# saugns/saugns

Hardware: AMD Instinct MI355X
Metric: mono samples/sec/GPU @ N voices (depth-3 FM) (higher is better)
Workload: dtype f32 (f64 table interpolation, u32 phase)

## Files before the change

### __graft_entry__.py

```python
import os
import subprocess
import sys

ROOT = os.path.dirname(os.path.abspath(__file__))
if ROOT not in sys.path:
    sys.path.insert(0, ROOT)


def build():
    import saugns_amd
    saugns_amd.build(force=False)
    subprocess.check_call(["make", "-s", "-C", os.path.join(ROOT, "tests", "seqexec")])
    subprocess.check_call(["make", "-s", "-C", os.path.join(ROOT, "tests", "hooks")])
    subprocess.check_call(["make", "-s", "-C", os.path.join(ROOT, "tests", "hooks_levels")])
    subprocess.check_call(["make", "-s", "-C", os.path.join(ROOT, "tests", "hooks_oversample")])
    subprocess.check_call(["make", "-s", "-C", os.path.join(ROOT, "tests", "hooks_loudness")])
    subprocess.check_call(["make", "-s", "-C", os.path.join(ROOT, "tests", "hooks_limiter")])
    subprocess.check_call(["make", "-s", "-C", os.path.join(ROOT, "tests", "hooks_spectrum")])
    subprocess.check_call(["make", "-s", "-C", os.path.join(ROOT, "tests", "hooks_plan")])
    subprocess.check_call(["make", "-s", "-C", os.path.join(ROOT, "oracle"), "oracle"])
    subprocess.check_call(["make", "-s", "-C", os.path.join(ROOT, "oracle"), "ref"])
    subprocess.check_call(["make", "-s", "-C", os.path.join(ROOT, "oracle"), "hosts"])
    saugns_amd.lib()


def smoke():
    import numpy as np
    import saugns_amd as sa
    from saugns_amd import voicebank
    from oracle import pyoracle as po

    tabs = np.fromfile(os.path.join(ROOT, "tests", "golden", "piluts_ref.f32"),
                       dtype="<f4").reshape(12, 2048)
    sa.set_piluts(tabs)
    po.oracle_use_tables(tabs)
    po.oracle().ora_set_fastmath_forms(1)
    prg = voicebank.config3(n=16, seconds=1)
    want = po.oracle_render(prg.ptr, 44100, False)
    got = sa.Generator(prg, 44100).render(stereo=False)
    assert len(got) == len(want) == 44100, (len(got), len(want))
    diff = int(np.abs(got.astype(np.int32) - want.astype(np.int32)).max())
    assert diff == 0, f"GPU render differs from the oracle by {diff} LSB"
    print("smoke ok: 16 voices x depth-3 PM, 44100 frames, bit-exact vs oracle")
    from saugns_amd.api import POP_FMOD
    fm = [voicebank.Op("sin", freq=voicebank.Line(110.0 + 20 * k, goal=330.0, shape="exp"), time_ms=500,
                       mods={POP_FMOD: [voicebank.Op("sin", freq=5.0 + k, amp=20.0)]}) for k in range(8)]
    for name, p in (("8 FM voices with gliding carriers", voicebank.build_program(fm)),
                    ("16 feedback voices (config 5)", voicebank.config5(n=16, seconds=1))):
        want = po.oracle_render(p.ptr, 44100, False)
        got = sa.Generator(p, 44100).render(stereo=False)
        assert len(got) == len(want) and (got == want).all(), name
        print(f"smoke ok: {name}, {len(got)} frames, bit-exact vs oracle")


if __name__ == "__main__":
    build()
    if "--smoke" in sys.argv:
        smoke()
```

### saugns_amd/build.py

```python
import os
import subprocess
import sys

HERE = os.path.dirname(os.path.abspath(__file__))
CSRC = os.path.join(HERE, "csrc")
LIB = os.path.join(HERE, "libsaugns_amd.so")
SOURCES = ["capi.cpp", "engine.cpp", "plan.cpp", "tables.cpp", "program_io.cpp", "sndout.cpp", "bank_builder.cpp",
           "hip_backend.hip"]
HEADERS = ["engine.h", "hip_backend.h", "capi_internal.h", "sau_dev_math.h", "sau_dev_ops.h", "launch_plan.h",
           "k_common.h", "k_wave_scan.h", "k_block_loop.h", "k_fast_types.h", "k_analyze.h", "k_decode.h", "k_fast_voice.h", "k_fast_group.h", "k_fast_group_lm.h",
           "k_chain.h", "k_finish.h", "k_levels.h", "k_decimate.h", "k_loudness.h", "k_limiter.h", "k_spectrum.h",
           "sau_dev_types.h", "../../include/sau_abi.h", "../../include/saugns_amd.h"]
FLAGS = ["--offload-arch=gfx950", "-O3", "-ffp-contract=off", "-fPIC", "-std=c++17",
         "-Wall", "-fvisibility=hidden", "-fvisibility-inlines-hidden"]


def _stale():
    if not os.path.exists(LIB):
        return True
    t = os.path.getmtime(LIB)
    deps = [os.path.join(CSRC, f) for f in SOURCES + HEADERS] + [__file__]
    return any(os.path.getmtime(d) > t for d in deps)


def build_variant(name, defines):
    build()
    hipcc = os.environ.get("HIPCC", "/opt/rocm/bin/hipcc")
    vdir = os.path.join(HERE, "variants")
    os.makedirs(vdir, exist_ok=True)
    obj = os.path.join(vdir, "hip_backend_%s.o" % name)
    subprocess.check_call([hipcc] + FLAGS + ["-D" + d for d in defines] +
                          ["-c", os.path.join(CSRC, "hip_backend.hip"), "-o", obj])
    objs = [os.path.join(CSRC, s.rsplit(".", 1)[0] + ".o") for s in SOURCES if s != "hip_backend.hip"]
    out = os.path.join(vdir, "lib_%s.so" % name)
    subprocess.check_call([hipcc, "--offload-arch=gfx950", "-shared", "-fPIC", "-o", out] + objs + [obj, "-ldl"])
    return out


def build(force=False, verbose=False):
    if not force and not _stale():
        return LIB
    import fcntl
    with open(os.path.join(HERE, ".build.lock"), "w") as lock:
        fcntl.flock(lock, fcntl.LOCK_EX)
        try:
            if not force and not _stale():
                return LIB
            return _build(verbose, force)
        finally:
            fcntl.flock(lock, fcntl.LOCK_UN)


def _build(verbose, force=False):
    hipcc = os.environ.get("HIPCC", "/opt/rocm/bin/hipcc")
    objs = []
    for src in SOURCES:
        obj = os.path.join(CSRC, src.rsplit(".", 1)[0] + ".o")
        objs.append(obj)
        deps = [src] + [h for h in HEADERS if src.endswith(".hip") or not h.startswith("k_")]
        if not force and os.path.exists(obj) and all(
                os.path.getmtime(os.path.join(CSRC, d)) <= os.path.getmtime(obj) for d in deps) and \
                os.path.getmtime(__file__) <= os.path.getmtime(obj):
            continue
        cmd = [hipcc] + FLAGS + ["-c", os.path.join(CSRC, src), "-o", obj]
        if verbose:
            print(" ".join(cmd), file=sys.stderr)
        subprocess.check_call(cmd)
    cmd = [hipcc, "--offload-arch=gfx950", "-shared", "-fPIC", "-o", LIB] + objs + ["-ldl"]
    subprocess.check_call(cmd)
    return LIB


if __name__ == "__main__":
    if len(sys.argv) > 2 and sys.argv[1] == "--variant":
        print(build_variant(sys.argv[2], sys.argv[3:]))
    else:
        print(build(force="--force" in sys.argv, verbose=True))
```

### saugns_amd/csrc/hip_backend.hip

```cpp
#include <hip/hip_runtime.h>
#include "hip_backend.h"
#include "launch_plan.h"
#include "sau_dev_ops.h"
#include <stdio.h>
#include <stdlib.h>
#include <string.h>
#include <deque>
#include <map>
#include <mutex>
#include <string>
#include <type_traits>
#include <vector>

namespace sauhip {

using namespace saudev;
using sauengine::BackendConfig;
using sauengine::tune_env;
using sauengine::SegmentDesc;
using namespace sauplan;

#include "k_common.h"
#include "k_block_loop.h"
#include "k_fast_types.h"
// ... 129 lines not shown
}
static void pool_free(bool pinned, void *q, size_t bytes) {
	if (!q) return;
	if (!BufPool::get().give(pinned, q, bytes)) { if (pinned) (void)hipHostFree(q); else (void)hipFree(q); }
}

static std::mutex &attr_mutex() { static std::mutex *m = new std::mutex; return *m; }
static bool raise_lds_attr(const void *fn, size_t lds, int dev, std::string &err) {
	static std::map<std::pair<const void *, int>, size_t> *slots = new std::map<std::pair<const void *, int>, size_t>;
	std::lock_guard<std::mutex> lk(attr_mutex());
	size_t &configured = (*slots)[std::make_pair(fn, dev & 15)];
	if (lds > configured) {
		hipError_t e = hipFuncSetAttribute(fn, hipFuncAttributeMaxDynamicSharedMemorySize, (int)lds);
		if (e != hipSuccess) { err = std::string("hipFuncSetAttribute: ") + hipGetErrorString(e); return false; }
		configured = lds;
	}
	return true;
}

enum : unsigned { FK_WIDE = 1, FK_TAIL = 2, FK_CUB = 4, FK_INNER = 8, FK_LANEMAJOR = 16 };
static const void *fast_kernel_fn(int build, uint32_t rows, unsigned form) {
	struct Entry { int build; uint32_t rows; unsigned form; const void *fn; };
#define FK(build, form, ...) {build, FK_ROWS(__VA_ARGS__), form, (const void *)fast_kernel<__VA_ARGS__>}
#define FK_ROWS(rows, ...) rows
	static const Entry table[] = {
		FK(0, 0, 2, 0), FK(0, 0, 4, 0), FK(0, 0, 5, 0), FK(0, 0, 6, 0), FK(0, 0, 8, 0),
		FK(1, 0, 2, 1), FK(1, 0, 4, 1),
		FK(2, 0, 2, 2), FK(2, 0, 4, 2), FK(2, 0, 5, 2), FK(2, 0, 6, 2), FK(2, 0, 8, 2),
		FK(3, 0, 4, 3), FK(3, 0, 5, 3), FK(3, 0, 6, 3),
		FK(0, FK_WIDE, 6, 0, false, true), FK(0, FK_WIDE, 8, 0, false, true), FK(0, FK_WIDE, 10, 0, false, true), FK(0, FK_WIDE, 12, 0, false, true),
		FK(2, FK_WIDE | FK_TAIL, 8, 2, false, true, true), FK(2, FK_WIDE, 8, 2, false, true), FK(2, FK_TAIL, 8, 2, false, false, true),
		FK(2, FK_CUB, (int)FAST_CUB_ROWS, 2, true),
		FK(0, FK_WIDE | FK_INNER | FK_LANEMAJOR, 12, 0, false, true, false, true, true), FK(0, FK_WIDE | FK_INNER, 12, 0, false, true, false, true),
		FK(0, FK_CUB, (int)FAST_CUB_ROWS, 0, true)};
#undef FK
#undef FK_ROWS
	for (const Entry &e : table)
		if (e.build == build && e.rows == rows && e.form == form) return e.fn;
	return nullptr;
}
static const void *repair_kernel_fn(uint32_t rows, bool wide) {
	if (wide)
		return rows == 12 ? (const void *)repair_kernel<12, true> : rows == 10 ? (const void *)repair_kernel<10, true>
		     : rows == 8 ? (const void *)repair_kernel<8, true> : rows == 6 ? (const void *)repair_kernel<6, true> : nullptr;
	return rows == 8 ? (const void *)repair_kernel<8> : rows == 6 ? (const void *)repair_kernel<6> : rows == 5 ? (const void *)repair_kernel<5>
	     : rows == 4 ? (const void *)repair_kernel<4> : rows == 2 ? (const void *)repair_kernel<2> : nullptr;
}
static const void *render_kernel_fn(uint32_t W, uint32_t T, uint32_t V, bool HB) {
	struct Entry { uint32_t W, T, V; bool HB; const void *fn; };
#define RK(W, T, V, HB) {W, T, V, HB, (const void *)render_kernel<W, T, V, HB>}
	static const Entry table[] = {
		RK(1, 4, 8, false), RK(1, 3, 8, false), RK(1, 2, 8, false), RK(1, 1, 8, false),
		RK(1, 4, 16, false), RK(1, 3, 16, false), RK(1, 2, 16, false), RK(1, 1, 16, false),
		RK(1, 1, 1, true), RK(1, 1, 1, false), RK(4, 4, 1, false), RK(8, 2, 1, false)};
#undef RK
	for (const Entry &e : table)
		if (e.W == W && e.T == T && e.V == V && e.HB == HB) return e.fn;
	return nullptr;
}

template <typename T, bool PINNED> struct PoolBuf {
	T *p = nullptr;
	size_t cap = 0, bytes = 0;
	PoolBuf() = default;
	PoolBuf(const PoolBuf &) = delete;
	PoolBuf &operator=(const PoolBuf &) = delete;
	~PoolBuf() { release(); }
	bool ensure(size_t n, std::string &err, bool keep = false) {
		if (n <= cap) return true;
		size_t nbytes = (n + n / 4 + 16) * sizeof(T);
		T *q = (T *)pool_alloc(PINNED, nbytes, err);
		if (!q) return false;
		if (keep && p && cap) {
			hipError_t e = PINNED ? (memcpy(q, p, cap * sizeof(T)), hipSuccess)
			                      : hipMemcpy(q, p, cap * sizeof(T), hipMemcpyDeviceToDevice);
			if (e != hipSuccess) { err = hipGetErrorString(e); return false; }
		}
		if (p) { (void)hipDeviceSynchronize(); pool_free(PINNED, p, bytes); }
		p = q; bytes = nbytes; cap = nbytes / sizeof(T);
		return true;
	}
	void release() { pool_free(PINNED, p, bytes); p = nullptr; cap = 0; bytes = 0; }
};
template <typename T> using DevBuf = PoolBuf<T, false>;
template <typename T> using PinBuf = PoolBuf<T, true>;

struct TableSet {
	int dev;
	std::vector<float> piluts;
	WaveConst wconst[12];
	HerpC23 *c23;
	HerpC01 *c01;
	WaveConst *wc;
};
static const TableSet *shared_tables(const float *piluts, const WaveConst *wconst, std::string &err) {
	static std::mutex mu;
	static std::vector<TableSet *> sets;
	int dev = 0;
	(void)hipGetDevice(&dev);
	std::lock_guard<std::mutex> lk(mu);
	for (const TableSet *t : sets)
		if (t->dev == dev && !memcmp(t->piluts.data(), piluts, (size_t)12 * WAVE_LEN * sizeof(float)) &&
		    !memcmp(t->wconst, wconst, sizeof t->wconst))
			return t;
	std::vector<HerpC23> h23((size_t)12 * WAVE_LEN);
	std::vector<HerpC01> h01((size_t)12 * WAVE_LEN);
	for (uint32_t wv = 0; wv < 12; ++wv)
		for (uint32_t i = 0; i < WAVE_LEN; ++i) {
			if (!herp_c1_scalable(piluts + (size_t)wv * WAVE_LEN, i)) {
				err = "wave table has slopes below 2^-100: unsupported";
				return nullptr;
			}
			herp_coeffs(piluts + (size_t)wv * WAVE_LEN, i,
					h23[(size_t)wv * WAVE_LEN + i], h01[(size_t)wv * WAVE_LEN + i]);
		}
	TableSet *t = new TableSet;
	t->dev = dev;
	t->piluts.assign(piluts, piluts + (size_t)12 * WAVE_LEN);
	memcpy(t->wconst, wconst, sizeof t->wconst);
	t->c23 = nullptr; t->c01 = nullptr; t->wc = nullptr;
	hipError_t e = hipMalloc((void **)&t->c23, h23.size() * sizeof(HerpC23));
	if (e == hipSuccess) e = hipMalloc((void **)&t->c01, h01.size() * sizeof(HerpC01));
	if (e == hipSuccess) e = hipMalloc((void **)&t->wc, 12 * sizeof(WaveConst));
	if (e == hipSuccess) e = hipMemcpy(t->c23, h23.data(), h23.size() * sizeof(HerpC23), hipMemcpyHostToDevice);
	if (e == hipSuccess) e = hipMemcpy(t->c01, h01.data(), h01.size() * sizeof(HerpC01), hipMemcpyHostToDevice);
	if (e == hipSuccess) e = hipMemcpy(t->wc, wconst, 12 * sizeof(WaveConst), hipMemcpyHostToDevice);
	if (e != hipSuccess) {
		err = std::string("wave tables: ") + hipGetErrorString(e);
		(void)hipFree(t->c23); (void)hipFree(t->c01); (void)hipFree(t->wc);
		delete t;
		return nullptr;
	}
	sets.push_back(t);
	return t;
}

int device_count() {
	int n = 0;
	if (hipGetDeviceCount(&n) != hipSuccess) return 0;
	return n;
}

bool device_pci_bus_id(int dev, char *buf, int len) {
	if (!buf || len < 16) return false;
	buf[0] = 0;
	return hipDeviceGetPCIBusId(buf, len, dev) == hipSuccess;
}

class HipBackendImpl : public HipBackend {
public:
	explicit HipBackendImpl(int device = -1) : want_dev_(device) {}
	void use_device() { (void)hipSetDevice(dev_); }

	~HipBackendImpl() override {
		use_device();
		if (stream_) (void)hipStreamSynchronize(stream_);
		if (chain_stream_) { (void)hipStreamSynchronize(chain_stream_); StreamPool::get().give(dev_, chain_stream_, 1); }
		for (hipEvent_t e : chain_ev_) (void)hipEventDestroy(e);
		for (int i = 0; i < 4; ++i) if (fetch_ev_[i]) (void)hipEventDestroy(fetch_ev_[i]);
		if (after_ev_) (void)hipEventDestroy(after_ev_);
		for (auto &e : events_) { (void)hipEventDestroy(e.a); (void)hipEventDestroy(e.b); }
		if (stream_) StreamPool::get().give(dev_, stream_);
	}

	bool init(const BackendConfig &cfg, std::string &err) override {
		cfg_ = cfg;
		int dev = 0;
		const char *env = getenv("SAU_AMD_DEVICE");
		if (want_dev_ >= 0) dev = want_dev_;
		else if (env) dev = atoi(env);
		if (dev < 0 || dev >= device_count()) { err = "no HIP device " + std::to_string(dev) + " (" + std::to_string(device_count()) + " visible)"; return false; }
		HIP_OK(hipSetDevice(dev));
		dev_ = dev;
		stream_ = StreamPool::get().take(dev);
		if (!stream_) HIP_OK(hipStreamCreateWithFlags(&stream_, hipStreamNonBlocking));
		static std::mutex prop_mu;
		static size_t dev_lds[16];
		static uint32_t dev_cus[16];
		static size_t dev_free[16];
		{
			std::lock_guard<std::mutex> lk(prop_mu);
			if (!dev_lds[dev & 15]) {
				hipDeviceProp_t prop;
				HIP_OK(hipGetDeviceProperties(&prop, dev));
				dev_lds[dev & 15] = prop.maxSharedMemoryPerMultiProcessor ? prop.maxSharedMemoryPerMultiProcessor
				                                                          : prop.sharedMemPerBlock;
				dev_cus[dev & 15] = prop.multiProcessorCount > 0 ? (uint32_t)prop.multiProcessorCount : FK_GRID;
				size_t mfree = 0, mtotal = 0;
				if (hipMemGetInfo(&mfree, &mtotal) == hipSuccess) dev_free[dev & 15] = mfree;
			}
			free_hint_ = dev_free[dev & 15];
			tun_ = tuning_from_env(tune_env);
			lim_ = device_limits(dev_lds[dev & 15], dev_cus[dev & 15], tun_);
		}
		debug_ = getenv("SAU_AMD_DEBUG") != nullptr;
		inmix_report_ = tune_env("SAU_AMD_INMIX_REPORT") != nullptr;
		inner_report_ = tune_env("SAU_AMD_INNER_REPORT") != nullptr;
		if (!ops_.ensure(cfg.op_count ? cfg.op_count : 1, err)) return false;
		HIP_OK(hipMemsetAsync(ops_.p, 0, ops_.cap * sizeof(DevOp), stream_));
		tables_ = shared_tables(cfg.piluts, cfg.wconst, err);
		if (!tables_) return false;
		memcpy(wconst_, cfg.wconst, sizeof wconst_);
		return true;
	}

	bool reserve_frames(uint32_t max_frames, bool , std::string &err) override {
		use_device();
		HIP_OK(hipStreamSynchronize(stream_));
		row_stride_ = (max_frames + 63) & ~63u;
		pcm_row_ = (size_t)row_stride_ * 2;
		if (!pcm_.ensure(pcm_row_ * cfg_.n_streams * pcm_units(), err)) return false;
		set_.vout_rows = 0;
		return true;
	}

	size_t pcm_units() const { return pcm_f32_ ? 2 : 1; }
	size_t pcm_pitch() const { return pcm_row_ * pcm_units() * sizeof(int16_t); }
	char *pcm_at(uint32_t stream) const { return (char *)pcm_.p + pcm_pitch() * stream; }
	bool set_format(sauengine::SampleFormat fmt, std::string &err) override {
		use_device();
		const bool f32 = fmt == sauengine::SF_F32;
		if (f32 == pcm_f32_) return true;
		pcm_f32_ = f32;
		if (pcm_row_ && !pcm_.ensure(pcm_row_ * cfg_.n_streams * pcm_units(), err)) { pcm_f32_ = !f32; return false; }
		return true;
	}

	void *stage(const void *src, size_t bytes, std::string &err) {
		const size_t need = (bytes + 63) & ~(size_t)63;
		if (arena_used_ + need > arena_.cap) {
			hipError_t e = hipStreamSynchronize(stream_);
			if (e != hipSuccess) { err = std::string("hipStreamSynchronize: ") + hipGetErrorString(e); return nullptr; }
			arena_used_ = 0;
			const size_t want = need > ((size_t)4 << 20) ? need : ((size_t)4 << 20);
			if (want > arena_.cap && !arena_.ensure(want, err)) return nullptr;
		}
		void *p = arena_.p + arena_used_;
		arena_used_ += need;
		memcpy(p, src, bytes);
		return p;
	}
	bool send(void *dst, const void *src, size_t bytes, std::string &err) {
		if (!bytes) return true;
		void *h = stage(src, bytes, err);
		if (!h) return false;
		HIP_OK(hipMemcpyAsync(dst, h, bytes, hipMemcpyHostToDevice, stream_));
		return true;
	}

	bool upload_plans(const Step *steps, const FastIds *fast_ids, size_t n_steps, const uint32_t *op_ids,
			size_t n_ids, std::string &err) override {
		use_device();
		if (!steps_.ensure(n_steps ? n_steps : 1, err) || !op_ids_.ensure(n_ids ? n_ids : 1, err) ||
		    !fast_ids_.ensure(n_steps ? 2 * n_steps : 1, err))
			return false;
		n_steps_total_ = (uint32_t)n_steps;
		return send(steps_.p, steps, n_steps * sizeof(Step), err) &&
			send(fast_ids_.p, fast_ids, 2 * n_steps * sizeof(FastIds), err) &&
			send(op_ids_.p, op_ids, n_ids * sizeof(uint32_t), err);
	}

	bool apply_updates(const OpUpdate *recs, size_t n, std::string &err) override {
		use_device();
		if (!n) return true;
		if (!recs_.ensure(n, err) || !send(recs_.p, recs, n * sizeof(OpUpdate), err)) return false;
		hipLaunchKernelGGL(event_kernel, dim3((unsigned)((n + 63) / 64)), dim3(64), 0, stream_,
				ops_.p, recs_.p, (uint32_t)n, tables_->wc);
		HIP_OK(hipGetLastError());
		return true;
	}

	bool poison_run(uint32_t frames, bool stereo, std::string &err) override {
		(void)frames; (void)stereo;
		use_device();
		if (pcm_.p) HIP_OK(hipMemsetD16Async((hipDeviceptr_t)pcm_.p, 0x5a5a, pcm_row_ * cfg_.n_streams * pcm_units(), stream_));
		return true;
	}

	bool zero_pcm(uint32_t first_stream, uint32_t n_streams, uint32_t first_frame, uint32_t n_frames, bool stereo,
			std::string &err) override {
		use_device();
		if (!pcm_.p || !n_streams || !n_frames) return true;
		const size_t fb = (stereo ? 2 : 1) * pcm_units() * sizeof(int16_t);
		char *at = pcm_at(first_stream) + (size_t)first_frame * fb;
		if (n_streams == 1) HIP_OK(hipMemsetAsync(at, 0, (size_t)n_frames * fb, stream_));
		else HIP_OK(hipMemset2DAsync(at, pcm_pitch(), 0, (size_t)n_frames * fb, n_streams, stream_));
		return true;
	}

	struct TimedPair { hipEvent_t a, b; int kind; bool used; };

	struct Job {
		const SegmentDesc &seg;
		PlanInputs in;
		BlockLoopPlan bl;
		FastPlan fk;
		RenderParams rp;
		FastParams fp;
		FastParams cfp;
		bool launched = true;
		bool tail_live = false;
		bool inmix_live = false;
		uint32_t early_mixed_blocks = 0;
		uint32_t block_grid = 1;
		TimedPair *tf = nullptr;
		explicit Job(const SegmentDesc &s) : seg(s) { memset(&rp, 0, sizeof rp); memset(&fp, 0, sizeof fp); }
	};

	bool render(const SegmentDesc &seg, std::string &err) override {
		use_device();
		if (!seg.n_voices) return true;
		++acc_launches_;
		Job j(seg);
		j.in.f32 = seg.format == sauengine::SF_F32;
		if (j.in.f32 != pcm_f32_) { err = "a segment of another sample format than the run announced"; return false; }
		if (j.in.f32 && seg.swap_bytes) { err = "float32 samples are not byte-swapped"; return false; }
		j.in.row_stride = row_stride_; j.in.pcm_row = pcm_row_; j.in.chain_budget = chain_rows_budget();
		j.bl = plan_block_loop(seg, tun_, lim_);
		if (!j.bl.ok) { err = "voice too large for one workgroup's LDS (block buffers + operator states)"; return false; }
		if (!ensure_rows(j, err) || !upload_descriptors(j, err)) return false;
		j.fk = plan_fast(seg, tun_, lim_, j.in);
		if (!prepare_fast(j, err) || !prepare_chains(j, err)) return false;
		fill_tables(j);
		if (!launch_analyze(j, err)) return false;
		if (j.fk.use_fast) {
			if (!launch_decode(j, err)) return false;
			if (j.fk.main_build == 2 && !launch_split(j, err)) return false;
			if (j.fp.scan ? !launch_sums_and_chains(j, err) : !launch_closed_form(j, err)) return false;
			if (!launch_cub(j, err)) return false;
			if (!j.launched) return false;
			if (!launch_repair(j, err)) return false;
			if (j.tf) (void)hipEventRecord(j.tf->b, stream_);
		}
		if (!launch_finalize(j, err)) return false;
		if (!launch_block_loop(j, err)) return false;
		return launch_mixer(j, err);
	}

	bool ensure_rows(Job &j, std::string &err) {
		const SegmentDesc &seg = j.seg;
		MixSet &S = set_;
		if (!voices_.ensure(seg.n_voices, err) || !S.vinfo.ensure(seg.n_voices, err)) return false;
		if (seg.n_voices > S.vout_rows || !S.vout.p) {
			HIP_OK(hipStreamSynchronize(stream_));
			if (!S.vout.ensure((size_t)seg.n_voices * row_stride_, err)) return false;
			S.vout_rows = seg.n_voices;
		}
		if (seg.n_pan_rows && !S.pan.ensure((size_t)seg.n_pan_rows * row_stride_, err)) return false;
		if (tun_.poison) {
			HIP_OK(hipMemsetD32Async((hipDeviceptr_t)S.vout.p, 0x3ea5a5a5, (size_t)seg.n_voices * row_stride_, stream_));
			if (seg.n_pan_rows) HIP_OK(hipMemsetD32Async((hipDeviceptr_t)S.pan.p, 0x3ea5a5a5, (size_t)seg.n_pan_rows * row_stride_, stream_));
		}
		return S.mstreams.ensure(seg.n_streams, err);
	}

	bool upload_descriptors(Job &j, std::string &err) {
		const SegmentDesc &seg = j.seg;
		MixSet &S = set_;
		ms_host_.resize(seg.n_streams);
		for (uint32_t s = 0; s < seg.n_streams; ++s) {
			MixStream &m = ms_host_[s];
			memset(&m, 0, sizeof m);
			m.first_row = seg.streams[s].first_voice;
			m.n_rows = seg.streams[s].n_voices;
			m.amp_scale = seg.streams[s].amp_scale;
			m.write_len = seg.streams[s].write_len;
			m.pcm = (int16_t *)pcm_at(s);
			if (m.write_len > j.in.max_write) j.in.max_write = m.write_len;
			if (m.n_rows > j.in.max_rows) j.in.max_rows = m.n_rows;
		}
		const bool same_voices = voices_sent_.size() == seg.n_voices && voices_dev_ == voices_.p &&
			memcmp(voices_sent_.data(), seg.voices, seg.n_voices * sizeof(VoiceDesc)) == 0;
		const bool same_ms = S.ms_sent.size() == seg.n_streams && S.ms_dev == S.mstreams.p &&
			memcmp(S.ms_sent.data(), ms_host_.data(), seg.n_streams * sizeof(MixStream)) == 0;
		if (!same_voices) {
			if (!send(voices_.p, seg.voices, seg.n_voices * sizeof(VoiceDesc), err)) return false;
			voices_sent_.assign(seg.voices, seg.voices + seg.n_voices);
			voices_dev_ = voices_.p;
		}
		if (!same_ms) {
			if (!send(S.mstreams.p, ms_host_.data(), seg.n_streams * sizeof(MixStream), err)) return false;
			S.ms_sent = ms_host_;
			S.ms_dev = S.mstreams.p;
		}
		return true;
	}

	bool prepare_fast(Job &j, std::string &err) {
		const SegmentDesc &seg = j.seg;
		const FastPlan &k = j.fk;
		FastParams &fp = j.fp;
		MixSet &S = set_;
		const size_t n_lists = (size_t)FAST_LISTS * seg.n_voices * k.fmax_steps;
		if (!finfo_.ensure(seg.n_voices, err) || !fdone_.ensure(seg.n_voices, err) ||
		    !worklist_.ensure(seg.n_voices, err) || !work_count_.ensure(4, err) ||
		    !fsteps_.ensure(n_lists * sizeof(FastStep), err) || !flines_.ensure(n_lists * sizeof(FastLine), err) ||
		    !faux_.ensure(n_lists * sizeof(FastAux), err)) return false;
		fp.voices = voices_.p; fp.steps = steps_.p; fp.fast_ids = fast_ids_.p; fp.op_ids = op_ids_.p; fp.ops = ops_.p;
		fp.vout = S.vout.p; fp.pan = S.pan.p; fp.info = finfo_.p; fp.fast_done = fdone_.p;
		fp.worklist = worklist_.p; fp.work_count = work_count_.p; fp.vinfo = S.vinfo.p;
		fp.g_c23 = tables_->c23; fp.g_c01 = tables_->c01; fp.fsteps = (FastStep *)fsteps_.p; fp.flines = (FastLine *)flines_.p; fp.faux = (FastAux *)faux_.p;
		fp.row_stride = row_stride_; fp.n_voices = seg.n_voices; fp.n_fast = k.n_fast;
		fp.seq_enable = k.seq_ok ? 1u : 0u; fp.ids_full_ofs = n_steps_total_;
		fp.scan = nullptr; fp.scan_groups = k.scan_groups; fp.mode = 0;
		if (tun_.xcd_queues && lim_.eight_xcds) {
			if (!inmix_ctl_.ensure(INMIX_WORDS, err)) return false;
			fp.inmix = inmix_ctl_.p;
		}
		if (k.scan) {
			if (!scan_.ensure((size_t)seg.n_voices * FAST_MAX_SCAN * k.scan_groups, err)) return false;
			fp.scan = scan_.p;
		}
		if (k.look) {
			if (k.look_words_real || !k.look_inside) {
				const unsigned long long *before = look_.p;
				if (!look_.ensure(k.look_words, err)) return false;
				if (look_.p != before || look_epoch_ >= (1u << 30) - 1) {
					HIP_OK(hipMemsetAsync(look_.p, 0, look_.cap * sizeof(unsigned long long), stream_));
					look_epoch_ = 0;
				}
				fp.look_epoch = ++look_epoch_;
			} else if (!look_.p && !look_.ensure(64, err)) {
				return false;
			}
			fp.look = look_.p;
		}
		if (!pass_flags_.p) {
			if (!pass_flags_.ensure(FAST_FLAGS, err)) return false;
			HIP_OK(hipMemsetAsync(pass_flags_.p, 0, pass_flags_.cap * sizeof(uint32_t), stream_));
		}
		fp.pass_flags = pass_flags_.p;
		fp.sum_levels = k.sum_levels;
		if (!repair_.ensure((size_t)seg.n_voices * FAST_REPAIR_WORDS, err)) return false;
		fp.repair = repair_.p;
		fp.repair_on = tun_.repair ? 1u : 0u;
		fp.max_ops = seg.max_ops; fp.max_steps = k.fmax_steps; fp.np = 64; fp.rows = k.rows; fp.rows_multi = k.rows_multi;
		fp.enable = k.use_fast ? 1u : 0u;
		if (k.inc_rows) {
			if (!inc_rows_.ensure((size_t)seg.n_inc_rows * 2 * k.inc_stride + 64, err)) return false;
			fp.inc_rows = inc_rows_.p; fp.inc_stride = k.inc_stride; fp.n_inc_rows = seg.n_inc_rows;
		}
		if (k.split_cf) {
			if (!vlists_.ensure((size_t)2 * seg.n_voices, err)) return false;
			fp.vlists = vlists_.p; fp.split_cf = 1; fp.rows_cf = k.rows_cf;
			fp.look_words_real = k.look_words_real && fp.look ? 1u : 0u;
		}
		fp.cub_ok = k.cub_ok ? 1u : 0u;
		memcpy(fp.wc, wconst_, sizeof wconst_);
		return true;
	}

	bool prepare_chains(Job &j, std::string &err) {
		const SegmentDesc &seg = j.seg;
		FastPlan &k = j.fk;
		FastParams &fp = j.fp;
		if (k.chains) {
			std::string rows_err;
			const size_t rows_need = (size_t)seg.n_chain_rows * 2 * k.chain_stride + 64;
			const char *rft = chain_rows_failed_once_ ? nullptr : tune_env("SAU_AMD_CHAIN_ROWS_FAIL");
			const bool rows_fail_test = rft && strcmp(rft, "real") != 0;
			if (rows_fail_test || !chain_rows_.ensure((rft && !rows_fail_test) ? (size_t)1 << 44 : rows_need, rows_err)) {
				chain_rows_failed_once_ = true;
				++chain_rows_failures_;
				if (debug_) fprintf(stderr, "saugns_amd: %zu bytes of chain rows not available (%s): block loop for this segment\n",
						rows_need * sizeof(float), rows_err.c_str());
				k.drop_chains();
			}
		}
		if (k.chains) {
			if (!chain_desc_.ensure(seg.n_chain_slots, err) ||
			    !fplines_.ensure((size_t)FAST_LISTS * seg.n_voices * k.fmax_steps * sizeof(FastLine), err)) return false;
			if (seg.chain_rows_padded) HIP_OK(hipMemsetAsync(chain_desc_.p, 0, (size_t)seg.n_chain_slots * sizeof(ChainDesc), stream_));
			fp.chain_rows = chain_rows_.p; fp.chain_stride = k.chain_stride; fp.n_chain_rows = seg.n_chain_rows; fp.n_chain_slots = seg.n_chain_slots;
			fp.chain_desc = chain_desc_.p; fp.fplines = (FastLine *)fplines_.p;
			fp.chain_inline = tun_.chain_inline ? 1u : 0u;
			fp.chain_early_ok = tun_.chain_early ? 1u : 0u;
			memcpy(fp.ctab_of_wave, k.ctabs.tab_of_wave, sizeof fp.ctab_of_wave);
			memcpy(fp.cwave_of_tab, k.ctabs.wave_of_tab, sizeof fp.cwave_of_tab);
			fp.n_ctabs = k.ctabs.n;
		}
		fp.lean_on = k.lean_on ? 1u : 0u;
		fp.rows_lean = k.rows_lean;
		return true;
	}

	void fill_tables(Job &j) {
		memcpy(j.fp.tab_of_wave, j.fk.tabs.tab_of_wave, sizeof j.fp.tab_of_wave);
		memcpy(j.fp.wave_of_tab, j.fk.tabs.wave_of_tab, sizeof j.fp.wave_of_tab);
		j.fp.n_tabs = j.fk.tabs.n;
	}

	bool launch_analyze(Job &j, std::string &err) {
		const SegmentDesc &seg = j.seg;
		(void)err;
		TimedPair *ta = timing_on_ ? new_pair(3) : nullptr;
		if (ta) (void)hipEventRecord(ta->a, stream_);
		uint32_t lo = seg.max_ops, ls = seg.max_steps;
		size_t albytes = (size_t)lo * sizeof(DevOp) + (size_t)ls * sizeof(Step) + (size_t)lo * sizeof(uint32_t);
		if (albytes > 48 * 1024 || !tun_.analyze_lds) { lo = 0; ls = 0; albytes = 0; }
		hipLaunchKernelGGL(analyze_kernel, dim3(seg.n_voices), dim3(64), albytes, stream_, j.fp, lo, ls);
		if (ta) (void)hipEventRecord(ta->b, stream_);
		return true;
	}
	bool launch_decode(Job &j, std::string &err) {
		hipLaunchKernelGGL(decode_kernel, dim3(j.seg.n_voices), dim3(64), 0, stream_, j.fp);
		if (!wait_for_predecessor(err)) return false;
		j.tf = timing_on_ ? new_pair(2) : nullptr;
		if (j.tf) (void)hipEventRecord(j.tf->a, stream_);
		return true;
	}

	bool launch_build(Job &j, std::string &err, int build, uint32_t rows, uint32_t grid, const FastParams *prm = nullptr, bool cf = false,
			bool wide = false) {
		if (build == 1 && rows > 4) rows = 4;
		if (build == 3) rows = rows < 5 ? 4 : rows > 6 ? 6 : rows;
		const void *fn = fast_kernel_fn(build, rows, (wide ? FK_WIDE : 0u) | (build == 2 && j.tail_live ? FK_TAIL : 0u));
		if (!fn) {
			err = "internal error: no fast_kernel build with " + std::to_string(rows) + " rows per pass in this form";
			return false;
		}
		const size_t lds = j.fk.launch_lds(build, rows, wide, cf);
		void *args[] = {(void *)(prm ? prm : &j.fp)};
		if (!raise_lds_attr(fn, lds, dev_, err)) return false;
		HIP_OK(hipLaunchKernel(fn, dim3(grid), dim3(1024), args, lds, stream_));
		return true;
	}
	void launch_fast(Job &j, std::string &err, uint32_t mode, uint32_t grid = 0) {
		FastParams &fp = j.fp;
		if (!grid) grid = j.fk.grid;
		fp.mode = mode;
		if (fp.lean_on && fp.chain_rows && (mode == fp.sum_levels + 1 || mode == fp.sum_levels + 2) &&
		    !launch_build(j, err, 3, fp.rows_lean, grid))
			j.launched = false;
		if (j.fk.main_build == 2) {
			fp.only_multi = 1;
			if (!launch_build(j, err, 1, j.fk.rows_multi, grid)) j.launched = false;
			fp.only_multi = 0;
		} else if (!launch_build(j, err, j.fk.main_build, j.fk.rows, grid, nullptr, false, j.fk.wide_cf)) {
			j.launched = false;
		}
	}

	bool launch_split(Job &j, std::string &err) {
		const SegmentDesc &seg = j.seg;
		const FastPlan &k = j.fk;
		FastParams &fp = j.fp, &cfp = j.cfp;
		if (k.tailmix) {
			if (!tail_ok_.ensure(seg.n_streams, err)) return false;
			fp.tail_ok = tail_ok_.p; fp.inmix_stream = set_.mstreams.p;
			fp.tail_flags = (seg.stereo ? 1u : 0u) | (seg.swap_bytes ? 2u : 0u);
			fp.tail_pcm_offset = seg.pcm_offset;
			hipLaunchKernelGGL(tailmix_kernel, dim3((seg.n_streams + 63) / 64), dim3(64), 0, stream_, fp, seg.n_streams);
			j.tail_live = true;
		}
		cfp = fp;
		cfp.n_fast = k.n_fast_cf; cfp.rows = k.rows_cf; cfp.mode = 0; cfp.only_multi = 0;
		if (getenv("SAU_AMD_DEBUG_DUO"))
			fprintf(stderr, "[sau-amd] duo %d: enabled %d look %d words_real %u FT %u rows_cf %u cub_ok %u tail %d may_scan %u of %u voices, lds %zu of %zu\n",
					(int)k.duo, (int)tun_.duo, fp.look != nullptr, fp.look_words_real, k.rows, k.rows_cf, fp.cub_ok, (int)j.tail_live, seg.n_may_scan, seg.n_voices,
					k.launch_lds(2, k.rows, false) + 1024, lim_.lds_limit);
		cfp.dyn_chunks = k.tasks_cf.dyn_chunks; cfp.dyn_static = k.tasks_cf.dyn_static;
		if (!k.duo && !launch_build(j, err, 0, k.rows_cf, k.grid_cf, &cfp, true, k.wide_cf)) j.launched = false;
		fp.mode = fp.sum_levels + 1; fp.only_multi = 0; fp.look_wpv = k.look_wpv; fp.look_groups = k.groups;
		fp.look_wpv_flags = k.look_wpv_flags;
		if (k.duo) {
			const size_t dlds = k.launch_lds(2, k.rows, false);
			if (!raise_lds_attr((const void *)duo_kernel, dlds, dev_, err)) return false;
			auto go = [&]() -> bool {
				void *da[] = {(void *)&fp, (void *)&cfp};
				return hipLaunchKernel((const void *)duo_kernel, dim3(lim_.fk_grid), dim3(1024), da, dlds, stream_) == hipSuccess;
			};
			if (!SpreadLaunchOrder::get().ordered(dev_, stream_, go)) j.launched = false;
		} else if (fp.look) {
			if (k.look_inside) {
				if (!launch_build(j, err, 2, k.rows, k.grid_look, nullptr, false, k.wide_look)) j.launched = false;
			} else if (!SpreadLaunchOrder::get().ordered(dev_, stream_, [&]() { return launch_build(j, err, 2, k.rows, k.grid_look, nullptr, false, k.wide_look); })) {
				j.launched = false;
			}
			if (fp.cub_ok) {
				const void *ck2 = fast_kernel_fn(2, FAST_CUB_ROWS, FK_CUB);
				const size_t lds2 = k.launch_lds(2, FAST_CUB_ROWS, false);
				if (!raise_lds_attr(ck2, lds2, dev_, err)) return false;
				auto go = [&]() -> bool {
					void *a2[] = {(void *)&fp};
					return hipLaunchKernel(ck2, dim3(k.grid_look), dim3(1024), a2, lds2, stream_) == hipSuccess;
				};
				if (k.look_inside ? !go() : !SpreadLaunchOrder::get().ordered(dev_, stream_, go)) j.launched = false;
			}
		}
		return true;
	}

	bool launch_sums_and_chains(Job &j, std::string &err) {
		const SegmentDesc &seg = j.seg;
		FastParams &fp = j.fp;
		if (fp.chain_rows && fp.chain_early_ok && !launch_early_chains(j, err)) return false;
		for (uint32_t pass = 1; pass <= fp.sum_levels && (!fp.look || seg.n_chain_rows); ++pass) {
			launch_fast(j, err, pass);
			hipLaunchKernelGGL(scan_kernel, dim3(seg.n_voices), dim3(64), 0, stream_, fp);
		}
		if (!fp.chain_rows) { launch_fast(j, err, fp.sum_levels + 1); return true; }
		return launch_chains(j, err);
	}

	bool launch_early_chains(Job &j, std::string &err) {
		FastParams &fp = j.fp;
		const uint32_t cgrid = j.fk.chain_grid;
		const size_t clds = chain_alone_lds((size_t)fp.n_ctabs * CHAIN_TAB_BYTES + CHAIN_IO_BYTES, cgrid);
		if (!raise_lds_attr((const void *)chain_kernel, clds, dev_, err)) return false;
		fp.chain_early = 1; fp.range_mode = 0;
		hipLaunchKernelGGL(chain_kernel, dim3(cgrid), dim3(192), clds, stream_, fp);
		const size_t rlds = chain_alone_lds(RCHAIN_LDS_BYTES, cgrid);
		if (!raise_lds_attr((const void *)rchain_kernel, rlds, dev_, err)) return false;
		hipLaunchKernelGGL(rchain_kernel, dim3(cgrid), dim3(RCHAIN_THREADS), rlds, stream_, fp);
		fp.chain_early = 0;
		return true;
	}

	bool launch_chains(Job &j, std::string &err) {
		const FastPlan &k = j.fk;
		FastParams &fp = j.fp;
		const uint32_t cgrid = k.chain_grid, n_chunks = k.chunks.n;
		const size_t clds = chain_alone_lds((size_t)fp.n_ctabs * CHAIN_TAB_BYTES + CHAIN_IO_BYTES, cgrid);
		if (!raise_lds_attr((const void *)chain_kernel, clds, dev_, err)) return false;
		TimedPair *tc = nullptr;
		if (n_chunks == 1) {
			tc = timing_on_ ? new_pair(0) : nullptr;
			fp.range_mode = 0;
			launch_fast(j, err, fp.sum_levels + 2);
			if (tc) (void)hipEventRecord(tc->a, stream_);
			hipLaunchKernelGGL(chain_kernel, dim3(cgrid), dim3(192), clds, stream_, fp);
			if (tc) (void)hipEventRecord(tc->b, stream_);
			launch_fast(j, err, fp.sum_levels + 1);
			return true;
		}
		if (!chain_stream_) {
			chain_stream_ = StreamPool::get().take(dev_, 1);
			if (!chain_stream_) {
				int lo = 0, hi = 0;
				(void)hipDeviceGetStreamPriorityRange(&lo, &hi);
				HIP_OK(hipStreamCreateWithPriority(&chain_stream_, hipStreamNonBlocking, hi));
			}
		}
		while (chain_ev_.size() < 2 * (size_t)n_chunks) {
			hipEvent_t e;
			HIP_OK(hipEventCreateWithFlags(&e, hipEventDisableTiming));
			chain_ev_.push_back(e);
		}
		tc = timing_on_ ? new_pair(0) : nullptr;
		const uint32_t *cb = k.chunks.cb;
		auto set_range = [&](FastParams &q, uint32_t mode, uint32_t c) {
			q.range_mode = mode; q.f_lo = cb[c]; q.f_hi = c + 1 == n_chunks ? 0xffffffffu : cb[c + 1];
		};
		for (uint32_t c = 0; c < n_chunks; ++c) {
			set_range(fp, 1, c);
			fp.range_last = c + 1 == n_chunks;
			launch_fast(j, err, fp.sum_levels + 2, k.pass_grid);
			HIP_OK(hipEventRecord(chain_ev_[2 * c], stream_));
			HIP_OK(hipStreamWaitEvent(chain_stream_, chain_ev_[2 * c], 0));
			FastParams cp = fp;
			set_range(cp, 1, c);
			if (tc && c == 0) (void)hipEventRecord(tc->a, chain_stream_);
			hipLaunchKernelGGL(chain_kernel, dim3(cgrid), dim3(192), clds, chain_stream_, cp);
			if (tc && c + 1 == n_chunks) (void)hipEventRecord(tc->b, chain_stream_);
			HIP_OK(hipEventRecord(chain_ev_[2 * c + 1], chain_stream_));
		}
		uint32_t mixed_blocks = 0;
		if (k.early_mix) hipLaunchKernelGGL(premix_kernel, dim3((j.seg.n_voices + 63) / 64), dim3(64), 0, stream_, fp);
		for (uint32_t c = 0; c < n_chunks; ++c) {
			HIP_OK(hipStreamWaitEvent(stream_, chain_ev_[2 * c + 1], 0));
			set_range(fp, 2, c);
			fp.range_last = c + 1 == n_chunks;
			launch_fast(j, err, fp.sum_levels + 1, c + 1 == n_chunks ? k.grid : k.pass_grid);
			if (k.early_mix && c + 1 < n_chunks && cb[c + 1] > 512) {
				const uint32_t hi = (cb[c + 1] - 512) / 256;
				if (hi > mixed_blocks) {
					MixParams mp = mix_params(j.seg, set_);
					mp.blk_lo = mixed_blocks; mp.blk_hi = hi;
					TimedPair *tm = timing_on_ ? new_pair(1) : nullptr;
					if (tm) (void)hipEventRecord(tm->a, stream_);
					hipLaunchKernelGGL((j.in.f32 ? mix_kernel_f32 : mix_kernel), dim3(hi - mixed_blocks, j.seg.n_streams), dim3(256), 0, stream_, mp);
					if (tm) (void)hipEventRecord(tm->b, stream_);
					mixed_blocks = hi;
				}
			}
		}
		j.early_mixed_blocks = mixed_blocks;
		fp.range_mode = 0; fp.f_lo = 0; fp.f_hi = 0; fp.range_last = 0;
		return true;
	}

	bool launch_closed_form(Job &j, std::string &err) {
		const SegmentDesc &seg = j.seg;
		const FastPlan &k = j.fk;
		FastParams &fp = j.fp;
		fp.dyn_chunks = k.tasks.dyn_chunks; fp.dyn_static = k.tasks.dyn_static; fp.dyn_small = k.tasks.dyn_small;
		if (k.queues) {
			fp.inmix_flags = k.inmix_flags;
			fp.inmix_div_s = k.div.s; fp.inmix_div_m = k.div.m;
			if (k.inmix) {
				fp.inmix_stream = set_.mstreams.p;
				fp.inmix_pcm_offset = seg.pcm_offset;
				hipLaunchKernelGGL(premix_kernel, dim3((seg.n_voices + 63) / 64), dim3(64), 0, stream_, fp);
				j.inmix_live = true;
			}
		}
		if (k.inner != INNER_NONE) {
			const bool lm = k.inner == INNER_LANE_MAJOR;
			const void *ik = fast_kernel_fn(0, 12, FK_WIDE | FK_INNER | (lm ? FK_LANEMAJOR : 0u));
			const size_t lds = k.inner_lds();
			FastParams ep = fp;
			ep.mode = 0; ep.edge_only = 1; ep.dyn_static = 1; ep.dyn_chunks = 2; ep.dyn_small = 0; ep.inmix_flags = 0;
			if (!launch_build(j, err, 0, k.rows, k.grid_edge, &ep, false, true)) j.launched = false;
			fp.mode = 0;
			void *iargs[] = {(void *)&fp};
			if (!raise_lds_attr(ik, lds, dev_, err)) return false;
			HIP_OK(hipLaunchKernel(ik, dim3(k.grid), dim3(1024), iargs, lds, stream_));
			if (inner_report_) fprintf(stderr, "[sau-amd] inner: %s, %u voices\n", lm ? "lane-major" : "row-major", seg.n_voices);
		} else {
			if (inner_report_) fprintf(stderr, "[sau-amd] inner: none (rows %u, wide %d, chunks %u), %u voices\n", k.rows, k.wide_cf ? 1 : 0, fp.dyn_chunks, seg.n_voices);
			launch_fast(j, err, 0);
		}
		fp.dyn_chunks = 0; fp.inmix_flags = 0; fp.dyn_small = 0;
		return true;
	}

	bool launch_cub(Job &j, std::string &err) {
		if (!j.fp.cub_ok) return true;
		const FastPlan &k = j.fk;
		FastParams q = k.main_build == 2 ? j.cfp : j.fp;
		q.n_fast = k.n_fast_cf; q.rows = FAST_CUB_ROWS; q.mode = 0; q.only_multi = 0;
		q.dyn_chunks = k.tasks_cub.dyn_chunks; q.dyn_static = k.tasks_cub.dyn_static;
		const size_t qlds = k.launch_lds(0, FAST_CUB_ROWS, false, true);
		const void *ck = fast_kernel_fn(0, FAST_CUB_ROWS, FK_CUB);
		if (!raise_lds_attr(ck, qlds, dev_, err)) return false;
		void *qargs[] = {(void *)&q};
		HIP_OK(hipLaunchKernel(ck, dim3(k.grid_cub), dim3(1024), qargs, qlds, stream_));
		return true;
	}

	bool launch_repair(Job &j, std::string &err) {
		const FastPlan &k = j.fk;
		const size_t rlds = k.launch_lds(0, k.rows_repair, k.wide_cf, k.main_build == 2);
		FastParams rpar = k.main_build == 2 ? j.cfp : j.fp;
		rpar.mode = 0;
		const void *rk = repair_kernel_fn(k.rows_repair, k.wide_cf);
		if (!rk) {
			err = "internal error: no repair_kernel build with " + std::to_string(k.rows_repair) + " rows per pass in this form";
			return false;
		}
		if (!raise_lds_attr(rk, rlds, dev_, err)) return false;
		j.fp.mode = 0;
		void *rargs[] = {(void *)&rpar};
		HIP_OK(hipLaunchKernel(rk, dim3(k.grid_repair), dim3(1024), rargs, rlds, stream_));
		return true;
	}

	bool launch_finalize(Job &j, std::string &err) {
		const SegmentDesc &seg = j.seg;
		TimedPair *tz = timing_on_ ? new_pair(3) : nullptr;
		if (tz) (void)hipEventRecord(tz->a, stream_);
		hipLaunchKernelGGL(finalize_kernel, dim3((unsigned)(((size_t)seg.n_voices * j.fp.max_ops * 8 + 63) / 64)), dim3(64), 0,
				stream_, j.fp);
		if (tz) (void)hipEventRecord(tz->b, stream_);
		HIP_OK(hipGetLastError());
		if (debug_ && j.fk.use_fast) {
			(void)hipStreamSynchronize(stream_);
			FastInfo fi0;
			(void)hipMemcpy(&fi0, finfo_.p, sizeof fi0, hipMemcpyDeviceToHost);
			fprintf(stderr, "[sau-amd] fast: voice 0 total %u H %u bail %u steps %u seq %u; n_fast %u rows %u\n",
					fi0.total, fi0.H, fi0.bail, fi0.n_fsteps, fi0.seq, j.fk.n_fast, j.fk.rows);
			std::vector<FastStep> fs(fi0.n_fsteps < 64 ? fi0.n_fsteps : 64);
			if (!fs.empty()) (void)hipMemcpy(fs.data(), fsteps_.p, fs.size() * sizeof(FastStep), hipMemcpyDeviceToHost);
			for (size_t i = 0; i < fs.size(); ++i)
				fprintf(stderr, "[sau-amd]   step %zu kind %u flags %#x which %u dep %u out %d pm %d fpm %d amp %d aux %d type %#x inc %u ac %g fc %g ramp %u\n",
						i, fs[i].kind & 0xff, (fs[i].kind >> 8) & 0xff, (fs[i].kind >> 16) & 0xff, fs[i].kind >> 24,
						(int)fs[i].out_off, (int)fs[i].pm_off, (int)fs[i].fpm_off, (int)fs[i].amp_off, (int)fs[i].aux_off,
						fs[i].type, fs[i].inc, fs[i].ac, fs[i].fc, fs[i].ramp);
		}
		return true;
	}

	bool launch_block_loop(Job &j, std::string &err) {
		const SegmentDesc &seg = j.seg;
		const BlockLoopPlan &b = j.bl;
		RenderParams &rp = j.rp;
		rp.team_bytes = (uint32_t)b.team_bytes;
		memcpy(rp.tab_of_wave, b.tabs.tab_of_wave, sizeof rp.tab_of_wave);
		memcpy(rp.wave_of_tab, b.tabs.wave_of_tab, sizeof rp.wave_of_tab);
		rp.voices = voices_.p; rp.steps = steps_.p; rp.op_ids = op_ids_.p; rp.ops = ops_.p;
		rp.vout = set_.vout.p; rp.pan = set_.pan.p; rp.vinfo = set_.vinfo.p;
		rp.g_c23 = tables_->c23; rp.g_c01 = tables_->c01;
		rp.row_stride = row_stride_; rp.seg_len = seg.len;
		rp.n_slots = seg.n_slots; rp.max_ops = seg.max_ops; rp.n_tabs = b.tabs.n;
		rp.max_steps = seg.max_steps; rp.n_main = seg.n_main;
		memcpy(rp.wc, wconst_, sizeof wconst_);
		rp.fast_done = fdone_.p; rp.worklist = worklist_.p; rp.work_count = work_count_.p;
		j.block_grid = b.grid(seg, j.fk.use_fast);
		if (b.HB) {
			const size_t stride = ((size_t)seg.n_slots * 64 * sizeof(float) + (size_t)seg.max_ops * sizeof(DevOp) +
				(size_t)seg.max_steps * sizeof(Step) + 255) / 256 * 256 / sizeof(float);
			if (stride > 0xffffffffu) { err = "voice too large (block buffers + operator records beyond 16 GiB)"; return false; }
			if (!big_slots_.ensure((size_t)j.block_grid * stride, err)) return false;
			rp.big_slots = big_slots_.p; rp.big_stride = (uint32_t)stride;
		}
		if (!wait_for_predecessor(err)) return false;
		TimedPair *tp = timing_on_ ? new_pair(0) : nullptr;
		if (tp) (void)hipEventRecord(tp->a, stream_);
		const void *fn = render_kernel_fn(b.W, b.T, b.V, b.HB);
		if (!fn) { err = "internal error: no render_kernel build of this geometry"; return false; }
		if (!raise_lds_attr(fn, b.lds, dev_, err)) return false;
		void *args[] = {(void *)&rp};
		HIP_OK(hipLaunchKernel(fn, dim3(j.block_grid), dim3(64 * b.W * b.V), args, b.lds, stream_));
		HIP_OK(hipGetLastError());
		if (tp) (void)hipEventRecord(tp->b, stream_);
		if (debug_) debug_dump("after render", seg, j.block_grid);
		return true;
	}

	bool launch_mixer(Job &j, std::string &err) {
		const SegmentDesc &seg = j.seg;
		const uint32_t max_write = j.in.max_write;
		const Mixer which = plan_mixer(seg, tun_, j.in, pcm_pitch(), j.inmix_live, j.early_mixed_blocks);
		if (which == MIX_NONE) return true;
		MixParams mp = mix_params(seg, set_);
		mp.early_blocks = j.early_mixed_blocks;
		mp.inmix = j.inmix_live ? inmix_ctl_.p : nullptr;
		mp.tail_ok = j.tail_live ? tail_ok_.p : nullptr;
		TimedPair *tm = timing_on_ ? new_pair(1) : nullptr;
		if (tm) (void)hipEventRecord(tm->a, stream_);
		switch (which) {
		case MIX_FEW_F32: hipLaunchKernelGGL(mix_few_kernel_f32, dim3((max_write + 1023) / 1024, seg.n_streams), dim3(256), 0, stream_, mp); break;
		case MIX_F32: hipLaunchKernelGGL(mix_kernel_f32, dim3((max_write + 255) / 256, seg.n_streams), dim3(256), 0, stream_, mp); break;
		case MIX_FEW: hipLaunchKernelGGL(mix_few_kernel, dim3((max_write + 1023) / 1024, seg.n_streams), dim3(256), 0, stream_, mp); break;
		case MIX_64: hipLaunchKernelGGL(mix_kernel64, dim3((max_write + 63) / 64, seg.n_streams), dim3(64), 0, stream_, mp); break;
		default: hipLaunchKernelGGL(mix_kernel, dim3((max_write + 255) / 256, seg.n_streams), dim3(256), 0, stream_, mp); break;
		}
		HIP_OK(hipGetLastError());
		if (tm) (void)hipEventRecord(tm->b, stream_);
		if (mp.inmix && inmix_report_) report_inmix(mp, seg.n_voices, max_write);
		return true;
	}

	void report_inmix(const MixParams &mp, uint32_t n_voices, uint32_t max_write) {
		std::vector<uint32_t> h(INMIX_WORDS);
		uint32_t g[2] = {0, 0};
		(void)hipStreamSynchronize(stream_);
		(void)hipMemcpy(h.data(), mp.inmix, INMIX_WORDS * sizeof(uint32_t), hipMemcpyDeviceToHost);
		(void)hipMemcpy(g, work_count_.p, sizeof g, hipMemcpyDeviceToHost);
		const uint32_t nch = h[INMIX_NCH] < INMIX_MAX_CHUNKS ? h[INMIX_NCH] : INMIX_MAX_CHUNKS, tpc = h[INMIX_TPC];
		uint32_t tiles = 0, whole = 0, all = 0;
		for (uint32_t k = 0; k < nch; ++k) {
			uint32_t lo_f = k * h[INMIX_CF], hi_f = lo_f + h[INMIX_CF];
			if (k >= h[INMIX_NCH1]) { lo_f = h[INMIX_BASE] + (k - h[INMIX_NCH1]) * h[INMIX_CFS]; hi_f = lo_f + h[INMIX_CFS]; }
			else if (hi_f > h[INMIX_BASE]) hi_f = h[INMIX_BASE];
			if (hi_f > max_write) hi_f = max_write;
			const uint32_t tk = hi_f > lo_f ? (hi_f - lo_f + INMIX_TILE - 1) / INMIX_TILE : 0u;
			uint32_t c = 0;
			for (uint32_t j = 0; j < tk && j < tpc && j < INMIX_MAX_TPC; ++j) c += (h[INMIX_CHUNK + INMIX_LINE * k + INMIX_BITS + (j >> 5)] >> (j & 31u)) & 1u;
			tiles += c; whole += c == tk ? 1u : 0u; all += tk;
		}
		fprintf(stderr, "[sau-amd] inmix: voices %u frames %u chunks %u x %u frames, tiles %u of %u, chunks mixed whole %u, guard %u %u\n",
				n_voices, max_write, nch, h[INMIX_CF], tiles, all, whole, g[0], g[1]);
	}

	template <typename SetT> MixParams mix_params(const SegmentDesc &seg, const SetT &S) {
		MixParams mp;
		mp.streams = S.mstreams.p; mp.vout = S.vout.p; mp.pan = S.pan.p; mp.vinfo = S.vinfo.p;
		mp.row_stride = row_stride_; mp.pcm_offset = seg.pcm_offset;
		mp.stereo = seg.stereo ? 1 : 0;
		mp.swap_bytes = seg.swap_bytes ? 1 : 0;
		mp.blk_lo = 0; mp.blk_hi = 0; mp.early_blocks = 0; mp.guard = work_count_.p; mp.inmix = nullptr; mp.tail_ok = nullptr;
		return mp;
	}

	bool fetch_pcm(uint32_t stream, int16_t *dst, uint32_t frames, bool stereo, std::string &err) override {
		if (pcm_f32_) { err = "the last run's samples are float32"; return false; }
		return fetch_units(stream, dst, (size_t)frames * (stereo ? 2 : 1), err);
	}
	bool fetch_pcm_f32(uint32_t stream, float *dst, uint32_t frames, bool stereo, std::string &err) override {
		if (!pcm_f32_) { err = "the last run's samples are int16"; return false; }
		return fetch_units(stream, (int16_t *)dst, (size_t)frames * (stereo ? 2 : 1) * 2, err);
	}
	bool fetch_units(uint32_t stream, int16_t *dst, const size_t n, std::string &err) {
		use_device();
		const bool pinned = host_blocks_.count(dst) != 0;
		if (!pinned && !h_pcm_.ensure(n, err)) return false;
		HIP_OK(hipMemcpyAsync(pinned ? dst : h_pcm_.p, pcm_at(stream), n * sizeof(int16_t),
				hipMemcpyDeviceToHost, stream_));
		HIP_OK(hipStreamSynchronize(stream_));
		if (!pinned) memcpy(dst, h_pcm_.p, n * sizeof(int16_t));
		return true;
	}

	bool fetch_pcm_async(uint32_t stream, int16_t *dst, uint32_t frames, bool stereo, int slot,
			std::string &err) override {
		if (pcm_f32_) { err = "the last run's samples are float32"; return false; }
		return fetch_bytes_async(stream, dst, (size_t)frames * (stereo ? 2 : 1) * sizeof(int16_t), slot, err);
	}
	bool fetch_pcm_f32_async(uint32_t stream, float *dst, uint32_t frames, bool stereo, int slot,
			std::string &err) override {
		if (!pcm_f32_) { err = "the last run's samples are int16"; return false; }
		return fetch_bytes_async(stream, dst, (size_t)frames * (stereo ? 2 : 1) * sizeof(float), slot, err);
	}
	bool fetch_bytes_async(uint32_t stream, void *dst, size_t bytes, int slot, std::string &err) {
		slot &= 3;
		use_device();
		if (!fetch_ev_[slot]) HIP_OK(hipEventCreateWithFlags(&fetch_ev_[slot], hipEventDisableTiming));
		hipStream_t cs = stream_;
		HIP_OK(hipMemcpyAsync(dst, pcm_at(stream), bytes, hipMemcpyDeviceToHost, cs));
		HIP_OK(hipEventRecord(fetch_ev_[slot], cs));
		return true;
	}
	bool wait_fetch(int slot, std::string &err) override {
		slot &= 3;
		if (fetch_ev_[slot]) HIP_OK(hipEventSynchronize(fetch_ev_[slot]));
		return true;
	}
	void *alloc_host(size_t bytes) override {
		use_device();
		std::string err;
		void *p = pool_alloc(true, bytes, err);
		if (p) host_blocks_[p] = bytes;
		return p;
	}
	void free_host(void *p) override {
		use_device();
		auto it = host_blocks_.find(p);
		if (it == host_blocks_.end()) return;
		(void)hipStreamSynchronize(stream_);
		pool_free(true, p, it->second);
		host_blocks_.erase(it);
	}

	bool begin_metering(std::string &err) override {
		use_device();
		if (lev_acc_.p) return true;
		if (!lev_acc_.ensure(cfg_.n_streams, err)) return false;
		HIP_OK(hipMemsetAsync(lev_acc_.p, 0, (size_t)cfg_.n_streams * sizeof(LevelsAcc), stream_));
		return true;
	}
	bool launch_levels(LevelsParams lp, const LevelsPlan &plan, std::string &err) {
		if (!plan.blocks) lp.parts = nullptr;
		else {
			if (!lev_parts_.ensure(plan.parts, err)) return false;
			lp.parts = lev_parts_.p;
			lp.blocks = plan.blocks;
			if (lp.f32) hipLaunchKernelGGL(levels_kernel<float>, dim3(plan.blocks, plan.rows), dim3(LEVELS_THREADS), 0, stream_, lp);
			else hipLaunchKernelGGL(levels_kernel<int16_t>, dim3(plan.blocks, plan.rows), dim3(LEVELS_THREADS), 0, stream_, lp);
			HIP_OK(hipGetLastError());
		}
		hipLaunchKernelGGL(levels_finish_kernel, dim3(plan.finish_grid), dim3(64), 0, stream_, lp);
		HIP_OK(hipGetLastError());
		return true;
	}
	bool measure_streams(const uint32_t *frames, bool stereo, sauengine::SampleFormat format, std::string &err) override {
		use_device();
		const bool f32 = format == sauengine::SF_F32;
		if (!lev_acc_.p) { err = "level metering has not begun"; return false; }
		if (f32 != pcm_f32_ || !pcm_.p) { err = "no rows of that sample format to measure"; return false; }
		uint32_t longest = 0;
		for (uint32_t s = 0; s < cfg_.n_streams; ++s) {
			if (frames[s] > row_stride_) { err = "frames beyond the streams' rows"; return false; }
			if (frames[s] > longest) longest = frames[s];
		}
		if (!longest) return true;
		const LevelsPlan plan = plan_levels(longest, stereo ? 2 : 1, cfg_.n_streams);
		if (!plan.ok) { err = "too many streams for one level measurement"; return false; }
		if (!lev_frames_.ensure(cfg_.n_streams, err) || !send(lev_frames_.p, frames, (size_t)cfg_.n_streams * sizeof(uint32_t), err)) return false;
		LevelsParams lp;
		memset((void *)&lp, 0, sizeof lp);
		lp.rows = pcm_.p; lp.pitch = pcm_pitch();
		lp.row_frames = lev_frames_.p;
		lp.channels = stereo ? 2 : 1;
		lp.acc = lev_acc_.p; lp.n_rows = cfg_.n_streams; lp.f32 = f32 ? 1 : 0; lp.accumulate = 1;
		return launch_levels(lp, plan, err);
	}
	static void levels_out(const LevelsAcc &a, sauengine::Levels &o) {
		o.frames = a.frames;
		for (int c = 0; c < 2; ++c) {
			const float ip = (float)a.ipeak[c] / 32767.0f;
			o.peak[c] = a.fpeak[c] > ip ? a.fpeak[c] : ip;
			o.sum_sq[c] = a.fsum[c] + (double)a.isum[c] / (32767.0 * 32767.0);
			o.over[c] = a.over[c]; o.full_scale[c] = a.full[c]; o.nonfinite[c] = a.nonf[c];
		}
	}
	bool read_records(const LevelsAcc *dev, size_t n, sauengine::Levels *out, std::string &err) {
		std::vector<LevelsAcc> h(n);
		HIP_OK(hipMemcpyAsync(h.data(), dev, n * sizeof(LevelsAcc), hipMemcpyDeviceToHost, stream_));
		HIP_OK(hipStreamSynchronize(stream_));
		for (size_t i = 0; i < n; ++i) levels_out(h[i], out[i]);
		return true;
	}
	bool read_levels(sauengine::Levels *out, bool reset, std::string &err) override {
		use_device();
		if (!lev_acc_.p) { memset((void *)out, 0, sizeof(sauengine::Levels) * cfg_.n_streams); return true; }
		if (!read_records(lev_acc_.p, cfg_.n_streams, out, err)) return false;
		if (reset) HIP_OK(hipMemsetAsync(lev_acc_.p, 0, (size_t)cfg_.n_streams * sizeof(LevelsAcc), stream_));
		return true;
	}
	bool measure_rows(const void *rows, size_t pitch, size_t n_rows, sauengine::SampleFormat format, size_t frames, bool stereo,
			sauengine::Levels *out, std::string &err) override {
		use_device();
		const bool f32 = format == sauengine::SF_F32;
		const size_t ch = stereo ? 2 : 1, size = f32 ? sizeof(float) : sizeof(int16_t);
		if (!n_rows) return true;
		if (!rows || ((uintptr_t)rows & 15u) || (pitch & 15u) || !out) { err = "bad argument: rows and pitch_bytes must be multiples of 16"; return false; }
		if (frames > SIZE_MAX / 8 || (n_rows > 1 && frames * ch * size > pitch)) { err = "bad argument: rows longer than their pitch"; return false; }
		if (frames) {
			hipPointerAttribute_t at;
			memset((void *)&at, 0, sizeof at);
			if (hipPointerGetAttributes(&at, rows) != hipSuccess) { (void)hipGetLastError(); err = "bad argument: rows is not device memory"; return false; }
			if (at.type != hipMemoryTypeDevice || at.device != dev_) { err = "bad argument: rows must be memory of the batch's device"; return false; }
			hipDeviceptr_t base = nullptr;
			size_t span = 0;
			if (hipMemGetAddressRange(&base, &span, (hipDeviceptr_t)rows) != hipSuccess) { (void)hipGetLastError(); err = "bad argument: rows is not device memory"; return false; }
			size_t need = 0;
			const bool wraps = __builtin_mul_overflow(pitch, n_rows - 1, &need) || __builtin_add_overflow(need, frames * ch * size, &need);
			const size_t ofs = (size_t)((const char *)rows - (const char *)base);
			if (wraps || ofs > span || need > span - ofs) { err = "bad argument: the rows reach beyond their allocation"; return false; }
		}
		const LevelsPlan plan = plan_levels(frames, (uint32_t)ch, n_rows);
		if (!plan.ok) { err = "bad argument: too many rows (65535 at most) or frames for one level measurement"; return false; }
		if (!lev_out_.ensure(n_rows, err)) return false;
		LevelsParams lp;
		memset((void *)&lp, 0, sizeof lp);
		lp.rows = rows; lp.pitch = pitch; lp.row_frames = nullptr; lp.frames = frames;
		lp.channels = (uint32_t)ch;
		lp.acc = lev_out_.p; lp.n_rows = (uint32_t)n_rows; lp.f32 = f32 ? 1 : 0; lp.accumulate = 0;
		return launch_levels(lp, plan, err) && read_records(lev_out_.p, n_rows, out, err);
	}
	bool requantize(uint32_t stream, uint32_t frames, bool stereo, float gain, sauengine::SampleFormat out, bool swap_bytes,
			std::string &err) override {
		use_device();
		if (!pcm_f32_ || !pcm_.p) { err = "the last run's samples are not float32"; return false; }
		if (stream >= cfg_.n_streams || frames > row_stride_) { err = "frames beyond the stream's row"; return false; }
		const bool f32 = out == sauengine::SF_F32;
		if (f32 && swap_bytes) { err = "float32 samples are not byte-swapped"; return false; }
		const size_t n = (size_t)frames * (stereo ? 2 : 1);
		if (!n) return true;
		if (!requant_.ensure(n * (f32 ? sizeof(float) : sizeof(int16_t)), err)) return false;
		RequantParams rq;
		rq.src = (const float *)pcm_at(stream); rq.dst = requant_.p; rq.n = n; rq.gain = gain; rq.swap_bytes = swap_bytes ? 1 : 0;
		const dim3 grid((unsigned)((n + 1023) / 1024));
		if (f32) hipLaunchKernelGGL(requant_kernel<float>, grid, dim3(256), 0, stream_, rq);
		else hipLaunchKernelGGL(requant_kernel<int16_t>, grid, dim3(256), 0, stream_, rq);
		HIP_OK(hipGetLastError());
		return true;
	}
	bool fetch_requant_async(void *dst, size_t bytes, int slot, std::string &err) override {
		slot &= 3;
		use_device();
		if (bytes > requant_.bytes) { err = "more bytes than were requantised"; return false; }
		if (!fetch_ev_[slot]) HIP_OK(hipEventCreateWithFlags(&fetch_ev_[slot], hipEventDisableTiming));
		HIP_OK(hipMemcpyAsync(dst, requant_.p, bytes, hipMemcpyDeviceToHost, stream_));
		HIP_OK(hipEventRecord(fetch_ev_[slot], stream_));
		return true;
	}

	bool begin_decimation(int factor, bool stereo, std::string &err) override {
		use_device();
		const DecimPlan plan = plan_decimate(0, factor, stereo ? 2 : 1, cfg_.n_streams, sizeof(float));
		if (!plan.ok) { err = "bad argument"; return false; }
		const size_t hist = (size_t)cfg_.n_streams * plan.hist_floats;
		if (!decim_hist_.ensure(hist, err) || !decim_taps_.ensure(plan.taps, err) || !decim_frames_.ensure(cfg_.n_streams, err)) return false;
		HIP_OK(hipMemsetAsync(decim_hist_.p, 0, hist * sizeof(float), stream_));
		std::vector<double> h(plan.taps);
		if (sauengine::decimator_taps(factor, h.data(), h.size()) != plan.taps) { err = "bad argument"; return false; }
		if (!send(decim_taps_.p, h.data(), h.size() * sizeof(double), err)) return false;
		decim_factor_ = factor; decim_stereo_ = stereo;
		return true;
	}
	template <int K, typename OutT> void launch_decimate(const DecimPlan &plan, const DecimParams &dp, bool stereo) {
		const dim3 grid(plan.tiles, plan.streams), block(DECIM_THREADS);
		if (stereo) hipLaunchKernelGGL((decimate_kernel<K, OutT, 2>), grid, block, 0, stream_, dp, (const double *)decim_taps_.p);
		else hipLaunchKernelGGL((decimate_kernel<K, OutT, 1>), grid, block, 0, stream_, dp, (const double *)decim_taps_.p);
	}
	bool decimate(const uint32_t *frames_hi, uint32_t buf_len, int factor, bool stereo, sauengine::SampleFormat out_fmt, bool swap_bytes,
			std::string &err) override {
		use_device();
		if (!decim_hist_.p || factor != decim_factor_ || stereo != decim_stereo_) { err = "decimation has not begun"; return false; }
		const bool f32 = out_fmt == sauengine::SF_F32;
		if (f32 && swap_bytes) { err = "float32 samples are not byte-swapped"; return false; }
		const uint32_t ch = stereo ? 2 : 1;
		const DecimPlan plan = plan_decimate(buf_len, factor, ch, cfg_.n_streams, f32 ? sizeof(float) : sizeof(int16_t));
		if (!plan.ok) { err = "bad argument"; return false; }
		const unsigned long long n_hi = (unsigned long long)buf_len * (unsigned)factor;
		bool any = false;
		for (uint32_t s = 0; s < cfg_.n_streams; ++s) {
			if (frames_hi[s] > n_hi || frames_hi[s] > row_stride_) { err = "frames beyond the streams' rows"; return false; }
			any = any || frames_hi[s] != 0;
		}
		if (any && (!pcm_f32_ || !pcm_.p)) { err = "the last run's samples are not float32"; return false; }
		decim_out_f32_ = f32; decim_out_pitch_ = plan.out_pitch; decim_out_bytes_ = (size_t)buf_len * ch * (f32 ? sizeof(float) : sizeof(int16_t));
		if (!plan.tiles) return true;
		if (!decim_out_.ensure(plan.out_pitch * cfg_.n_streams, err)) return false;
		if (!send(decim_frames_.p, frames_hi, (size_t)cfg_.n_streams * sizeof(uint32_t), err)) return false;
		DecimParams dp;
		memset((void *)&dp, 0, sizeof dp);
		dp.rows = (const float *)pcm_.p; dp.row_pitch = pcm_f32_ ? pcm_pitch() : 0;
		dp.frames = decim_frames_.p; dp.hist = decim_hist_.p;
		dp.out = decim_out_.p; dp.out_pitch = plan.out_pitch;
		dp.buf_len = buf_len; dp.swap_bytes = swap_bytes ? 1 : 0;
		switch (factor * 2 + (f32 ? 1 : 0)) {
		case 5: launch_decimate<2, float>(plan, dp, stereo); break;
		case 4: launch_decimate<2, int16_t>(plan, dp, stereo); break;
		case 9: launch_decimate<4, float>(plan, dp, stereo); break;
		case 8: launch_decimate<4, int16_t>(plan, dp, stereo); break;
		case 17: launch_decimate<8, float>(plan, dp, stereo); break;
		default: launch_decimate<8, int16_t>(plan, dp, stereo); break;
		}
		HIP_OK(hipGetLastError());
		hipLaunchKernelGGL(decimate_carry_kernel, dim3(plan.streams), dim3(DECIM_CARRY_THREADS), 0, stream_, dp, plan.hist_floats, ch, n_hi);
		HIP_OK(hipGetLastError());
		return true;
	}
	bool fetch_decimated_async(uint32_t stream, void *dst, size_t bytes, int slot, std::string &err) override {
		slot &= 3;
		use_device();
		if (stream >= cfg_.n_streams || bytes > decim_out_bytes_ || (bytes && !decim_out_.p)) { err = "more bytes than were decimated"; return false; }
		if (!fetch_ev_[slot]) HIP_OK(hipEventCreateWithFlags(&fetch_ev_[slot], hipEventDisableTiming));
		if (bytes) {
			const char *src = (const char *)decim_out_.p + decim_out_pitch_ * stream;
			if (host_blocks_.count(dst)) HIP_OK(hipMemcpyAsync(dst, src, bytes, hipMemcpyDeviceToHost, stream_));
			else {
				if (!h_pcm_.ensure((bytes + 1) / 2, err)) return false;
				HIP_OK(hipMemcpyAsync(h_pcm_.p, src, bytes, hipMemcpyDeviceToHost, stream_));
				HIP_OK(hipStreamSynchronize(stream_));
				memcpy(dst, h_pcm_.p, bytes);
			}
		}
		HIP_OK(hipEventRecord(fetch_ev_[slot], stream_));
		return true;
	}
	const float *device_decimated_f32(uint32_t stream) override {
		return decim_out_.p && decim_out_f32_ && decim_out_bytes_ && stream < cfg_.n_streams ? (const float *)((const char *)decim_out_.p + decim_out_pitch_ * stream) : nullptr;
	}
	size_t device_decimated_pitch() override { return decim_out_.p && decim_out_bytes_ ? decim_out_pitch_ : 0; }

	struct LoudSet {
		DevBuf<LoudState> state;
		DevBuf<unsigned long long> pos;
		DevBuf<double> E;
		DevBuf<uint32_t> peak;
		DevBuf<float> hist;
		std::vector<uint64_t> pos_h;
		size_t e_cap = 0;
		uint32_t rows = 0, channels = 0;
	};
	bool loud_setup(uint32_t srate, std::string &err) {
		if (loud_rate_ == srate) return true;
		double f[10], m[16];
		if (!sauengine::loudness_filter(srate, f)) { err = "bad argument: loudness metering needs a rate of 2560 Hz or more"; return false; }
		sauengine::loudness_chunk_map(f, LOUD_CHUNK, m);
		loud_f_ = LoudFilter{f[0], f[1], f[2], f[3], f[4], f[5], f[6], f[7], f[8], f[9]};
		for (int r = 0; r < 4; ++r) for (int k = 0; k < 4; ++k) loud_m_.m[r][k] = m[4 * r + k];
		if (!loud_taps_.p) {
			double g[TP_TAPS];
			if (sauengine::truepeak_taps(g, TP_TAPS) != TP_TAPS || !loud_taps_.ensure(TP_TAPS, err) || !send(loud_taps_.p, g, sizeof g, err)) return false;
		}
		loud_rate_ = srate;
		return true;
	}
	bool loud_clear(LoudSet &L, std::string &err) {
		HIP_OK(hipMemsetAsync(L.state.p, 0, (size_t)L.rows * 2 * sizeof(LoudState), stream_));
		HIP_OK(hipMemsetAsync(L.pos.p, 0, (size_t)L.rows * sizeof(unsigned long long), stream_));
		HIP_OK(hipMemsetAsync(L.peak.p, 0, (size_t)L.rows * 2 * sizeof(uint32_t), stream_));
		HIP_OK(hipMemsetAsync(L.hist.p, 0, (size_t)L.rows * TP_LEAD * 2 * sizeof(float), stream_));
		if (L.e_cap) HIP_OK(hipMemsetAsync(L.E.p, 0, L.e_cap * L.rows * 2 * sizeof(double), stream_));
		L.pos_h.assign(L.rows, 0);
		L.channels = 0;
		return true;
	}
	bool loud_make(LoudSet &L, size_t rows, std::string &err) {
		if (L.rows != rows && L.E.p) {
			HIP_OK(hipStreamSynchronize(stream_));
			L.E.release();
			L.e_cap = 0;
		}
		L.rows = (uint32_t)rows;
		if (!L.state.ensure(rows * 2, err) || !L.pos.ensure(rows, err) || !L.peak.ensure(rows * 2, err) || !L.hist.ensure(rows * TP_LEAD * 2, err)) return false;
		return loud_clear(L, err);
	}
	bool loud_grow(LoudSet &L, size_t need, std::string &err) {
		if (need <= L.e_cap) return true;
		const size_t want = need + need / 2 + 32, per = (size_t)L.rows * 2;
		DevBuf<double> nb;
		if (!nb.ensure(want * per, err)) return false;
		if (L.e_cap) HIP_OK(hipMemcpyAsync(nb.p, L.E.p, L.e_cap * per * sizeof(double), hipMemcpyDeviceToDevice, stream_));
		HIP_OK(hipMemsetAsync(nb.p + L.e_cap * per, 0, (want - L.e_cap) * per * sizeof(double), stream_));
		if (L.E.p) { HIP_OK(hipStreamSynchronize(stream_)); L.E.release(); }
		L.E.p = nb.p; L.E.cap = nb.cap; L.E.bytes = nb.bytes;
		nb.p = nullptr; nb.cap = 0; nb.bytes = 0;
		L.e_cap = want;
		return true;
	}
	bool loud_measure(LoudSet &L, const void *rows, size_t pitch, const uint32_t *frames, uint32_t ch, std::string &err) {
		uint32_t longest = 0;
		for (uint32_t r = 0; r < L.rows; ++r) if (frames[r] > longest) longest = frames[r];
		if (!longest) return true;
		const LoudPlan plan = plan_loudness(longest, ch, L.rows, loud_rate_);
		if (!plan.ok) { err = "bad argument: too many rows (65535 at most) for one loudness measurement"; return false; }
		size_t need = 0;
		for (uint32_t r = 0; r < L.rows; ++r) {
			const size_t h = (size_t)((L.pos_h[r] + frames[r]) / plan.hop) + 1;
			if (h > need) need = h;
		}
		if (!loud_grow(L, need, err)) return false;
		const size_t lanes = (size_t)L.rows * 2 * plan.chunks;
		if (!loud_z_.ensure(lanes, err) || !loud_s_.ensure(lanes, err) || !loud_parts_.ensure(lanes * 2, err) ||
		    !loud_tp_parts_.ensure((size_t)L.rows * plan.tiles * 2, err) || !loud_frames_.ensure(L.rows, err) ||
		    !send(loud_frames_.p, frames, (size_t)L.rows * sizeof(uint32_t), err))
			return false;
		LoudParams lp;
		memset((void *)&lp, 0, sizeof lp);
		lp.rows = (const float *)rows; lp.row_pitch = pitch; lp.frames = loud_frames_.p;
		lp.channels = ch; lp.n_rows = L.rows; lp.hop = plan.hop; lp.chunk_cap = plan.chunks; lp.tile_cap = plan.tiles;
		lp.state = L.state.p; lp.pos = L.pos.p; lp.zstate = loud_z_.p; lp.sstate = loud_s_.p; lp.parts = loud_parts_.p;
		lp.E = L.E.p; lp.e_cap = (uint32_t)(L.e_cap > 0xffffffffull ? 0xffffffffull : L.e_cap);
		lp.tp_parts = loud_tp_parts_.p; lp.peak = L.peak.p; lp.hist = L.hist.p;
		const dim3 cgrid(plan.chunk_grid, plan.rows), tgrid(plan.tiles, plan.rows);
		if (ch == 2) hipLaunchKernelGGL((loud_chunk_kernel<2, 0>), cgrid, dim3(LOUD_THREADS), 0, stream_, lp, loud_f_);
		else hipLaunchKernelGGL((loud_chunk_kernel<1, 0>), cgrid, dim3(LOUD_THREADS), 0, stream_, lp, loud_f_);
		HIP_OK(hipGetLastError());
		hipLaunchKernelGGL(loud_scan_kernel, dim3(plan.lane_grid), dim3(64), 0, stream_, lp, loud_m_);
		HIP_OK(hipGetLastError());
		if (ch == 2) hipLaunchKernelGGL((loud_chunk_kernel<2, 1>), cgrid, dim3(LOUD_THREADS), 0, stream_, lp, loud_f_);
		else hipLaunchKernelGGL((loud_chunk_kernel<1, 1>), cgrid, dim3(LOUD_THREADS), 0, stream_, lp, loud_f_);
		HIP_OK(hipGetLastError());
		if (ch == 2) hipLaunchKernelGGL(truepeak_kernel<2>, tgrid, dim3(TP_THREADS), 0, stream_, lp, (const double *)loud_taps_.p);
		else hipLaunchKernelGGL(truepeak_kernel<1>, tgrid, dim3(TP_THREADS), 0, stream_, lp, (const double *)loud_taps_.p);
		HIP_OK(hipGetLastError());
		hipLaunchKernelGGL(loud_finish_kernel, dim3((plan.rows + 63) / 64), dim3(64), 0, stream_, lp);
		HIP_OK(hipGetLastError());
		hipLaunchKernelGGL(loud_carry_kernel, dim3(plan.rows), dim3(64), 0, stream_, lp);
		HIP_OK(hipGetLastError());
		for (uint32_t r = 0; r < L.rows; ++r) L.pos_h[r] += frames[r];
		L.channels = ch;
		return true;
	}
	bool loud_read(LoudSet &L, sauengine::Loudness *out, std::vector<double> *hops_out, size_t *hops_stride, std::string &err) {
		const size_t per = (size_t)L.rows * 2;
		const uint32_t hop = loud_rate_ / 10, ch = L.channels ? L.channels : 1;
		size_t max_hops = 0;
		for (uint32_t r = 0; r < L.rows; ++r) { const size_t h = (size_t)(L.pos_h[r] / hop); if (h > max_hops) max_hops = h; }
		std::vector<double> E(max_hops * per);
		std::vector<uint32_t> peak(per);
		std::vector<float> hist((size_t)L.rows * TP_LEAD * 2);
		if (max_hops) HIP_OK(hipMemcpyAsync(E.data(), L.E.p, E.size() * sizeof(double), hipMemcpyDeviceToHost, stream_));
		HIP_OK(hipMemcpyAsync(peak.data(), L.peak.p, per * sizeof(uint32_t), hipMemcpyDeviceToHost, stream_));
		HIP_OK(hipMemcpyAsync(hist.data(), L.hist.p, hist.size() * sizeof(float), hipMemcpyDeviceToHost, stream_));
		HIP_OK(hipStreamSynchronize(stream_));
		double g[TP_TAPS];
		(void)sauengine::truepeak_taps(g, TP_TAPS);
		if (hops_out) { hops_out->assign((size_t)L.rows * max_hops * 2, 0.0); *hops_stride = max_hops; }
		std::vector<double> mine;
		for (uint32_t r = 0; r < L.rows; ++r) {
			const size_t nh = (size_t)(L.pos_h[r] / hop);
			mine.assign(nh * 2, 0.0);
			for (size_t h = 0; h < nh; ++h) { mine[2 * h] = E[h * per + (size_t)r * 2]; mine[2 * h + 1] = E[h * per + (size_t)r * 2 + 1]; }
			if (!sauengine::loudness_gate(mine.data(), nh, hop, (int)ch, &out[r])) { err = "bad argument"; return false; }
			out[r].frames = L.pos_h[r];
			uint32_t pk[2] = {peak[(size_t)r * 2], peak[(size_t)r * 2 + 1]};
			if (L.pos_h[r]) sauengine::truepeak_tail(hist.data() + (size_t)r * TP_LEAD * 2, (int)ch, g, pk);
			memcpy(out[r].true_peak, pk, sizeof pk);
			if (hops_out && nh) memcpy(hops_out->data() + (size_t)r * max_hops * 2, mine.data(), nh * 2 * sizeof(double));
		}
		return true;
	}
	bool begin_loudness(std::string &err) override {
		use_device();
		if (loud_own_.state.p) return true;
		return loud_setup(cfg_.srate, err) && loud_make(loud_own_, cfg_.n_streams, err);
	}
	bool measure_loudness(const uint32_t *frames, bool stereo, std::string &err) override {
		use_device();
		if (!loud_own_.state.p) { err = "loudness metering has not begun"; return false; }
		if (!pcm_f32_ || !pcm_.p) { err = "the last run's samples are not float32"; return false; }
		for (uint32_t s = 0; s < cfg_.n_streams; ++s)
			if (frames[s] > row_stride_) { err = "frames beyond the streams' rows"; return false; }
		if (!loud_setup(cfg_.srate, err)) return false;
		return loud_measure(loud_own_, pcm_.p, pcm_pitch(), frames, stereo ? 2 : 1, err);
	}
	bool read_loudness(sauengine::Loudness *out, bool reset, std::string &err) override {
		use_device();
		if (!loud_own_.state.p) { err = "loudness metering has not begun"; return false; }
		if (!loud_setup(cfg_.srate, err) || !loud_read(loud_own_, out, nullptr, nullptr, err)) return false;
		return !reset || loud_clear(loud_own_, err);
	}
	bool read_loudness_hops(uint32_t stream, double *out, size_t cap, size_t *n_hops, std::string &err) override {
		use_device();
		if (!loud_own_.state.p || stream >= cfg_.n_streams) { err = "loudness metering has not begun"; return false; }
		const uint32_t hop = cfg_.srate / 10;
		const size_t nh = (size_t)(loud_own_.pos_h[stream] / hop), per = (size_t)loud_own_.rows * 2;
		*n_hops = nh;
		if (!out || cap < nh || !nh) return true;
		HIP_OK(hipMemcpy2DAsync(out, 2 * sizeof(double), loud_own_.E.p + (size_t)stream * 2, per * sizeof(double), 2 * sizeof(double), nh,
				hipMemcpyDeviceToHost, stream_));
		HIP_OK(hipStreamSynchronize(stream_));
		return true;
	}
	bool measure_loudness_rows(const void *rows, size_t pitch, size_t n_rows, size_t frames, bool stereo, uint32_t srate,
			sauengine::Loudness *out, double *hops_out, size_t hops_cap, std::string &err) override {
		use_device();
		const size_t ch = stereo ? 2 : 1, size = sizeof(float);
		if (!n_rows) return true;
		if (!rows || ((uintptr_t)rows & 15u) || (pitch & 15u) || !out) { err = "bad argument: rows and pitch_bytes must be multiples of 16"; return false; }
		if (frames > 0xffffffffull || (n_rows > 1 && frames * ch * size > pitch)) { err = "bad argument: rows longer than their pitch, or than 32 bits of frames"; return false; }
		if (srate < LOUD_MIN_RATE || n_rows > LOUD_MAX_ROWS) { err = "bad argument: a rate below 2560 Hz, or more than 65535 rows"; return false; }
		if (frames) {
			hipPointerAttribute_t at;
			memset((void *)&at, 0, sizeof at);
			if (hipPointerGetAttributes(&at, rows) != hipSuccess) { (void)hipGetLastError(); err = "bad argument: rows is not device memory"; return false; }
			if (at.type != hipMemoryTypeDevice || at.device != dev_) { err = "bad argument: rows must be memory of the batch's device"; return false; }
			hipDeviceptr_t base = nullptr;
			size_t span = 0;
			if (hipMemGetAddressRange(&base, &span, (hipDeviceptr_t)rows) != hipSuccess) { (void)hipGetLastError(); err = "bad argument: rows is not device memory"; return false; }
			size_t need = 0;
			const bool wraps = __builtin_mul_overflow(pitch, n_rows - 1, &need) || __builtin_add_overflow(need, frames * ch * size, &need);
			const size_t ofs = (size_t)((const char *)rows - (const char *)base);
			if (wraps || ofs > span || need > span - ofs) { err = "bad argument: the rows reach beyond their allocation"; return false; }
		}
		const size_t nh = frames / (srate / 10);
		if (hops_out && hops_cap < n_rows * nh * 2) hops_out = nullptr;
		if (!loud_setup(srate, err) || !loud_make(loud_rows_, n_rows, err)) return false;
		loud_rows_.channels = (uint32_t)ch;
		const std::vector<uint32_t> fr(n_rows, (uint32_t)frames);
		std::vector<double> hops;
		size_t stride = 0;
		const bool ok = loud_measure(loud_rows_, rows, pitch, fr.data(), (uint32_t)ch, err) &&
			loud_read(loud_rows_, out, hops_out ? &hops : nullptr, &stride, err);
		if (ok && hops_out && !hops.empty()) memcpy(hops_out, hops.data(), hops.size() * sizeof(double));
		return ok;
	}

	bool lim_setup(uint32_t srate, std::string &err) {
		if (!lim_taps_.p) {
			double g[TP_TAPS];
			if (sauengine::truepeak_taps(g, TP_TAPS) != TP_TAPS || !lim_taps_.ensure(TP_TAPS, err) || !send(lim_taps_.p, g, sizeof g, err)) return false;
		}
		if (lim_rate_ == srate) return true;
		std::vector<double> h(sauengine::limiter_window(srate, nullptr, 0));
		if (h.empty() || sauengine::limiter_window(srate, h.data(), h.size()) != h.size()) { err = "bad argument"; return false; }
		if (!lim_win_.ensure(2 * LIM_A_MAX + 1, err) || !send(lim_win_.p, h.data(), h.size() * sizeof(double), err)) return false;
		lim_rate_ = srate;
		return true;
	}
	template <typename OutT> void lim_launch_gain(const LimitPlan &plan, const LimParams &lp, bool stereo) {
		const dim3 grid(plan.tiles, plan.streams), block(LIM_THREADS);
		if (stereo) hipLaunchKernelGGL((lim_gain_kernel<OutT, 2>), grid, block, 0, stream_, lp, (const double *)lim_win_.p);
		else hipLaunchKernelGGL((lim_gain_kernel<OutT, 1>), grid, block, 0, stream_, lp, (const double *)lim_win_.p);
	}
	bool lim_launch(const LimitPlan &plan, LimParams &lp, bool stereo, bool f32, std::string &err) {
		const size_t sc = plan.scratch_pitch * plan.streams, parts = (size_t)plan.tiles * plan.streams;
		if (!lim_s_.ensure(sc, err) || !lim_r_.ensure(sc, err) || !lim_part_min_.ensure(parts, err) || !lim_part_cnt_.ensure(parts, err)) return false;
		lp.s = lim_s_.p; lp.r = lim_r_.p; lp.scratch_pitch = plan.scratch_pitch;
		lp.part_min = lim_part_min_.p; lp.part_cnt = lim_part_cnt_.p;
		lp.env_n = plan.env_n; lp.A = plan.A; lp.hist_frames = plan.hist_frames; lp.tiles = plan.tiles; lp.n_streams = plan.streams;
		const dim3 egrid(plan.env_tiles, plan.streams), block(LIM_THREADS);
		if (stereo) hipLaunchKernelGGL(lim_env_kernel<2>, egrid, block, 0, stream_, lp, (const double *)lim_taps_.p);
		else hipLaunchKernelGGL(lim_env_kernel<1>, egrid, block, 0, stream_, lp, (const double *)lim_taps_.p);
		HIP_OK(hipGetLastError());
		if (f32) lim_launch_gain<float>(plan, lp, stereo);
		else lim_launch_gain<int16_t>(plan, lp, stereo);
		HIP_OK(hipGetLastError());
		hipLaunchKernelGGL(lim_finish_kernel, dim3(plan.streams), dim3(64), 0, stream_, lp);
		HIP_OK(hipGetLastError());
		return true;
	}
	bool lim_clear_stats(LimStats *dst, size_t n, std::string &err) {
		const std::vector<LimStats> empty(n, LimStats{0, 0, 1.0});
		return send(dst, empty.data(), n * sizeof(LimStats), err);
	}
	bool begin_limiting(bool stereo, std::string &err) override {
		use_device();
		const LimitPlan plan = plan_limit(0, cfg_.srate, stereo ? 2 : 1, cfg_.n_streams, sizeof(float));
		if (!plan.ok) { err = "bad argument"; return false; }
		const size_t hist = (size_t)cfg_.n_streams * plan.hist_frames * 2;
		if (!lim_hist_[0].ensure(hist, err) || !lim_hist_[1].ensure(hist, err) || !lim_frames_.ensure(cfg_.n_streams, err)) return false;
		if (!lim_stats_.p) {
			if (!lim_stats_.ensure(cfg_.n_streams, err) || !lim_clear_stats(lim_stats_.p, cfg_.n_streams, err)) return false;
		}
		lim_cur_ = 0;
		HIP_OK(hipMemsetAsync(lim_hist_[0].p, 0, hist * sizeof(float), stream_));
		lim_on_ = true; lim_stereo_ = stereo;
		return true;
	}
	bool limit(const uint32_t *frames, uint32_t buf_len, float pre_gain, float ceiling, bool stereo, sauengine::SampleFormat out_fmt,
			bool swap_bytes, std::string &err) override {
		use_device();
		if (!lim_on_ || stereo != lim_stereo_) { err = "limiting has not begun"; return false; }
		if (!sauengine::limiter_param_ok(pre_gain) || !sauengine::limiter_param_ok(ceiling)) { err = "bad argument"; return false; }
		const bool f32 = out_fmt == sauengine::SF_F32;
		if (f32 && swap_bytes) { err = "float32 samples are not byte-swapped"; return false; }
		const uint32_t ch = stereo ? 2 : 1;
		const LimitPlan plan = plan_limit(buf_len, cfg_.srate, ch, cfg_.n_streams, f32 ? sizeof(float) : sizeof(int16_t));
		if (!plan.ok) { err = "bad argument"; return false; }
		bool any = false;
		for (uint32_t s = 0; s < cfg_.n_streams; ++s) {
			if (frames[s] > buf_len || frames[s] > row_stride_) { err = "frames beyond the streams' rows"; return false; }
			any = any || frames[s] != 0;
		}
		if (any && (!pcm_f32_ || !pcm_.p)) { err = "the last run's samples are not float32"; return false; }
		lim_out_f32_ = f32; lim_out_pitch_ = plan.out_pitch; lim_out_bytes_ = (size_t)buf_len * ch * (f32 ? sizeof(float) : sizeof(int16_t));
		if (!plan.tiles) return true;
		if (!lim_setup(cfg_.srate, err) || !lim_out_.ensure(plan.out_pitch * cfg_.n_streams, err)) return false;
		if (!send(lim_frames_.p, frames, (size_t)cfg_.n_streams * sizeof(uint32_t), err)) return false;
		LimParams lp;
		memset((void *)&lp, 0, sizeof lp);
		lp.rows = (const float *)pcm_.p; lp.row_pitch = pcm_f32_ ? pcm_pitch() : 0;
		lp.frames = lim_frames_.p;
		lp.hist = lim_hist_[lim_cur_].p; lp.hist_next = lim_hist_[lim_cur_ ^ 1].p;
		lp.out = lim_out_.p; lp.out_pitch = plan.out_pitch;
		lp.stats = lim_stats_.p;
		lp.base = -(long long)plan.D - 2 * (long long)plan.A;
		lp.n_out = buf_len; lp.run_frames = buf_len; lp.swap_bytes = swap_bytes ? 1 : 0;
		lp.pre_gain = pre_gain; lp.ceiling = ceiling;
		if (!lim_launch(plan, lp, stereo, f32, err)) return false;
		hipLaunchKernelGGL(lim_carry_kernel, dim3((plan.hist_frames * ch + LIM_THREADS - 1) / LIM_THREADS, plan.streams), dim3(LIM_THREADS), 0,
				stream_, lp, ch);
		HIP_OK(hipGetLastError());
		lim_cur_ ^= 1;
		return true;
	}
	bool fetch_limited_async(uint32_t stream, void *dst, size_t bytes, int slot, std::string &err) override {
		slot &= 3;
		use_device();
		if (stream >= cfg_.n_streams || bytes > lim_out_bytes_ || (bytes && !lim_out_.p)) { err = "more bytes than were limited"; return false; }
		if (!fetch_ev_[slot]) HIP_OK(hipEventCreateWithFlags(&fetch_ev_[slot], hipEventDisableTiming));
		if (bytes) {
			const char *src = (const char *)lim_out_.p + lim_out_pitch_ * stream;
			if (host_blocks_.count(dst)) HIP_OK(hipMemcpyAsync(dst, src, bytes, hipMemcpyDeviceToHost, stream_));
			else {
				if (!h_pcm_.ensure((bytes + 1) / 2, err)) return false;
				HIP_OK(hipMemcpyAsync(h_pcm_.p, src, bytes, hipMemcpyDeviceToHost, stream_));
				HIP_OK(hipStreamSynchronize(stream_));
				memcpy(dst, h_pcm_.p, bytes);
			}
		}
		HIP_OK(hipEventRecord(fetch_ev_[slot], stream_));
		return true;
	}
	const float *device_limited_f32(uint32_t stream) override {
		return lim_out_.p && lim_out_f32_ && lim_out_bytes_ && stream < cfg_.n_streams ? (const float *)((const char *)lim_out_.p + lim_out_pitch_ * stream) : nullptr;
	}
	size_t device_limited_pitch() override { return lim_out_.p && lim_out_bytes_ ? lim_out_pitch_ : 0; }
	bool read_limiter_stats(sauengine::LimiterStats *out, bool reset, std::string &err) override {
		use_device();
		if (!lim_stats_.p) { err = "limiting has not begun"; return false; }
		HIP_OK(hipMemcpyAsync(out, lim_stats_.p, (size_t)cfg_.n_streams * sizeof(LimStats), hipMemcpyDeviceToHost, stream_));
		HIP_OK(hipStreamSynchronize(stream_));
		return !reset || lim_clear_stats(lim_stats_.p, cfg_.n_streams, err);
	}
	bool lim_rows_inside(const void *p, size_t pitch, size_t n_rows, size_t row_bytes, const char *what, std::string &err) {
		hipPointerAttribute_t at;
		memset((void *)&at, 0, sizeof at);
		if (hipPointerGetAttributes(&at, p) != hipSuccess) { (void)hipGetLastError(); err = std::string("bad argument: ") + what + " is not device memory"; return false; }
		if (at.type != hipMemoryTypeDevice || at.device != dev_) { err = std::string("bad argument: ") + what + " must be memory of the batch's device"; return false; }
		hipDeviceptr_t base = nullptr;
		size_t span = 0;
		if (hipMemGetAddressRange(&base, &span, (hipDeviceptr_t)p) != hipSuccess) { (void)hipGetLastError(); err = std::string("bad argument: ") + what + " is not device memory"; return false; }
		size_t need = 0;
		const bool wraps = __builtin_mul_overflow(pitch, n_rows - 1, &need) || __builtin_add_overflow(need, row_bytes, &need);
		const size_t ofs = (size_t)((const char *)p - (const char *)base);
		if (wraps || ofs > span || need > span - ofs) { err = std::string("bad argument: ") + what + " reaches beyond its allocation"; return false; }
		return true;
	}
	bool limit_rows(const void *rows, size_t pitch, size_t n_rows, size_t frames, bool stereo, uint32_t srate, float pre_gain, float ceiling,
			void *out_rows, size_t out_pitch, sauengine::LimiterStats *stats_out, std::string &err) override {
		use_device();
		const size_t ch = stereo ? 2 : 1, row_bytes = frames * ch * sizeof(float);
		if (!sauengine::limiter_param_ok(pre_gain) || !sauengine::limiter_param_ok(ceiling) || !srate) { err = "bad argument"; return false; }
		if (!rows || !out_rows || ((uintptr_t)rows & 15u) || (pitch & 15u) || ((uintptr_t)out_rows & 15u) || (out_pitch & 15u)) {
			err = "bad argument: rows, out_rows and their pitches must be multiples of 16"; return false;
		}
		if (frames > 0xffffffffull - 4 * LIM_A_MAX || (n_rows > 1 && (row_bytes > pitch || row_bytes > out_pitch))) {
			err = "bad argument: rows longer than their pitch, or than 32 bits of frames"; return false;
		}
		if (n_rows > LIM_MAX_STREAMS) { err = "bad argument: more than 65535 rows"; return false; }
		for (size_t r = 0; stats_out && r < n_rows; ++r) stats_out[r] = sauengine::LimiterStats{0, 0, 1.0};
		if (!n_rows || !frames) return true;
		if (!lim_rows_inside(rows, pitch, n_rows, row_bytes, "rows", err) || !lim_rows_inside(out_rows, out_pitch, n_rows, row_bytes, "out_rows", err)) return false;
		{
			const uintptr_t a0 = (uintptr_t)rows, a1 = a0 + pitch * (n_rows - 1) + row_bytes, b0 = (uintptr_t)out_rows, b1 = b0 + out_pitch * (n_rows - 1) + row_bytes;
			if (a0 < b1 && b0 < a1) { err = "bad argument: out_rows overlaps rows"; return false; }
		}
		const LimitPlan plan = plan_limit(frames, srate, (uint32_t)ch, n_rows, sizeof(float));
		if (!plan.ok) { err = "bad argument"; return false; }
		if (!lim_setup(srate, err) || !lim_rows_frames_.ensure(n_rows, err) || !lim_rows_stats_.ensure(n_rows, err)) return false;
		const std::vector<uint32_t> fr(n_rows, (uint32_t)frames);
		if (!send(lim_rows_frames_.p, fr.data(), n_rows * sizeof(uint32_t), err) || !lim_clear_stats(lim_rows_stats_.p, n_rows, err)) return false;
		LimParams lp;
		memset((void *)&lp, 0, sizeof lp);
		lp.rows = (const float *)rows; lp.row_pitch = pitch;
		lp.frames = lim_rows_frames_.p;
		lp.out = out_rows; lp.out_pitch = out_pitch;
		lp.stats = lim_rows_stats_.p;
		lp.base = -2 * (long long)plan.A;
		lp.n_out = (uint32_t)frames; lp.run_frames = (uint32_t)frames;
		lp.pre_gain = pre_gain; lp.ceiling = ceiling;
		if (!lim_launch(plan, lp, stereo, true, err)) return false;
		std::vector<LimStats> st(n_rows);
		HIP_OK(hipMemcpyAsync(st.data(), lim_rows_stats_.p, n_rows * sizeof(LimStats), hipMemcpyDeviceToHost, stream_));
		HIP_OK(hipStreamSynchronize(stream_));
		if (stats_out) memcpy((void *)stats_out, st.data(), n_rows * sizeof(LimStats));
		return true;
	}

	class Spectrum : public sauengine::SpectrumMeter {
	public:
		Spectrum(HipBackendImpl *be, size_t n_rows, uint32_t channels, unsigned log2n, uint32_t hop)
			: be_(be), n_(n_rows), ch_(channels), L_(log2n), N_(1u << log2n), bins_((1u << log2n) / 2 + 1), hop_(hop), pos_(n_rows, 0) {}
		~Spectrum() override {
			be_->use_device();
			if (be_->stream_) (void)hipStreamSynchronize(be_->stream_);
		}
		size_t n_rows() const override { return n_; }
		uint32_t channels() const override { return ch_; }
		uint32_t log2n() const override { return L_; }
		bool init(std::string &err) {
			const SpectrumPlan plan = plan_spectrum(L_, hop_, ch_, n_, nullptr);
			if (!plan.ok) { err = "bad argument"; return false; }
			const size_t sums = n_ * plan.sum_pitch, pend = n_ * plan.pend_pitch;
			if (!total_.ensure(sums, err) || !acc_.ensure(sums, err) || !pend_[0].ensure(pend, err) || !pend_[1].ensure(pend, err) ||
			    !desc_.ensure(n_, err) || !win_.ensure(N_, err) || !tw_.ensure(N_, err))
				return false;
			std::vector<double> t(N_);
			if (sauengine::spectrum_window(L_, t.data(), N_) != N_ || !be_->send(win_.p, t.data(), N_ * sizeof(double), err)) return false;
			if (sauengine::spectrum_twiddles(L_, t.data(), N_) != N_ || !be_->send(tw_.p, t.data(), N_ * sizeof(double), err)) return false;
			return clear(err);
		}
		bool clear(std::string &err) {
			HIP_OK(hipMemsetAsync(total_.p, 0, n_ * bins_ * ch_ * sizeof(double), be_->stream_));
			std::fill(pos_.begin(), pos_.end(), 0);
			return true;
		}
		bool feed_into(const void *rows, size_t pitch, const uint32_t *frames, float *sgram, size_t sgram_segs, std::string &err) {
			be_->use_device();
			if (!rows || !frames || ((uintptr_t)rows & 15u) || (pitch & 15u)) { err = "bad argument: rows and pitch_bytes must be multiples of 16"; return false; }
			uint32_t longest = 0;
			for (size_t r = 0; r < n_; ++r) longest = frames[r] > longest ? frames[r] : longest;
			if (!longest) return true;
			const size_t row_bytes = (size_t)longest * ch_ * sizeof(float);
			if (n_ > 1 && row_bytes > pitch) { err = "bad argument: rows longer than their pitch"; return false; }
			if (!be_->lim_rows_inside(rows, pitch, n_, row_bytes, "rows", err)) return false;
			std::vector<SpecRow> d(n_);
			for (size_t r = 0; r < n_; ++r) d[r] = plan_spectrum_row(pos_[r], frames[r], N_, hop_);
			const SpectrumPlan plan = plan_spectrum(L_, hop_, ch_, n_, d.data());
			if (!plan.ok) { err = "bad argument: too many frames for one feed"; return false; }
			if (plan.scratch && !part_.ensure(plan.scratch, err)) return false;
			if (!be_->send(desc_.p, d.data(), n_ * sizeof(SpecRow), err)) return false;
			SpecParams sp;
			memset((void *)&sp, 0, sizeof sp);
			sp.rows = (const float *)rows; sp.row_pitch = pitch; sp.desc = desc_.p;
			sp.pend = pend_[cur_].p; sp.pend_next = pend_[cur_ ^ 1].p; sp.pend_pitch = plan.pend_pitch;
			sp.acc = acc_.p; sp.total = total_.p; sp.part = part_.p;
			sp.sgram = sgram; sp.sgram_segs = sgram_segs;
			sp.win = win_.p; sp.tw = (const double2 *)tw_.p;
			sp.hop = hop_; sp.channels = ch_; sp.max_groups = plan.max_groups;
			hipStream_t st = be_->stream_;
			if (plan.max_groups) {
				const dim3 grid(plan.max_groups, plan.rows, ch_), block(SPEC_THREADS);
				switch (L_) {
				case 8: hipLaunchKernelGGL(spec_segment_kernel<8>, grid, block, plan.lds_bytes, st, sp); break;
				case 9: hipLaunchKernelGGL(spec_segment_kernel<9>, grid, block, plan.lds_bytes, st, sp); break;
				case 10: hipLaunchKernelGGL(spec_segment_kernel<10>, grid, block, plan.lds_bytes, st, sp); break;
				case 11: hipLaunchKernelGGL(spec_segment_kernel<11>, grid, block, plan.lds_bytes, st, sp); break;
				default: hipLaunchKernelGGL(spec_segment_kernel<12>, grid, block, plan.lds_bytes, st, sp); break;
				}
				HIP_OK(hipGetLastError());
				hipLaunchKernelGGL(spec_finish_kernel, dim3((bins_ + SPEC_THREADS - 1) / SPEC_THREADS, plan.rows, ch_), block, 0, st, sp, bins_);
				HIP_OK(hipGetLastError());
			}
			hipLaunchKernelGGL(spec_carry_kernel, dim3((uint32_t)((plan.pend_pitch + SPEC_THREADS - 1) / SPEC_THREADS), plan.rows), dim3(SPEC_THREADS), 0, st, sp);
			HIP_OK(hipGetLastError());
			cur_ ^= 1;
			for (size_t r = 0; r < n_; ++r) pos_[r] += frames[r];
			return true;
		}
		bool feed(const void *rows, size_t pitch, const uint32_t *frames, std::string &err) override {
			return feed_into(rows, pitch, frames, nullptr, 0, err);
		}
		bool read(double *power_out, uint64_t *segments_out, bool reset, std::string &err) override {
			be_->use_device();
			const size_t sums = n_ * bins_ * ch_;
			std::vector<double> acc(sums);
			HIP_OK(hipMemcpyAsync(power_out, total_.p, sums * sizeof(double), hipMemcpyDeviceToHost, be_->stream_));
			HIP_OK(hipMemcpyAsync(acc.data(), acc_.p, sums * sizeof(double), hipMemcpyDeviceToHost, be_->stream_));
			HIP_OK(hipStreamSynchronize(be_->stream_));
			for (size_t r = 0; r < n_; ++r) {
				const uint64_t S = sauengine::spectrum_segments(pos_[r], N_, hop_);
				segments_out[r] = S;
				if (S % SPEC_GROUP)
					for (size_t k = r * bins_ * ch_; k < (r + 1) * bins_ * ch_; ++k) power_out[k] = power_out[k] + acc[k];
			}
			return !reset || clear(err);
		}
	private:
		HipBackendImpl *be_;
		size_t n_;
		uint32_t ch_, L_, N_, bins_, hop_;
		std::vector<uint64_t> pos_;
		DevBuf<double> total_, acc_, part_, win_, tw_;
		DevBuf<float> pend_[2];
		DevBuf<SpecRow> desc_;
		int cur_ = 0;
	};
	sauengine::SpectrumMeter *create_spectrum(size_t n_rows, uint32_t channels, unsigned log2n, uint32_t hop, std::string &err) override {
		use_device();
		if (!sauengine::spectrum_params_ok((int)channels, log2n, hop) || !n_rows) { err = "bad argument"; return nullptr; }
		if (n_rows > SPEC_MAX_ROWS) { err = "bad argument: more than 65535 rows"; return nullptr; }
		Spectrum *m = new Spectrum(this, n_rows, channels, log2n, hop);
		if (!m->init(err)) { delete m; return nullptr; }
		return m;
	}
	bool spectrum_rows(const void *rows, size_t pitch, size_t n_rows, size_t frames, uint32_t channels, unsigned log2n, uint32_t hop,
			double *power_out, uint64_t *segments_out, float *spectrogram_out, size_t spectrogram_cap, std::string &err) override {
		use_device();
		if (!sauengine::spectrum_params_ok((int)channels, log2n, hop) || !n_rows || !power_out || !segments_out) { err = "bad argument"; return false; }
		if (!rows || ((uintptr_t)rows & 15u) || (pitch & 15u)) { err = "bad argument: rows and pitch_bytes must be multiples of 16"; return false; }
		if (n_rows > SPEC_MAX_ROWS || frames > 0xffffffffull) { err = "bad argument: more than 65535 rows, or than 32 bits of frames"; return false; }
		const uint32_t N = 1u << log2n, bins = N / 2 + 1;
		const uint64_t S = sauengine::spectrum_segments(frames, N, hop);
		size_t sg = 0;
		if (spectrogram_out && (__builtin_mul_overflow((size_t)S, (size_t)bins * channels, &sg) || __builtin_mul_overflow(sg, n_rows, &sg) || sg > spectrogram_cap)) {
			err = "bad argument: the spectrogram needs more floats than spectrogram_cap"; return false;
		}
		Spectrum m(this, n_rows, channels, log2n, hop);
		if (!m.init(err)) return false;
		if (spectrogram_out && sg && !spec_gram_.ensure(sg, err)) return false;
		const std::vector<uint32_t> fr(n_rows, (uint32_t)frames);
		if (!m.feed_into(rows, pitch, fr.data(), spectrogram_out && sg ? spec_gram_.p : nullptr, (size_t)S, err)) return false;
		if (!m.read(power_out, segments_out, false, err)) return false;
		if (spectrogram_out && sg) HIP_OK(hipMemcpy(spectrogram_out, spec_gram_.p, sg * sizeof(float), hipMemcpyDeviceToHost));
		return true;
	}

	const int16_t *device_pcm(uint32_t stream) override { return pcm_.p && !pcm_f32_ ? (const int16_t *)pcm_at(stream) : nullptr; }
	const float *device_pcm_f32(uint32_t stream) override { return pcm_.p && pcm_f32_ ? (const float *)pcm_at(stream) : nullptr; }
	size_t device_pcm_pitch() override { return pcm_.p ? pcm_pitch() : 0; }

	bool sync(std::string &err) override {
		use_device();
		HIP_OK(hipStreamSynchronize(stream_));
		arena_used_ = 0;
		return true;
	}
	bool save_state(int slot, std::string &err) override {
		slot &= 3;
		use_device();
		if (!ops_snap_[slot].ensure(ops_.cap, err)) return false;
		HIP_OK(hipMemcpyAsync(ops_snap_[slot].p, ops_.p, ops_.cap * sizeof(DevOp), hipMemcpyDeviceToDevice, stream_));
		return true;
	}
	bool load_state(int slot, std::string &err) override {
		slot &= 3;
		use_device();
		if (!ops_snap_[slot].p || ops_snap_[slot].cap < ops_.cap) { err = "no operator state was saved under this slot"; return false; }
		HIP_OK(hipMemcpyAsync(ops_.p, ops_snap_[slot].p, ops_.cap * sizeof(DevOp), hipMemcpyDeviceToDevice, stream_));
		return true;
	}

	void timing(double *render_ms, double *mix_ms, uint64_t *launches, bool reset) override {
		if (!timing_on_) { timing_on_ = true; }
		(void)hipStreamSynchronize(stream_);
		drain_pairs();
		if (render_ms) *render_ms = acc_ms_[0] + acc_ms_[2];
		if (mix_ms) *mix_ms = acc_ms_[1];
		if (launches) *launches = acc_launches_;
		if (reset) { acc_ms_[0] = acc_ms_[1] = acc_ms_[2] = acc_ms_[3] = 0; acc_launches_ = 0; }
	}

	size_t chain_rows_budget() override { return sauengine::chain_rows_budget(free_hint_, chain_rows_failures_); }
	void *stream_handle() override { return (void *)stream_; }
	bool order_after(HipBackend *before, std::string &err) override {
		HipBackendImpl *o = static_cast<HipBackendImpl *>(before);
		if (o == this) return true;
		if (o->dev_ != dev_) { err = "sauAmd_Batch_order_after: the two batches are on different devices"; return false; }
		use_device();
		if (!after_ev_) HIP_OK(hipEventCreateWithFlags(&after_ev_, hipEventDisableTiming));
		HIP_OK(hipEventRecord(after_ev_, o->stream_));
		after_pending_ = true;
		return true;
	}
	bool wait_for_predecessor(std::string &err) {
		if (!after_pending_) return true;
		after_pending_ = false;
		HIP_OK(hipStreamWaitEvent(stream_, after_ev_, 0));
		return true;
	}
	void set_timing(int level) override { timing_on_ = level > 0; timing_level_ = level; }

	void timing_ex(double *out4, uint64_t *segments, bool reset) override {
		if (!timing_on_) timing_on_ = true;
		(void)hipStreamSynchronize(stream_);
		drain_pairs();
		out4[0] = acc_ms_[2]; out4[1] = acc_ms_[0]; out4[2] = acc_ms_[1]; out4[3] = acc_ms_[3];
		if (segments) *segments = acc_launches_;
		if (reset) { acc_ms_[0] = acc_ms_[1] = acc_ms_[2] = acc_ms_[3] = 0; acc_launches_ = 0; }
	}

	void debug_dump(const char *what, const SegmentDesc &seg, uint32_t block_grid) {
		(void)hipStreamSynchronize(stream_);
		uint32_t n = cfg_.op_count < 8 ? cfg_.op_count : 8;
		std::vector<DevOp> h(n);
		(void)hipMemcpy(h.data(), ops_.p, n * sizeof(DevOp), hipMemcpyDeviceToHost);
		fprintf(stderr, "[sau-amd] %s: seg len %u off %u voices %u slots %u\n", what, seg.len,
				seg.pcm_offset, seg.n_voices, seg.n_slots);
		for (uint32_t v = 0; v < seg.n_voices && v < 4; ++v)
			fprintf(stderr, "  voice %u: run_len %u plan %u+%u ops %u+%u\n", v, seg.voices[v].run_len,
					seg.voices[v].plan_ofs, seg.voices[v].plan_len, seg.voices[v].ops_ofs, seg.voices[v].nops);
		{
			uint32_t wc = 0;
			(void)hipMemcpy(&wc, work_count_.p, 4, hipMemcpyDeviceToHost);
			{
				std::vector<FastInfo> all(seg.n_voices);
				(void)hipMemcpy(all.data(), finfo_.p, all.size() * sizeof(FastInfo), hipMemcpyDeviceToHost);
				uint32_t shown = 0;
				for (size_t v = 0; v < all.size() && shown < 16; ++v)
					if (all[v].bail || all[v].total < seg.voices[v].run_len) {
						uint32_t dbg = 0;
						(void)hipMemcpy(&dbg, repair_.p + v * FAST_REPAIR_WORDS + 1, 4, hipMemcpyDeviceToHost);
						fprintf(stderr, "  voice %zu: fast total %u of %u, bail %u, H %u, seq %u; last unresolved hold: lane p_min+%u row %u step %u group %u (mod 4096)\n", v, all[v].total,
								seg.voices[v].run_len, all[v].bail, all[v].H, all[v].seq, dbg >> 24, (dbg >> 20) & 15, (dbg >> 12) & 255, dbg & 0xfff);
						++shown;
					}
			}
			std::vector<VoiceOut> vi(seg.n_voices < 4 ? seg.n_voices : 4);
			std::vector<uint32_t> fd(vi.size());
			std::vector<FastInfo> fi(vi.size());
			(void)hipMemcpy(vi.data(), set_.vinfo.p, vi.size() * sizeof(VoiceOut), hipMemcpyDeviceToHost);
			(void)hipMemcpy(fd.data(), fdone_.p, fd.size() * 4, hipMemcpyDeviceToHost);
			(void)hipMemcpy(fi.data(), finfo_.p, fi.size() * sizeof(FastInfo), hipMemcpyDeviceToHost);
			float v8[8] = {0};
			(void)hipMemcpy(v8, set_.vout.p, sizeof v8, hipMemcpyDeviceToHost);
			fprintf(stderr, "  work_count %u block_grid %u; row0: %g %g %g %g %g %g\n", wc, block_grid, v8[0], v8[1],
					v8[2], v8[3], v8[4], v8[5]);
			for (size_t v = 0; v < vi.size(); ++v)
				fprintf(stderr, "  vinfo %zu: pan %g has_pan %u valid %u prow %u | fast total %u H %u bail %u done %u\n", v,
						vi[v].pan_const, vi[v].has_pan, vi[v].valid_len, vi[v].pan_row, fi[v].total, fi[v].H,
						fi[v].bail, fd[v]);
		}
		for (uint32_t i = 0; i < n; ++i) {
			const DevOp &o = h[i];
			fprintf(stderr, "  op %u: time %u flags %#x type %u wave %u phase %u prev_s %g fb %g\n", i, o.time,
					o.flags, o.type, o.wave, o.phase, o.prev_s, o.fb_s);
			for (int l = 0; l < 6; ++l)
				if (o.line[l].flags || o.line[l].v0 != 0.f)
					fprintf(stderr, "     line %d: v0 %g vt %g pos %u end %u type %u flags %#x\n", l,
							o.line[l].v0, o.line[l].vt, o.line[l].pos, o.line[l].end, o.line[l].type,
							o.line[l].flags);
		}
	}

private:
	TimedPair *new_pair(int kind) {
		if (timing_level_ == 1 && kind != 2) return nullptr;
		if (n_used_ == events_.size()) {
			if (events_.size() >= 4096) { (void)hipStreamSynchronize(stream_); drain_pairs(); }
			else {
				TimedPair p; p.kind = 0; p.used = false;
				if (hipEventCreate(&p.a) != hipSuccess || hipEventCreate(&p.b) != hipSuccess) return nullptr;
				events_.push_back(p);
			}
		}
		TimedPair *p = &events_[n_used_++];
		p->kind = kind; p->used = true;
		return p;
	}
	void drain_pairs() {
		for (size_t i = 0; i < n_used_; ++i) {
			float ms = 0;
			if (hipEventElapsedTime(&ms, events_[i].a, events_[i].b) == hipSuccess) {
				acc_ms_[events_[i].kind & 3] += ms;
			}
		}
		n_used_ = 0;
	}

	BackendConfig cfg_;
	hipStream_t stream_ = nullptr;
	Tuning tun_;
	DeviceLimits lim_;
	bool debug_ = false;
	bool inner_report_ = false;
	bool inmix_report_ = false;
	uint32_t row_stride_ = 0;
	size_t pcm_row_ = 0;
	bool pcm_f32_ = false;
	WaveConst wconst_[12];
	DevBuf<DevOp> ops_;
	DevBuf<DevOp> ops_snap_[4];
	DevBuf<Step> steps_;
	DevBuf<FastIds> fast_ids_;
	uint32_t n_steps_total_ = 0;
	DevBuf<uint32_t> op_ids_;
	DevBuf<VoiceDesc> voices_;
	struct MixSet {
		DevBuf<float> vout, pan;
		DevBuf<VoiceOut> vinfo;
		DevBuf<MixStream> mstreams;
		uint32_t vout_rows = 0;
		std::vector<MixStream> ms_sent;
		const void *ms_dev = nullptr;
	};
	MixSet set_;
	DevBuf<int16_t> pcm_;
	DevBuf<OpUpdate> recs_;
	const TableSet *tables_ = nullptr;
	PinBuf<int16_t> h_pcm_;
	PinBuf<unsigned char> arena_;
	size_t arena_used_ = 0;
	std::vector<VoiceDesc> voices_sent_;
	std::vector<MixStream> ms_host_;
	const void *voices_dev_ = nullptr;
	std::deque<TimedPair> events_;
	size_t n_used_ = 0;
	bool timing_on_ = false;
	double acc_ms_[4] = {0, 0, 0, 0};
	uint64_t acc_launches_ = 0;
	int timing_level_ = 2;
	DevBuf<FastInfo> finfo_;
	DevBuf<uint32_t> fdone_, worklist_, work_count_;
	DevBuf<float> big_slots_;
	DevBuf<unsigned char> fsteps_, flines_, faux_;
	DevBuf<unsigned long long> scan_;
	DevBuf<uint32_t> pass_flags_, repair_;
	hipEvent_t fetch_ev_[4] = {nullptr, nullptr, nullptr, nullptr};
	int dev_ = 0;
	int want_dev_ = -1;
	std::map<void *, size_t> host_blocks_;
	DevBuf<unsigned long long> look_;
	uint32_t look_epoch_ = 0;
	DevBuf<uint32_t> inc_rows_;
	hipStream_t chain_stream_ = nullptr;
	std::vector<hipEvent_t> chain_ev_;
	DevBuf<float> chain_rows_;
	bool chain_rows_failed_once_ = false;
	unsigned chain_rows_failures_ = 0;
	size_t free_hint_ = 0;
	DevBuf<ChainDesc> chain_desc_;
	DevBuf<unsigned char> fplines_;
	hipEvent_t after_ev_ = nullptr;
	bool after_pending_ = false;
	DevBuf<uint32_t> inmix_ctl_;
	DevBuf<uint32_t> tail_ok_;
	DevBuf<LevelsAcc> lev_acc_, lev_out_;
	DevBuf<LevelsPart> lev_parts_;
	DevBuf<uint32_t> lev_frames_;
	DevBuf<unsigned char> requant_;
	DevBuf<float> decim_hist_;
	DevBuf<double> decim_taps_;
	DevBuf<uint32_t> decim_frames_;
	DevBuf<unsigned char> decim_out_;
	int decim_factor_ = 0;
	bool decim_stereo_ = false, decim_out_f32_ = false;
	LoudSet loud_own_, loud_rows_;
	DevBuf<LoudState> loud_z_, loud_s_;
	DevBuf<double> loud_parts_, loud_taps_;
	DevBuf<uint32_t> loud_tp_parts_, loud_frames_;
	LoudFilter loud_f_;
	LoudMap loud_m_;
	uint32_t loud_rate_ = 0;
	DevBuf<float> lim_hist_[2];
	DevBuf<uint32_t> lim_frames_, lim_rows_frames_, lim_part_cnt_;
	DevBuf<unsigned char> lim_out_;
	DevBuf<LimStats> lim_stats_, lim_rows_stats_;
	DevBuf<double> lim_s_, lim_r_, lim_part_min_, lim_win_, lim_taps_;
	int lim_cur_ = 0;
	uint32_t lim_rate_ = 0;
	bool lim_on_ = false, lim_stereo_ = false, lim_out_f32_ = false;
	size_t lim_out_pitch_ = 0, lim_out_bytes_ = 0;
	DevBuf<float> spec_gram_;
	size_t decim_out_pitch_ = 0, decim_out_bytes_ = 0;
	DevBuf<uint32_t> vlists_;
	size_t chain_alone_lds(size_t need, uint32_t grid) const {
		if (!tun_.chain_alone || grid > lim_.cus || need * 2 > lim_.lds_limit) return need;
		const size_t half = lim_.lds_limit / 2 + 1024;
		return need > half ? need : half;
	}
};

HipBackend *create_hip_backend(std::string &err, int device) {
	if (device_count() <= 0) {
		err = "no HIP device available (this backend has no CPU fallback)";
		return nullptr;
	}
	return new HipBackendImpl(device);
}

}
```

### saugns_amd/csrc/launch_plan.h

```cpp
#ifndef SAU_LAUNCH_PLAN_H
#define SAU_LAUNCH_PLAN_H

#include "engine.h"
#include "sau_dev_math.h"
#include <string.h>

namespace sauplan {

using namespace saudev;
using sauengine::SegmentDesc;

#ifndef FK_GRID
#define FK_GRID 256
#endif
constexpr uint32_t FAST_TAB_BYTES = (uint32_t)(WAVE_LEN * (sizeof(HerpC23) + sizeof(HerpC01))), FAST_TAB_BYTES_WIDE = 65536u;
constexpr uint32_t FAST_MAX_SCAN = 8;
constexpr uint32_t LOOK_LDS_BYTES = FAST_MAX_SCAN * 2 * 64 * sizeof(unsigned long long);
constexpr uint32_t FAST_MAX_LEVELS = 3;
constexpr uint32_t FAST_CUB_ROWS = 4;
constexpr uint32_t FAST_LISTS = 5;
constexpr uint32_t INMIX_NSMALL = 8;
#ifndef SAU_CHAIN_BATCH_FRAMES
#define SAU_CHAIN_BATCH_FRAMES 32
#endif
constexpr uint32_t CHAIN_BATCH = SAU_CHAIN_BATCH_FRAMES;
constexpr uint32_t CHAIN_IO_WORDS = CHAIN_BATCH * 64;
constexpr uint32_t CHAIN_TAB_BYTES = 65536, CHAIN_TAB_C01 = 32768;
constexpr size_t CHAIN_IO_BYTES = (size_t)(2 * 2 + 2) * CHAIN_IO_WORDS * 4;
constexpr size_t MISC_BYTES = 1488;
constexpr size_t BLOCK_TAB_BYTES = (size_t)WAVE_LEN * (sizeof(HerpC23) + sizeof(HerpC01));

struct Tuning {
	int geo = 1;
	uint32_t multi_min = 256;
	uint32_t multi_teams = 16;
	uint32_t fk_grid = 0;
	bool lds_limit_set = false;
	size_t lds_limit = 0;
	bool fast = true;
	bool seq = true;
	bool two_pass = true;
	bool lookback = true;
	bool inc_rows = true;
	uint32_t fast_rows = 8;
	uint32_t look_rows = 8;
	uint32_t look_min_voices = 1;
	bool look_no_lds = false, look_withhold = false, look_spread = false;
	bool wide_tabs = true;
	bool wide_look = true;
	uint32_t more_rows = 12;
	bool repair = true;
	bool analyze_lds = true;
	bool chain = true;
	bool chain_inline = true;
	bool chain_early = true;
	uint32_t chain_chunks = 0;
	uint32_t chain_chunk_frames = 16384;
	bool short_last_chunk = true;
	bool chain_alone = false;
	bool lean = true;
	uint32_t lean_rows = 6;
	bool dyn = true;
	uint32_t dyn_groups = 12;
	uint32_t dyn_floor = 24;
	uint32_t dyn_min_tasks = 2;
	bool xcd_queues = true;
	bool inmix = true;
	uint32_t inmix_min_voices = 64;
	uint32_t inmix_min_steps = 2;
	bool inmix_taper = false;
	uint32_t inmix_at = 13;
	bool inmix_dry = false;
	bool inner = true;
	bool lanemajor = true;
	bool duo = true;
	uint32_t duo_lw = 0, duo_prio = 0;
	bool tailmix = false;
	bool mix_few = true;
	bool early_mix = true;
	bool mix64 = true;
	bool poison = false;
};

inline Tuning tuning_from_env(const char *(*env)(const char *)) {
	Tuning t;
	auto off = [&](const char *name) { return env(name) == nullptr; };
	auto num = [&](const char *name, uint32_t &v) { if (const char *s = env(name)) v = (uint32_t)atoi(s); };
	auto at_least_1 = [&](const char *name, uint32_t &v) { if (const char *s = env(name)) { const int n = atoi(s); v = n >= 1 ? (uint32_t)n : 1u; } };
	const char *wt = env("SAU_AMD_GEOMETRY");
	t.geo = (wt && !strcmp(wt, "8x2")) ? 0 : 1;
	if (const char *mm = env("SAU_AMD_MULTI_MIN")) t.multi_min = (uint32_t)atol(mm);
	if (const char *mt = env("SAU_AMD_MULTI_TEAMS")) t.multi_teams = atoi(mt) == 8 ? 8u : 16u;
	if (const char *fg = env("SAU_AMD_FK_GRID")) { const int n = atoi(fg); if (n >= 1 && n <= (int)FK_GRID) t.fk_grid = (uint32_t)n; }
	if (const char *ll = env("SAU_AMD_LDS_LIMIT")) { t.lds_limit_set = true; t.lds_limit = (size_t)atol(ll); }
	t.fast = off("SAU_AMD_NO_FAST");
	t.seq = off("SAU_AMD_NO_SEQ");
	t.two_pass = off("SAU_AMD_NO_TWO_PASS");
	t.lookback = off("SAU_AMD_NO_LOOKBACK");
	t.inc_rows = off("SAU_AMD_NO_INC_ROWS");
	if (const char *fr = env("SAU_AMD_FAST_ROWS")) {
		const int r = atoi(fr);
		t.fast_rows = r >= 8 ? 8 : r >= 6 ? 6 : r >= 5 ? 5 : r >= 4 ? 4 : 2;
	}
	num("SAU_AMD_LOOK_ROWS", t.look_rows);
	num("SAU_AMD_LOOK_MIN_VOICES", t.look_min_voices);
	t.look_no_lds = !off("SAU_AMD_LOOK_NO_LDS");
	t.look_withhold = !off("SAU_AMD_LOOK_WITHHOLD");
	t.look_spread = !off("SAU_AMD_LOOK_SPREAD");
	t.wide_tabs = off("SAU_AMD_NO_WIDE_TABS");
	t.wide_look = off("SAU_AMD_NO_WIDE_LOOK");
	num("SAU_AMD_MORE_ROWS", t.more_rows);
	t.repair = off("SAU_AMD_NO_REPAIR");
	t.analyze_lds = off("SAU_AMD_ANALYZE_NO_LDS");
	t.chain = off("SAU_AMD_NO_CHAIN");
	t.chain_inline = off("SAU_AMD_NO_CHAIN_INLINE");
	t.chain_early = off("SAU_AMD_NO_EARLY_CHAINS");
	if (const char *cc = env("SAU_AMD_CHAIN_CHUNKS")) {
		const int n = atoi(cc);
		t.chain_chunks = n >= 32 ? 32 : n >= 1 ? (uint32_t)n : 1;
	}
	if (const char *cf = env("SAU_AMD_CHAIN_CHUNK_FRAMES")) { const int n = atoi(cf); if (n >= 4096) t.chain_chunk_frames = (uint32_t)n; }
	t.short_last_chunk = off("SAU_AMD_NO_SHORT_LAST_CHUNK");
	if (const char *ca = env("SAU_AMD_CHAIN_ALONE")) t.chain_alone = atoi(ca) != 0;
	t.lean = off("SAU_AMD_NO_LEAN");
	num("SAU_AMD_LEAN_ROWS", t.lean_rows);
	t.dyn = off("SAU_AMD_NO_DYN");
	at_least_1("SAU_AMD_DYN_GROUPS", t.dyn_groups);
	at_least_1("SAU_AMD_DYN_FLOOR", t.dyn_floor);
	at_least_1("SAU_AMD_DYN_MIN_TASKS", t.dyn_min_tasks);
	t.xcd_queues = off("SAU_AMD_NO_XCD_QUEUES");
	t.inmix = off("SAU_AMD_NO_INMIX");
	num("SAU_AMD_INMIX_MIN_VOICES", t.inmix_min_voices);
	num("SAU_AMD_INMIX_MIN_STEPS", t.inmix_min_steps);
	t.inmix_taper = !off("SAU_AMD_INMIX_TAPER");
	if (const char *ia = env("SAU_AMD_INMIX_AT")) t.inmix_at = (uint32_t)atoi(ia) & 15u;
	t.inmix_dry = !off("SAU_AMD_INMIX_DRY");
	t.inner = off("SAU_AMD_NO_INNER");
	t.lanemajor = off("SAU_AMD_NO_LANEMAJOR");
	t.duo = off("SAU_AMD_NO_DUO");
	if (const char *lw = env("SAU_AMD_DUO_LW")) t.duo_lw = (uint32_t)atoi(lw) & 15u;
	if (const char *pr = env("SAU_AMD_DUO_PRIO")) t.duo_prio = (uint32_t)atoi(pr) & 7u;
	t.tailmix = !off("SAU_AMD_TAILMIX");
	t.mix_few = off("SAU_AMD_NO_MIX_FEW");
	t.early_mix = off("SAU_AMD_NO_EARLY_MIX");
	t.mix64 = off("SAU_AMD_NO_MIX64");
	t.poison = !off("SAU_AMD_POISON");
	return t;
}

struct DeviceLimits {
	size_t lds_limit = 160 * 1024;
	uint32_t fk_grid = FK_GRID;
	uint32_t cus = 256;
	bool eight_xcds = true;
};
inline DeviceLimits device_limits(size_t lds_per_cu, uint32_t cus, const Tuning &t) {
	DeviceLimits d;
	d.cus = cus;
	d.eight_xcds = cus == 256;
	d.fk_grid = t.fk_grid ? t.fk_grid : cus < FK_GRID ? cus : FK_GRID;
	d.lds_limit = t.lds_limit_set ? t.lds_limit : lds_per_cu > 160 * 1024 ? (size_t)160 * 1024 : lds_per_cu;
	return d;
}

struct PlanInputs {
	uint32_t row_stride = 0;
	size_t pcm_row = 0;
	size_t chain_budget = 0;
	bool f32 = false;
	uint32_t max_write = 0;
	uint32_t max_rows = 0;
};

struct TableMap {
	uint32_t n = 0;
	int8_t tab_of_wave[12];
	uint8_t wave_of_tab[12];
};
inline TableMap map_tables(uint64_t wave_mask, size_t max_tabs) {
	TableMap m;
	memset(m.wave_of_tab, 0, sizeof m.wave_of_tab);
	for (int wv = 0; wv < 12; ++wv) {
		m.tab_of_wave[wv] = -1;
		if (((wave_mask >> wv) & 1) && m.n < max_tabs) {
			m.tab_of_wave[wv] = (int8_t)m.n;
			m.wave_of_tab[m.n] = (uint8_t)wv;
			++m.n;
		}
	}
	return m;
}
inline size_t tabs_that_fit(size_t limit, size_t fixed, size_t tab_bytes) { return fixed > limit ? 0 : (limit - fixed) / tab_bytes; }
inline uint32_t n_waves_used(uint64_t wave_mask) { return (uint32_t)__builtin_popcountll(wave_mask & 0xffffffffull); }

inline size_t buf_area(uint32_t n_bufs, uint32_t rows, uint32_t fmax_steps) {
	return (size_t)n_bufs * 64 * rows * sizeof(float) + (size_t)fmax_steps * sizeof(unsigned long long);
}
inline bool fits_lds(const DeviceLimits &d, size_t n_tabs, size_t tab_bytes, size_t area, size_t extra = 0) {
	return n_tabs * tab_bytes + 16 * area + extra + 1024 <= d.lds_limit;
}
inline uint32_t row_groups(uint32_t len, uint32_t rows) { return (len + (60 * rows) - 1) / (60 * rows); }
inline uint32_t wave_grid(unsigned long long waves, uint32_t max_grid) {
	const unsigned long long g = (waves + 15) / 16;
	return g > max_grid ? max_grid : g < 1 ? 1u : (uint32_t)g;
}
inline uint32_t group_grid(uint32_t n_voices, uint32_t groups, uint32_t max_grid) {
	return wave_grid((unsigned long long)n_voices * (groups < 64 ? groups : 64), max_grid);
}
inline uint32_t fewer_rows(uint32_t t) { return t > 6 ? 6u : t > 5 ? 5u : t > 4 ? 4u : 2u; }
inline uint32_t rows_at_most(uint32_t r) { return r >= 8 ? 8u : r >= 6 ? 6u : r >= 5 ? 5u : r >= 4 ? 4u : 2u; }

struct BlockLoopPlan {
	bool ok = true;
	uint32_t W = 4, T = 4, V = 1;
	bool HB = false;
	size_t team_bytes = 0, lds = 0;
	TableMap tabs;
	uint32_t grid(const SegmentDesc &seg, bool use_fast) const {
		const bool all = seg.maybe_block || !use_fast;
		if (V > 1) {
			const uint32_t full = (seg.n_voices + V - 1) / V;
			return all ? (full < 512 ? full : 512) : 2;
		}
		return all ? (seg.n_voices < 1024 ? seg.n_voices : 1024) : 16;
	}
};
inline BlockLoopPlan plan_block_loop(const SegmentDesc &seg, const Tuning &tun, const DeviceLimits &dev) {
	BlockLoopPlan p;
	p.W = tun.geo ? 4 : 8; p.T = tun.geo ? 4 : 2;
	auto team_size = [&](uint32_t w, uint32_t t) {
		size_t b = p.HB ? MISC_BYTES + 64
			: (size_t)w * 64 * t * sizeof(float) * seg.n_slots + (size_t)seg.max_ops * sizeof(DevOp) +
			MISC_BYTES + (size_t)seg.max_steps * sizeof(Step) + 64;
		return (b + 15) & ~(size_t)15;
	};
	if (tun.multi_min && seg.n_voices >= tun.multi_min && (seg.serial || tun.multi_min == 1)) {
		const size_t need_tab = seg.wave_mask ? BLOCK_TAB_BYTES : 0;
		const uint32_t mt = tun.multi_teams;
		for (uint32_t t : {4u, 3u, 2u, 1u})
			if (mt * team_size(1, t) + need_tab <= dev.lds_limit) { p.W = 1; p.T = t; p.V = mt; break; }
	}
	if (p.V == 1 && team_size(p.W, p.T) > dev.lds_limit) { p.W = 1; p.T = 1; }
	if (p.V == 1 && p.W == 1 && team_size(1, 1) > dev.lds_limit) p.HB = true;
	p.team_bytes = team_size(p.W, p.T);
	const size_t fixed = p.team_bytes * p.V;
	if (fixed > dev.lds_limit) { p.ok = false; return p; }
	size_t budget = dev.lds_limit / 2 > fixed ? dev.lds_limit / 2 - fixed : 0;
	if (p.V > 1) budget = dev.lds_limit - fixed;
	if (budget < BLOCK_TAB_BYTES && dev.lds_limit - fixed >= BLOCK_TAB_BYTES) budget = BLOCK_TAB_BYTES;
	p.tabs = map_tables(seg.wave_mask, budget / BLOCK_TAB_BYTES);
	p.lds = p.tabs.n * BLOCK_TAB_BYTES + fixed;
	return p;
}

struct ChainChunks {
	uint32_t n = 1;
	uint32_t cb[34];
	bool short_last = false;
};
inline ChainChunks chain_chunk_bounds(uint32_t len, const Tuning &tun) {
	ChainChunks k;
	uint32_t n = tun.chain_chunks ? tun.chain_chunks : (len + tun.chain_chunk_frames - 1) / tun.chain_chunk_frames;
	if (n > 32) n = 32;
	while (n > 1 && len / n < 4096) --n;
	if (n < 1) n = 1;
	k.short_last = !tun.chain_chunks && tun.short_last_chunk && n >= 4 && n < 32 && len > 8 * 4096u;
	const uint32_t tail = k.short_last ? 4096u : 0u;
	const uint32_t body = tail ? (len - tail) & ~255u : len;
	const uint32_t clen0 = ((body + n - 1) / n + 255) & ~255u;
	for (uint32_t c = 0; c <= n; ++c) k.cb[c] = (unsigned long long)c * clen0 < body ? c * clen0 : body;
	if (tail) { ++n; k.cb[n] = len; }
	uint32_t m = 0;
	for (uint32_t c = 0; c < n; ++c)
		if (k.cb[c + 1] > k.cb[c]) { k.cb[m] = k.cb[c]; ++m; k.cb[m] = k.cb[c + 1]; }
	if (m) n = m;
	k.n = n;
	return k;
}

struct Tasks { uint32_t dyn_chunks = 0, dyn_static = 0, dyn_small = 0; };
inline uint32_t task_groups(const SegmentDesc &seg, const Tuning &tun) {
	const uint32_t S = seg.max_steps ? seg.max_steps : 1;
	uint32_t G = tun.dyn_groups;
	if (G * S < tun.dyn_floor) G = (tun.dyn_floor + S - 1) / S;
	return G;
}
inline Tasks plan_tasks(const SegmentDesc &seg, const Tuning &tun, uint32_t n_groups, uint32_t grid) {
	Tasks q;
	const uint32_t waves = grid * 16;
	const uint32_t G = task_groups(seg, tun);
	const uint32_t k_dyn = (n_groups + G - 1) / G;
	if (tun.dyn && (unsigned long long)seg.n_voices * k_dyn >= (unsigned long long)tun.dyn_min_tasks * waves) {
		q.dyn_chunks = k_dyn ? k_dyn : 1;
		q.dyn_static = 0;
	} else {
		uint32_t k = waves / seg.n_voices;
		if (k > n_groups) k = n_groups;
		q.dyn_chunks = k ? k : 1;
		q.dyn_static = 1;
// ... 84 lines not shown
	if (tun.seq && seg.may_scan && FT > 4 && !p.look_split) FT = 4;
	if (p.look_split && FT > tun.look_rows) FT = rows_at_most(tun.look_rows);
	p.seq_ok = tun.seq && seg.may_scan;
	p.n_fast = p.seq_ok && seg.n_fast_full > seg.n_fast ? seg.n_fast_full : seg.n_fast;
	p.n_fast_cf = seg.n_fast;
	p.n_want = n_waves_used(seg.wave_mask);
	auto area_of = [&](uint32_t t) { return buf_area(p.n_fast, t, p.fmax_steps); };
	const size_t look_lds = p.look_split ? LOOK_LDS_BYTES : 0;
	while (FT > 2 && !fits_lds(dev, seg.wave_mask ? 1 : 0, FAST_TAB_BYTES, area_of(FT), look_lds)) FT = fewer_rows(FT);
	{
		uint32_t t = FT;
		while (t > 4 && !fits_lds(dev, p.n_want, FAST_TAB_BYTES, area_of(t), look_lds)) t = fewer_rows(t);
		if (fits_lds(dev, p.n_want, FAST_TAB_BYTES, area_of(t), look_lds)) FT = t;
	}
	p.use_fast = tun.fast && fits_lds(dev, 0, 0, area_of(FT), look_lds);
	p.rows = FT;
	p.rows_multi = FT > 4 && p.seq_ok ? 4 : FT;
	p.tabs = map_tables(seg.wave_mask, p.use_fast ? tabs_that_fit(dev.lds_limit, 16 * area_of(FT) + look_lds + 1024, FAST_TAB_BYTES) : 0);
	const uint32_t ft = p.tabs.n;
	const bool all_wide_ok = tun.wide_tabs && tun.more_rows && ft > 0 && ft == p.n_want && seg.max_steps >= 2;
	if (p.use_fast && !p.seq_ok && all_wide_ok && FT == 8)
		for (uint32_t t : {12u, 10u})
			if (t <= tun.more_rows && fits_lds(dev, ft, FAST_TAB_BYTES_WIDE, area_of(t))) { p.rows = p.rows_multi = t; break; }
	p.split_cf = p.use_fast && p.seq_ok && p.look_split;
	auto area_cf = [&](uint32_t t) { return buf_area(p.n_fast_cf, t, p.fmax_steps); };
	p.rows_cf = 2;
	if (p.split_cf) {
		for (uint32_t t : {8u, 6u, 5u, 4u})
			if (t <= tun.fast_rows && fits_lds(dev, ft, FAST_TAB_BYTES, area_cf(t))) { p.rows_cf = t; break; }
		if (p.rows_cf == 8 && all_wide_ok)
			for (uint32_t t : {12u, 10u})
				if (t <= tun.more_rows && fits_lds(dev, ft, FAST_TAB_BYTES_WIDE, area_cf(t))) { p.rows_cf = t; break; }
	}
	p.cub_ok = p.use_fast && seg.maybe_cub && fits_lds(dev, ft, FAST_TAB_BYTES, area_cf(FAST_CUB_ROWS)) &&
		(!p.look_split || fits_lds(dev, ft, FAST_TAB_BYTES, area_of(FAST_CUB_ROWS), LOOK_LDS_BYTES));
	p.rows_lean = 4;
	for (uint32_t t : {6u, 5u})
		if (t <= tun.fast_rows && t <= tun.lean_rows && fits_lds(dev, ft, FAST_TAB_BYTES, area_of(t))) { p.rows_lean = t; break; }
	p.main_build = !p.seq_ok ? 0 : p.look_split ? 2 : 1;
	auto wide_fits = [&](uint32_t rows, size_t area) {
		return tun.wide_tabs && (rows == 8 || rows == 6 || rows == 10 || rows == 12) && ft > 0 && ft == p.n_want && seg.max_steps >= 2 &&
			fits_lds(dev, ft, FAST_TAB_BYTES_WIDE, area);
	};
	p.wide_cf = p.main_build == 2 ? wide_fits(p.rows_cf, area_cf(p.rows_cf)) : p.main_build == 0 && wide_fits(p.rows, area_of(p.rows));
	p.wide_look = tun.wide_tabs && tun.wide_look && p.rows == 8 && ft > 0 && ft == p.n_want &&
		fits_lds(dev, ft, FAST_TAB_BYTES_WIDE, area_of(p.rows), LOOK_LDS_BYTES);
	p.sum_levels = seg.sum_levels >= FAST_MAX_LEVELS ? FAST_MAX_LEVELS : 2u;
}

inline void plan_sums(FastPlan &p, const SegmentDesc &seg, const Tuning &tun, const DeviceLimits &dev) {
	if (p.seq_ok && tun.two_pass) {
		p.scan_groups = seg.len / (32 * p.rows_multi) + 2;
		p.scan = !p.look_split || seg.n_chain_rows;
		p.look = p.look_split && seg.n_look_rows;
	}
	if (p.look) {
		const uint32_t groups = row_groups(seg.len, p.rows);
		unsigned long long wpv = ((unsigned long long)dev.fk_grid * 16) / seg.n_voices;
		if (wpv > 64) wpv = 64;
		if (wpv > groups) wpv = groups;
		if (wpv < 1) wpv = 1;
		auto is_inside = [&](unsigned long long w) { return w <= 16 && (16 % w) == 0 && !tun.look_no_lds; };
		p.look_words = (size_t)seg.n_look_rows * 2 * p.scan_groups;
		p.look_words_real = p.look_words * sizeof(unsigned long long) <= ((size_t)1 << 30);
		if (!p.look_words_real && !is_inside(wpv) && !tun.look_no_lds)
			wpv = wpv > 16 ? 16 : wpv > 8 ? 8 : wpv > 4 ? 4 : 2;
		p.look_wpv = (uint32_t)wpv;
		p.look_inside = !p.look_words_real && is_inside(wpv);
	}
	p.inc_stride = (seg.len + 63) & ~63u;
	p.inc_rows = tun.inc_rows && p.use_fast && p.scan && seg.n_inc_rows && seg.len <= sauengine::CHAIN_SEG &&
		(size_t)seg.n_inc_rows * 2 * p.inc_stride * sizeof(uint32_t) <= ((size_t)1 << 30);
}

inline void plan_chains(FastPlan &p, const SegmentDesc &seg, const Tuning &tun, const DeviceLimits &dev, const PlanInputs &in) {
	p.chains = tun.chain && p.use_fast && p.scan && seg.serial && seg.n_chain_rows &&
		seg.len <= sauengine::chain_seg_frames(seg.n_chain_rows, in.chain_budget);
	p.chain_stride = (seg.len + 63) & ~63u;
	p.ctabs = map_tables(seg.wave_mask, tabs_that_fit(dev.lds_limit, CHAIN_IO_BYTES + 1024, CHAIN_TAB_BYTES));
	p.lean_on = p.chains && tun.lean &&
		fits_lds(dev, p.tabs.n, FAST_TAB_BYTES, buf_area(p.n_fast, p.rows_lean, p.fmax_steps));
	p.chain_grid = (seg.n_chain_slots + 63) / 64;
	if (p.chains) p.chunks = chain_chunk_bounds(seg.len, tun);
	p.pass_grid = p.chunks.n > 1 && p.grid + p.chain_grid > dev.fk_grid ? (dev.fk_grid > p.chain_grid + 32 ? dev.fk_grid - p.chain_grid : 32) : p.grid;
	p.early_mix = tun.early_mix && in.max_write && !p.cub_ok && !(tun.mix_few && in.max_rows <= 8 && seg.n_streams >= 8);
}

inline void plan_split(FastPlan &p, const SegmentDesc &seg, const Tuning &tun, const DeviceLimits &dev, const PlanInputs &in) {
	const uint32_t ft = p.tabs.n;
	p.tailmix = p.look && p.rows == 8 && tun.tailmix && !in.f32 && in.max_write && !p.cub_ok && seg.len < (1u << 30) &&
		tun.mix_few && in.max_rows <= 8 && seg.n_streams >= 8 && (seg.pcm_offset & 3u) == 0 && (in.pcm_row & 3u) == 0;
	p.groups_cf = row_groups(seg.len, p.rows_cf);
	p.grid_cf = group_grid(seg.n_voices, p.groups_cf, dev.fk_grid);
	p.duo = tun.duo && p.look && p.look_words_real && p.rows == 8 && p.rows_cf == 8 && !p.cub_ok && !p.tailmix &&
		!p.wide_look && !p.wide_cf && fits_lds(dev, ft, FAST_TAB_BYTES, buf_area(p.n_fast, p.rows, p.fmax_steps), LOOK_LDS_BYTES);
	p.tasks_cf = plan_tasks(seg, tun, p.groups_cf, p.duo ? (dev.fk_grid + 1) / 2 : p.grid_cf);
	p.look_wpv_flags = (tun.look_no_lds ? 1u : 0u) | (tun.look_withhold ? 2u : 0u) | (tun.look_spread ? 4u : 0u);
	if (p.duo) p.look_wpv_flags |= (tun.duo_lw << 8) | (tun.duo_prio << 12);
	p.grid_look = wave_grid((unsigned long long)seg.n_voices * (p.look_words_real ? (p.groups < 64 ? p.groups : 64) : p.look_wpv), dev.fk_grid);
}

inline void plan_closed_form(FastPlan &p, const SegmentDesc &seg, const Tuning &tun, const DeviceLimits &dev, const PlanInputs &in) {
	if (p.main_build == 0) p.tasks = plan_tasks(seg, tun, p.groups, p.grid);
	p.queues = tun.xcd_queues && dev.eight_xcds && p.main_build == 0 && !p.tasks.dyn_static && p.tasks.dyn_chunks >= 16 && !p.cub_ok;
	if (p.queues) {
		p.inmix_flags = 64u;
		if (tun.inmix_taper) {
			const uint32_t G = task_groups(seg, tun);
			const uint32_t small = G / 4 ? G / 4 : 1;
			if (p.groups >= 32 * G + INMIX_NSMALL * small) {
				p.tasks.dyn_small = small;
				p.tasks.dyn_chunks = (p.groups - INMIX_NSMALL * small + G - 1) / G + INMIX_NSMALL;
			}
		}
		p.div = magic_div(seg.n_voices);
		p.inmix = tun.inmix && !in.f32 && seg.n_streams == 1 && in.max_write && seg.n_voices >= tun.inmix_min_voices &&
			seg.max_steps >= tun.inmix_min_steps && in.row_stride < (1u << 24);
		if (p.inmix)
			p.inmix_flags = 64u | 32u | (seg.stereo ? 1u : 0u) | (seg.swap_bytes ? 2u : 0u) | (tun.inmix_dry ? 4u : 0u) | ((tun.inmix_at & 15u) << 8);
	}
	if (tun.inner && p.main_build == 0 && p.wide_cf && p.rows == 12 && p.tasks.dyn_chunks >= 3)
		p.inner = tun.lanemajor && p.n_fast == 1 ? INNER_LANE_MAJOR : INNER_ROW_MAJOR;
	p.grid_edge = wave_grid(2ull * seg.n_voices, dev.fk_grid);
}

inline FastPlan plan_fast(const SegmentDesc &seg, const Tuning &tun, const DeviceLimits &dev, const PlanInputs &in) {
	FastPlan p;
	plan_rows(p, seg, tun, dev);
	plan_sums(p, seg, tun, dev);
	p.groups = row_groups(seg.len, p.rows);
	p.grid = group_grid(seg.n_voices, p.groups, dev.fk_grid);
	plan_chains(p, seg, tun, dev, in);
	if (p.use_fast && p.main_build == 2) plan_split(p, seg, tun, dev, in);
	if (p.use_fast && !p.scan) plan_closed_form(p, seg, tun, dev, in);
	const uint32_t g4 = row_groups(seg.len, FAST_CUB_ROWS);
	p.grid_cub = group_grid(seg.n_voices, g4, dev.fk_grid);
	p.tasks_cub = static_tasks(seg, g4, p.grid_cub);
	p.rows_repair = p.main_build == 2 ? p.rows_cf : p.rows;
	p.grid_repair = wave_grid(seg.n_voices, 64);
	return p;
}

inline Mixer plan_mixer(const SegmentDesc &seg, const Tuning &tun, const PlanInputs &in, size_t pcm_pitch, bool inmix_live,
		uint32_t early_blocks) {
	if (!in.max_write) return MIX_NONE;
	const bool few = tun.mix_few && in.max_rows <= 8 && seg.n_streams >= 8;
	const bool few_f32_aligned = (pcm_pitch & 15u) == 0 && (seg.pcm_offset & (seg.stereo ? 1u : 3u)) == 0;
	if (in.f32) return few && few_f32_aligned ? MIX_FEW_F32 : MIX_F32;
	if (few && (seg.pcm_offset & 3u) == 0 && (in.pcm_row & 3u) == 0) return MIX_FEW;
	if (inmix_live && !early_blocks && tun.mix64) return MIX_64;
	return MIX_256;
}

constexpr uint32_t LEVELS_THREADS = 256;
constexpr uint32_t LEVELS_SWEEP_F32 = LEVELS_THREADS * 4, LEVELS_SWEEP_S16 = LEVELS_THREADS * 8;
constexpr uint32_t LEVELS_WG_SAMPLES = 16384;
static_assert(LEVELS_WG_SAMPLES % LEVELS_SWEEP_S16 == 0 && LEVELS_WG_SAMPLES % LEVELS_SWEEP_F32 == 0, "a block is whole sweeps (and begins on an even sample, on 16 bytes)");
constexpr uint32_t LEVELS_MAX_ROWS = 65535;
struct LevelsPlan {
	bool ok = false;
	uint32_t blocks = 0;
	uint32_t rows = 0;
	uint32_t finish_grid = 0;
	size_t parts = 0;
};
inline LevelsPlan plan_levels(uint64_t max_frames, uint32_t channels, size_t n_rows) {
	LevelsPlan p;
	const uint64_t samples = max_frames * channels;
	const uint64_t blocks = (samples + LEVELS_WG_SAMPLES - 1) / LEVELS_WG_SAMPLES;
	if (n_rows > LEVELS_MAX_ROWS || blocks > 0x7fffffffull || max_frames > (~(uint64_t)0 >> 2)) return p;
	p.ok = true;
	p.blocks = (uint32_t)blocks;
	p.rows = (uint32_t)n_rows;
	p.finish_grid = (uint32_t)((n_rows + 63) / 64);
	p.parts = (size_t)n_rows * (size_t)blocks;
	return p;
}

constexpr uint32_t DECIM_THREADS = 64, DECIM_PER_LANE = 4;
constexpr uint32_t DECIM_TILE = 256;
static_assert(DECIM_TILE == DECIM_THREADS * DECIM_PER_LANE, "a lane's frames are DECIM_THREADS apart");
constexpr uint32_t DECIM_HALF = (uint32_t)sauengine::DECIM_HALF;
constexpr uint32_t DECIM_SPAN_Q = DECIM_TILE + 2 * DECIM_HALF;
constexpr uint32_t DECIM_CARRY_THREADS = 256;
constexpr uint32_t DECIM_MAX_STREAMS = 65535;
struct DecimPlan {
	bool ok = false;
	uint32_t tiles = 0;
	uint32_t streams = 0;
	uint32_t taps = 0;
	uint32_t hist_floats = 0;
	uint32_t lds_bytes = 0;
	size_t out_pitch = 0;
};
inline DecimPlan plan_decimate(uint64_t buf_len, int factor, uint32_t channels, size_t n_streams, size_t sample_bytes) {
	DecimPlan p;
	if ((factor != 2 && factor != 4 && factor != 8) || (channels != 1 && channels != 2) || n_streams > DECIM_MAX_STREAMS) return p;
	const uint64_t tiles = (buf_len + DECIM_TILE - 1) / DECIM_TILE;
	if (tiles > 0x7fffffffull || buf_len * (uint64_t)factor > 0xffffffffull) return p;
	p.ok = true;
	p.tiles = (uint32_t)tiles;
	p.streams = (uint32_t)n_streams;
	p.taps = 2 * DECIM_HALF * (uint32_t)factor + 1;
	p.hist_floats = (p.taps - 1) * channels;
	p.lds_bytes = DECIM_SPAN_Q * (uint32_t)factor * channels * (uint32_t)sizeof(float);
	p.out_pitch = ((size_t)buf_len * channels * sample_bytes + 255) & ~(size_t)255;
	return p;
}
static_assert(2 * DECIM_HALF * 8 * 2 <= DECIM_CARRY_THREADS * 4, "decimate_carry_kernel: a stream's longest history, four floats per thread");

constexpr uint32_t LOUD_CHUNK = 256;
constexpr uint32_t LOUD_THREADS = 64, LOUD_WG_CHUNKS = LOUD_THREADS, LOUD_SUB = 32;
static_assert(LOUD_CHUNK % LOUD_SUB == 0 && LOUD_SUB % 4 == 0, "a chunk is whole sub-tiles of whole 16-byte vectors");
constexpr uint32_t LOUD_MIN_RATE = sauengine::LOUD_MIN_RATE;
constexpr uint32_t TP_FACTOR = 4, TP_HALF = 16, TP_TAPS = 2 * TP_HALF * TP_FACTOR + 1;
constexpr uint32_t TP_HIST = 2 * TP_HALF - 1, TP_LEAD = 2 * TP_HALF;
static_assert(TP_TAPS == sauengine::TP_TAPS && TP_LEAD == sauengine::TP_LEAD, "engine.h: the host's copies");
constexpr uint32_t TP_THREADS = 64, TP_PER_LANE = 4, TP_TILE = TP_THREADS * TP_PER_LANE;
constexpr uint32_t LOUD_MAX_ROWS = 65535;
struct LoudPlan {
	bool ok = false;
	uint32_t hop = 0;
	uint32_t chunks = 0;
	uint32_t chunk_grid = 0;
	uint32_t tiles = 0;
	uint32_t rows = 0;
	uint32_t lane_grid = 0;
	uint32_t lds_bytes = 0;
};
inline LoudPlan plan_loudness(uint64_t max_frames, uint32_t channels, size_t n_rows, uint32_t srate) {
	LoudPlan p;
	if ((channels != 1 && channels != 2) || srate < LOUD_MIN_RATE || n_rows > LOUD_MAX_ROWS || max_frames > 0xffffffffull) return p;
	p.ok = true;
	p.hop = srate / 10;
	p.chunks = (uint32_t)((max_frames + LOUD_CHUNK - 1) / LOUD_CHUNK);
	p.chunk_grid = (p.chunks + LOUD_WG_CHUNKS - 1) / LOUD_WG_CHUNKS;
	p.tiles = (uint32_t)((max_frames + TP_TILE - 1) / TP_TILE);
	p.rows = (uint32_t)n_rows;
	p.lane_grid = (uint32_t)((n_rows * 2 + 63) / 64);
	p.lds_bytes = LOUD_WG_CHUNKS * (LOUD_SUB * channels + channels) * (uint32_t)sizeof(float);
	return p;
}

constexpr uint32_t LIM_A_MIN = sauengine::LIM_A_MIN, LIM_A_MAX = sauengine::LIM_A_MAX;
constexpr uint32_t LIM_THREADS = 256, LIM_PER_LANE = 2, LIM_TILE = LIM_THREADS * LIM_PER_LANE;
constexpr uint32_t LIM_ENV_TILE = LIM_THREADS;
constexpr uint32_t LIM_SPAN_MAX = LIM_TILE + 4 * LIM_A_MAX;
constexpr uint32_t LIM_SPAN_PER_THREAD = (LIM_SPAN_MAX + LIM_THREADS - 1) / LIM_THREADS;
static_assert(LIM_SPAN_MAX * sizeof(double) <= 65536, "lim_gain_kernel's span is static LDS");
constexpr uint32_t LIM_MAX_STREAMS = 65535;
struct LimitPlan {
	bool ok = false;
	uint32_t A = 0, D = 0;
	uint32_t taps = 0;
	uint32_t hist_frames = 0;
	uint32_t env_n = 0;
	uint32_t env_tiles = 0;
	uint32_t tiles = 0;
	uint32_t streams = 0;
	uint32_t span = 0;
	size_t scratch_pitch = 0;
	size_t out_pitch = 0;
};
inline LimitPlan plan_limit(uint64_t frames, uint32_t srate, uint32_t channels, size_t n_streams, size_t sample_bytes) {
	LimitPlan p;
	if (!srate || (channels != 1 && channels != 2) || n_streams > LIM_MAX_STREAMS || frames > 0xffffffffull - 4 * LIM_A_MAX) return p;
	p.ok = true;
	p.A = srate / 200 < LIM_A_MIN ? LIM_A_MIN : srate / 200 > LIM_A_MAX ? LIM_A_MAX : srate / 200;
	p.D = 2 * p.A + 16;
	p.taps = 2 * p.A + 1;
	p.hist_frames = 4 * p.A + 32;
	p.streams = (uint32_t)n_streams;
	p.span = LIM_TILE + 4 * p.A;
	if (frames) {
		p.env_n = (uint32_t)frames + 4 * p.A;
		p.env_tiles = (p.env_n + LIM_ENV_TILE - 1) / LIM_ENV_TILE;
		p.tiles = (uint32_t)((frames + LIM_TILE - 1) / LIM_TILE);
	}
	p.scratch_pitch = ((size_t)p.env_n + 31) & ~(size_t)31;
	p.out_pitch = ((size_t)frames * channels * sample_bytes + 255) & ~(size_t)255;
	return p;
}

constexpr uint32_t SPEC_THREADS = 256, SPEC_GROUP = sauengine::SPEC_GROUP;
constexpr uint32_t SPEC_MAX_ROWS = 65535;
constexpr uint64_t SPEC_MAX_SCRATCH = 1ull << 27;
struct SpecRow {
	uint64_t seg0;
	uint32_t n_seg;
	uint32_t pend;
	uint32_t pend_next;
	uint32_t acc_cnt;
	uint32_t n_groups;
	uint32_t n_complete;
};
static_assert(sizeof(SpecRow) == 32, "SpecRow is uploaded as it stands");
inline SpecRow plan_spectrum_row(uint64_t pos, uint32_t frames, uint32_t N, uint32_t hop) {
	SpecRow r;
	const uint64_t s0 = sauengine::spectrum_segments(pos, N, hop), s1 = sauengine::spectrum_segments(pos + frames, N, hop);
	r.seg0 = s0;
	r.n_seg = (uint32_t)(s1 - s0);
	r.pend = (uint32_t)(pos - s0 * hop);
	r.pend_next = (uint32_t)(pos + frames - s1 * hop);
	r.acc_cnt = (uint32_t)(s0 % SPEC_GROUP);
	r.n_groups = s1 > s0 ? (uint32_t)((s1 - 1) / SPEC_GROUP - s0 / SPEC_GROUP + 1) : 0;
	r.n_complete = s1 > s0 ? (uint32_t)(s1 / SPEC_GROUP - s0 / SPEC_GROUP) : 0;
// ... 32 lines not shown
```

Baseline: 247.5 million.

## Run final mixer on a separate stream overlapping next segment's render

```diff
diff --git a/__graft_entry__.py b/__graft_entry__.py
--- a/__graft_entry__.py
+++ b/__graft_entry__.py
@@ -18,6 +18,7 @@
     subprocess.check_call(["make", "-s", "-C", os.path.join(ROOT, "tests", "hooks_limiter")])
     subprocess.check_call(["make", "-s", "-C", os.path.join(ROOT, "tests", "hooks_spectrum")])
     subprocess.check_call(["make", "-s", "-C", os.path.join(ROOT, "tests", "hooks_plan")])
+    subprocess.check_call(["make", "-s", "-C", os.path.join(ROOT, "tests", "hooks_overlap")])
     subprocess.check_call(["make", "-s", "-C", os.path.join(ROOT, "oracle"), "oracle"])
     subprocess.check_call(["make", "-s", "-C", os.path.join(ROOT, "oracle"), "ref"])
     subprocess.check_call(["make", "-s", "-C", os.path.join(ROOT, "oracle"), "hosts"])
diff --git a/saugns_amd/build.py b/saugns_amd/build.py
--- a/saugns_amd/build.py
+++ b/saugns_amd/build.py
@@ -7,7 +7,7 @@
 LIB = os.path.join(HERE, "libsaugns_amd.so")
 SOURCES = ["capi.cpp", "engine.cpp", "plan.cpp", "tables.cpp", "program_io.cpp", "sndout.cpp", "bank_builder.cpp",
            "hip_backend.hip"]
-HEADERS = ["engine.h", "hip_backend.h", "capi_internal.h", "sau_dev_math.h", "sau_dev_ops.h", "launch_plan.h",
+HEADERS = ["engine.h", "hip_backend.h", "capi_internal.h", "sau_dev_math.h", "sau_dev_ops.h", "launch_plan.h", "mix_overlap.h",
            "k_common.h", "k_wave_scan.h", "k_block_loop.h", "k_fast_types.h", "k_analyze.h", "k_decode.h", "k_fast_voice.h", "k_fast_group.h", "k_fast_group_lm.h",
            "k_chain.h", "k_finish.h", "k_levels.h", "k_decimate.h", "k_loudness.h", "k_limiter.h", "k_spectrum.h",
            "sau_dev_types.h", "../../include/sau_abi.h", "../../include/saugns_amd.h"]
diff --git a/saugns_amd/csrc/hip_backend.hip b/saugns_amd/csrc/hip_backend.hip
--- a/saugns_amd/csrc/hip_backend.hip
+++ b/saugns_amd/csrc/hip_backend.hip
@@ -305,9 +305,42 @@
 	explicit HipBackendImpl(int device = -1) : want_dev_(device) {}
 	void use_device() { (void)hipSetDevice(dev_); }
 
+	bool wait_mixer(uint64_t t, const char *where, std::string &err) {
+		if (!t) return true;
+		hipEvent_t done = mix_done_[MixOverlapTracker::slot(t)];
+		if (overlap_report_) {
+			const bool was_done = hipEventQuery(done) == hipSuccess;
+			report_waits_ += std::string(" ") + where + ":" + std::to_string(t) + (was_done ? ":done" : ":busy");
+		}
+		HIP_OK(hipStreamWaitEvent(stream_, done, 0));
+		return true;
+	}
+	bool join_mixer(const char *where, std::string &err) { return wait_mixer(mixo_.join(), where, err); }
+	void join_mixer_quiet(const char *where) { std::string e; (void)join_mixer(where, e); }
+	bool ensure_mix_stream(std::string &err) {
+		if (mix_ready_) return true;
+		if (!mix_stream_) mix_stream_ = StreamPool::get().take(dev_, 1);
+		if (!mix_stream_) {
+			int lo = 0, hi = 0;
+			(void)hipDeviceGetStreamPriorityRange(&lo, &hi);
+			HIP_OK(hipStreamCreateWithPriority(&mix_stream_, hipStreamNonBlocking, hi));
+		}
+		for (uint32_t i = 0; i < MIXO_RING; ++i) {
+			if (!mix_fork_[i]) HIP_OK(hipEventCreateWithFlags(&mix_fork_[i], hipEventDisableTiming));
+			if (!mix_done_[i]) HIP_OK(hipEventCreateWithFlags(&mix_done_[i], hipEventDisableTiming));
+		}
+		mix_ready_ = true;
+		return true;
+	}
+
 	~HipBackendImpl() override {
 		use_device();
-		if (stream_) (void)hipStreamSynchronize(stream_);
+		if (stream_) { join_mixer_quiet("destroy"); (void)hipStreamSynchronize(stream_); }
+		if (mix_stream_) { (void)hipStreamSynchronize(mix_stream_); StreamPool::get().give(dev_, mix_stream_, 1); }
+		for (uint32_t i = 0; i < MIXO_RING; ++i) {
+			if (mix_fork_[i]) (void)hipEventDestroy(mix_fork_[i]);
+			if (mix_done_[i]) (void)hipEventDestroy(mix_done_[i]);
+		}
 		if (chain_stream_) { (void)hipStreamSynchronize(chain_stream_); StreamPool::get().give(dev_, chain_stream_, 1); }
 		for (hipEvent_t e : chain_ev_) (void)hipEventDestroy(e);
 		for (int i = 0; i < 4; ++i) if (fetch_ev_[i]) (void)hipEventDestroy(fetch_ev_[i]);
@@ -349,6 +382,7 @@
 		debug_ = getenv("SAU_AMD_DEBUG") != nullptr;
 		inmix_report_ = tune_env("SAU_AMD_INMIX_REPORT") != nullptr;
 		inner_report_ = tune_env("SAU_AMD_INNER_REPORT") != nullptr;
+		overlap_report_ = tune_env("SAU_AMD_OVERLAP_REPORT") != nullptr;
 		if (!ops_.ensure(cfg.op_count ? cfg.op_count : 1, err)) return false;
 		HIP_OK(hipMemsetAsync(ops_.p, 0, ops_.cap * sizeof(DevOp), stream_));
 		tables_ = shared_tables(cfg.piluts, cfg.wconst, err);
@@ -359,11 +393,12 @@
 
 	bool reserve_frames(uint32_t max_frames, bool , std::string &err) override {
 		use_device();
+		if (!join_mixer("reserve_frames", err)) return false;
 		HIP_OK(hipStreamSynchronize(stream_));
 		row_stride_ = (max_frames + 63) & ~63u;
 		pcm_row_ = (size_t)row_stride_ * 2;
 		if (!pcm_.ensure(pcm_row_ * cfg_.n_streams * pcm_units(), err)) return false;
-		set_.vout_rows = 0;
+		sets_[0].vout_rows = sets_[1].vout_rows = 0;
 		return true;
 	}
 
@@ -374,6 +409,7 @@
 		use_device();
 		const bool f32 = fmt == sauengine::SF_F32;
 		if (f32 == pcm_f32_) return true;
+		if (!join_mixer("set_format", err)) return false;
 		pcm_f32_ = f32;
 		if (pcm_row_ && !pcm_.ensure(pcm_row_ * cfg_.n_streams * pcm_units(), err)) { pcm_f32_ = !f32; return false; }
 		return true;
@@ -426,6 +462,7 @@
 	bool poison_run(uint32_t frames, bool stereo, std::string &err) override {
 		(void)frames; (void)stereo;
 		use_device();
+		if (!join_mixer("poison_run", err)) return false;
 		if (pcm_.p) HIP_OK(hipMemsetD16Async((hipDeviceptr_t)pcm_.p, 0x5a5a, pcm_row_ * cfg_.n_streams * pcm_units(), stream_));
 		return true;
 	}
@@ -434,6 +471,7 @@
 			std::string &err) override {
 		use_device();
 		if (!pcm_.p || !n_streams || !n_frames) return true;
+		if (!join_mixer("zero_pcm", err)) return false;
 		const size_t fb = (stereo ? 2 : 1) * pcm_units() * sizeof(int16_t);
 		char *at = pcm_at(first_stream) + (size_t)first_frame * fb;
 		if (n_streams == 1) HIP_OK(hipMemsetAsync(at, 0, (size_t)n_frames * fb, stream_));
@@ -456,6 +494,9 @@
 		bool inmix_live = false;
 		uint32_t early_mixed_blocks = 0;
 		uint32_t block_grid = 1;
+		MixOverlap mode = MIXO_OFF;
+		uint32_t set = 0;
+		uint32_t block = 0;
 		TimedPair *tf = nullptr;
 		explicit Job(const SegmentDesc &s) : seg(s) { memset(&rp, 0, sizeof rp); memset(&fp, 0, sizeof fp); }
 	};
@@ -469,10 +510,15 @@
 		if (j.in.f32 != pcm_f32_) { err = "a segment of another sample format than the run announced"; return false; }
 		if (j.in.f32 && seg.swap_bytes) { err = "float32 samples are not byte-swapped"; return false; }
 		j.in.row_stride = row_stride_; j.in.pcm_row = pcm_row_; j.in.chain_budget = chain_rows_budget();
+		for (uint32_t s = 0; s < seg.n_streams; ++s) {
+			if (seg.streams[s].write_len > j.in.max_write) j.in.max_write = seg.streams[s].write_len;
+			if (seg.streams[s].n_voices > j.in.max_rows) j.in.max_rows = seg.streams[s].n_voices;
+		}
+		j.fk = plan_fast(seg, tun_, lim_, j.in);
+		if (!begin_overlap(j, err)) return false;
 		j.bl = plan_block_loop(seg, tun_, lim_);
 		if (!j.bl.ok) { err = "voice too large for one workgroup's LDS (block buffers + operator states)"; return false; }
 		if (!ensure_rows(j, err) || !upload_descriptors(j, err)) return false;
-		j.fk = plan_fast(seg, tun_, lim_, j.in);
 		if (!prepare_fast(j, err) || !prepare_chains(j, err)) return false;
 		fill_tables(j);
 		if (!launch_analyze(j, err)) return false;
@@ -490,26 +536,65 @@
 		return launch_mixer(j, err);
 	}
 
+	bool begin_overlap(Job &j, std::string &err) {
+		const SegmentDesc &seg = j.seg;
+		j.set = mixo_.begin_segment();
+		const size_t rows_bytes = ((size_t)seg.n_voices + seg.n_pan_rows) * row_stride_ * sizeof(float);
+		j.mode = plan_mix_overlap(tun_, j.in, j.fk, rows_bytes, second_refused_);
+		if (j.mode == MIXO_ALTERNATE && j.set == 1 && !second_rows(j)) j.mode = MIXO_SHARED;
+		j.block = MixOverlapTracker::block_of(j.mode, j.set);
+		if (j.mode != MIXO_OFF && !ensure_mix_stream(err)) return false;
+		return wait_mixer(mixo_.before_records(j.set), "records", err);
+	}
+	bool second_rows(Job &j) {
+		const SegmentDesc &seg = j.seg;
+		MixSet &R = sets_[1];
+		const size_t nv = (size_t)seg.n_voices * row_stride_, np = (size_t)seg.n_pan_rows * row_stride_;
+		if (R.vout.p && seg.n_voices <= R.vout_rows && np <= R.pan.cap) return true;
+		std::string why = "refused by SAU_AMD_MIX_OVERLAP_FAIL";
+		bool ok = !tun_.mix_overlap_fail;
+		if (ok && (seg.n_voices > R.vout_rows || !R.vout.p)) {
+			if (R.vout.p) {
+				join_mixer_quiet("second_rows");
+				(void)hipStreamSynchronize(stream_);
+			}
+			ok = R.vout.ensure(nv, why);
+			if (ok) R.vout_rows = seg.n_voices;
+		}
+		if (ok && np) ok = R.pan.ensure(np, why);
+		if (!ok) {
+			second_refused_ = true;
+			if (R.vout.p || R.pan.p) { join_mixer_quiet("second_rows"); (void)hipStreamSynchronize(stream_); (void)hipStreamSynchronize(mix_stream_ ? mix_stream_ : stream_); }
+			R.vout.release(); R.pan.release(); R.vout_rows = 0;
+			if (debug_) fprintf(stderr, "saugns_amd: no second block of %zu bytes of voice rows (%s): the final mixer's two sets share one\n", nv * sizeof(float), why.c_str());
+		}
+		return ok;
+	}
+	bool rows_hazard(Job &j, std::string &err) { return wait_mixer(mixo_.before_rows(j.block), "rows", err); }
+	bool pcm_hazard(std::string &err) { return wait_mixer(mixo_.before_pcm(), "pcm", err); }
+
 	bool ensure_rows(Job &j, std::string &err) {
 		const SegmentDesc &seg = j.seg;
-		MixSet &S = set_;
+		MixSet &S = sets_[j.set], &R = sets_[j.block];
 		if (!voices_.ensure(seg.n_voices, err) || !S.vinfo.ensure(seg.n_voices, err)) return false;
-		if (seg.n_voices > S.vout_rows || !S.vout.p) {
+		if (seg.n_voices > R.vout_rows || !R.vout.p) {
+			if (!join_mixer("ensure_rows", err)) return false;
 			HIP_OK(hipStreamSynchronize(stream_));
-			if (!S.vout.ensure((size_t)seg.n_voices * row_stride_, err)) return false;
-			S.vout_rows = seg.n_voices;
-		}
-		if (seg.n_pan_rows && !S.pan.ensure((size_t)seg.n_pan_rows * row_stride_, err)) return false;
+			if (!R.vout.ensure((size_t)seg.n_voices * row_stride_, err)) return false;
+			R.vout_rows = seg.n_voices;
+		}
+		if (seg.n_pan_rows && !R.pan.ensure((size_t)seg.n_pan_rows * row_stride_, err)) return false;
 		if (tun_.poison) {
-			HIP_OK(hipMemsetD32Async((hipDeviceptr_t)S.vout.p, 0x3ea5a5a5, (size_t)seg.n_voices * row_stride_, stream_));
-			if (seg.n_pan_rows) HIP_OK(hipMemsetD32Async((hipDeviceptr_t)S.pan.p, 0x3ea5a5a5, (size_t)seg.n_pan_rows * row_stride_, stream_));
+			if (!wait_mixer(mixo_.before_rows(j.block), "poison", err)) return false;
+			HIP_OK(hipMemsetD32Async((hipDeviceptr_t)R.vout.p, 0x3ea5a5a5, (size_t)seg.n_voices * row_stride_, stream_));
+			if (seg.n_pan_rows) HIP_OK(hipMemsetD32Async((hipDeviceptr_t)R.pan.p, 0x3ea5a5a5, (size_t)seg.n_pan_rows * row_stride_, stream_));
 		}
 		return S.mstreams.ensure(seg.n_streams, err);
 	}
 
 	bool upload_descriptors(Job &j, std::string &err) {
 		const SegmentDesc &seg = j.seg;
-		MixSet &S = set_;
+		MixSet &S = sets_[j.set];
 		ms_host_.resize(seg.n_streams);
 		for (uint32_t s = 0; s < seg.n_streams; ++s) {
 			MixStream &m = ms_host_[s];
@@ -519,8 +604,6 @@
 			m.amp_scale = seg.streams[s].amp_scale;
 			m.write_len = seg.streams[s].write_len;
 			m.pcm = (int16_t *)pcm_at(s);
-			if (m.write_len > j.in.max_write) j.in.max_write = m.write_len;
-			if (m.n_rows > j.in.max_rows) j.in.max_rows = m.n_rows;
 		}
 		const bool same_voices = voices_sent_.size() == seg.n_voices && voices_dev_ == voices_.p &&
 			memcmp(voices_sent_.data(), seg.voices, seg.n_voices * sizeof(VoiceDesc)) == 0;
@@ -543,22 +626,22 @@
 		const SegmentDesc &seg = j.seg;
 		const FastPlan &k = j.fk;
 		FastParams &fp = j.fp;
-		MixSet &S = set_;
+		MixSet &S = sets_[j.set], &R = sets_[j.block];
 		const size_t n_lists = (size_t)FAST_LISTS * seg.n_voices * k.fmax_steps;
 		if (!finfo_.ensure(seg.n_voices, err) || !fdone_.ensure(seg.n_voices, err) ||
-		    !worklist_.ensure(seg.n_voices, err) || !work_count_.ensure(4, err) ||
+		    !worklist_.ensure(seg.n_voices, err) || !S.work_count.ensure(4, err) ||
 		    !fsteps_.ensure(n_lists * sizeof(FastStep), err) || !flines_.ensure(n_lists * sizeof(FastLine), err) ||
 		    !faux_.ensure(n_lists * sizeof(FastAux), err)) return false;
 		fp.voices = voices_.p; fp.steps = steps_.p; fp.fast_ids = fast_ids_.p; fp.op_ids = op_ids_.p; fp.ops = ops_.p;
-		fp.vout = S.vout.p; fp.pan = S.pan.p; fp.info = finfo_.p; fp.fast_done = fdone_.p;
-		fp.worklist = worklist_.p; fp.work_count = work_count_.p; fp.vinfo = S.vinfo.p;
+		fp.vout = R.vout.p; fp.pan = R.pan.p; fp.info = finfo_.p; fp.fast_done = fdone_.p;
+		fp.worklist = worklist_.p; fp.work_count = S.work_count.p; fp.vinfo = S.vinfo.p;
 		fp.g_c23 = tables_->c23; fp.g_c01 = tables_->c01; fp.fsteps = (FastStep *)fsteps_.p; fp.flines = (FastLine *)flines_.p; fp.faux = (FastAux *)faux_.p;
 		fp.row_stride = row_stride_; fp.n_voices = seg.n_voices; fp.n_fast = k.n_fast;
 		fp.seq_enable = k.seq_ok ? 1u : 0u; fp.ids_full_ofs = n_steps_total_;
 		fp.scan = nullptr; fp.scan_groups = k.scan_groups; fp.mode = 0;
 		if (tun_.xcd_queues && lim_.eight_xcds) {
-			if (!inmix_ctl_.ensure(INMIX_WORDS, err)) return false;
-			fp.inmix = inmix_ctl_.p;
+			if (!S.inmix_ctl.ensure(INMIX_WORDS, err)) return false;
+			fp.inmix = S.inmix_ctl.p;
 		}
 		if (k.scan) {
 			if (!scan_.ensure((size_t)seg.n_voices * FAST_MAX_SCAN * k.scan_groups, err)) return false;
@@ -665,6 +748,7 @@
 
 	bool launch_build(Job &j, std::string &err, int build, uint32_t rows, uint32_t grid, const FastParams *prm = nullptr, bool cf = false,
 			bool wide = false) {
+		if (!rows_hazard(j, err)) return false;
 		if (build == 1 && rows > 4) rows = 4;
 		if (build == 3) rows = rows < 5 ? 4 : rows > 6 ? 6 : rows;
 		const void *fn = fast_kernel_fn(build, rows, (wide ? FK_WIDE : 0u) | (build == 2 && j.tail_live ? FK_TAIL : 0u));
@@ -698,14 +782,17 @@
 		const SegmentDesc &seg = j.seg;
 		const FastPlan &k = j.fk;
 		FastParams &fp = j.fp, &cfp = j.cfp;
+		MixSet &S = sets_[j.set];
 		if (k.tailmix) {
-			if (!tail_ok_.ensure(seg.n_streams, err)) return false;
-			fp.tail_ok = tail_ok_.p; fp.inmix_stream = set_.mstreams.p;
+			if (!S.tail_ok.ensure(seg.n_streams, err)) return false;
+			fp.tail_ok = S.tail_ok.p; fp.inmix_stream = S.mstreams.p;
 			fp.tail_flags = (seg.stereo ? 1u : 0u) | (seg.swap_bytes ? 2u : 0u);
 			fp.tail_pcm_offset = seg.pcm_offset;
 			hipLaunchKernelGGL(tailmix_kernel, dim3((seg.n_streams + 63) / 64), dim3(64), 0, stream_, fp, seg.n_streams);
 			j.tail_live = true;
 		}
+		if (!rows_hazard(j, err)) return false;
+		if (j.tail_live && !pcm_hazard(err)) return false;
 		cfp = fp;
 		cfp.n_fast = k.n_fast_cf; cfp.rows = k.rows_cf; cfp.mode = 0; cfp.only_multi = 0;
 		if (getenv("SAU_AMD_DEBUG_DUO"))
@@ -747,6 +834,7 @@
 	bool launch_sums_and_chains(Job &j, std::string &err) {
 		const SegmentDesc &seg = j.seg;
 		FastParams &fp = j.fp;
+		if (!rows_hazard(j, err)) return false;
 		if (fp.chain_rows && fp.chain_early_ok && !launch_early_chains(j, err)) return false;
 		for (uint32_t pass = 1; pass <= fp.sum_levels && (!fp.look || seg.n_chain_rows); ++pass) {
 			launch_fast(j, err, pass);
@@ -828,7 +916,8 @@
 			if (k.early_mix && c + 1 < n_chunks && cb[c + 1] > 512) {
 				const uint32_t hi = (cb[c + 1] - 512) / 256;
 				if (hi > mixed_blocks) {
-					MixParams mp = mix_params(j.seg, set_);
+					if (!pcm_hazard(err)) return false;
+					MixParams mp = mix_params(j);
 					mp.blk_lo = mixed_blocks; mp.blk_hi = hi;
 					TimedPair *tm = timing_on_ ? new_pair(1) : nullptr;
 					if (tm) (void)hipEventRecord(tm->a, stream_);
@@ -852,7 +941,7 @@
 			fp.inmix_flags = k.inmix_flags;
 			fp.inmix_div_s = k.div.s; fp.inmix_div_m = k.div.m;
 			if (k.inmix) {
-				fp.inmix_stream = set_.mstreams.p;
+				fp.inmix_stream = sets_[j.set].mstreams.p;
 				fp.inmix_pcm_offset = seg.pcm_offset;
 				hipLaunchKernelGGL(premix_kernel, dim3((seg.n_voices + 63) / 64), dim3(64), 0, stream_, fp);
 				j.inmix_live = true;
@@ -868,10 +957,12 @@
 			fp.mode = 0;
 			void *iargs[] = {(void *)&fp};
 			if (!raise_lds_attr(ik, lds, dev_, err)) return false;
+			if (fp.inmix_flags && !pcm_hazard(err)) return false;
 			HIP_OK(hipLaunchKernel(ik, dim3(k.grid), dim3(1024), iargs, lds, stream_));
 			if (inner_report_) fprintf(stderr, "[sau-amd] inner: %s, %u voices\n", lm ? "lane-major" : "row-major", seg.n_voices);
 		} else {
 			if (inner_report_) fprintf(stderr, "[sau-amd] inner: none (rows %u, wide %d, chunks %u), %u voices\n", k.rows, k.wide_cf ? 1 : 0, fp.dyn_chunks, seg.n_voices);
+			if (fp.inmix_flags && (!rows_hazard(j, err) || !pcm_hazard(err))) return false;
 			launch_fast(j, err, 0);
 		}
 		fp.dyn_chunks = 0; fp.inmix_flags = 0; fp.dyn_small = 0;
@@ -888,6 +979,7 @@
 		const void *ck = fast_kernel_fn(0, FAST_CUB_ROWS, FK_CUB);
 		if (!raise_lds_attr(ck, qlds, dev_, err)) return false;
 		void *qargs[] = {(void *)&q};
+		if (!rows_hazard(j, err)) return false;
 		HIP_OK(hipLaunchKernel(ck, dim3(k.grid_cub), dim3(1024), qargs, qlds, stream_));
 		return true;
 	}
@@ -905,6 +997,7 @@
 		if (!raise_lds_attr(rk, rlds, dev_, err)) return false;
 		j.fp.mode = 0;
 		void *rargs[] = {(void *)&rpar};
+		if (!rows_hazard(j, err)) return false;
 		HIP_OK(hipLaunchKernel(rk, dim3(k.grid_repair), dim3(1024), rargs, rlds, stream_));
 		return true;
 	}
@@ -942,13 +1035,13 @@
 		memcpy(rp.tab_of_wave, b.tabs.tab_of_wave, sizeof rp.tab_of_wave);
 		memcpy(rp.wave_of_tab, b.tabs.wave_of_tab, sizeof rp.wave_of_tab);
 		rp.voices = voices_.p; rp.steps = steps_.p; rp.op_ids = op_ids_.p; rp.ops = ops_.p;
-		rp.vout = set_.vout.p; rp.pan = set_.pan.p; rp.vinfo = set_.vinfo.p;
+		rp.vout = sets_[j.block].vout.p; rp.pan = sets_[j.block].pan.p; rp.vinfo = sets_[j.set].vinfo.p;
 		rp.g_c23 = tables_->c23; rp.g_c01 = tables_->c01;
 		rp.row_stride = row_stride_; rp.seg_len = seg.len;
 		rp.n_slots = seg.n_slots; rp.max_ops = seg.max_ops; rp.n_tabs = b.tabs.n;
 		rp.max_steps = seg.max_steps; rp.n_main = seg.n_main;
 		memcpy(rp.wc, wconst_, sizeof wconst_);
-		rp.fast_done = fdone_.p; rp.worklist = worklist_.p; rp.work_count = work_count_.p;
+		rp.fast_done = fdone_.p; rp.worklist = worklist_.p; rp.work_count = sets_[j.set].work_count.p;
 		j.block_grid = b.grid(seg, j.fk.use_fast);
 		if (b.HB) {
 			const size_t stride = ((size_t)seg.n_slots * 64 * sizeof(float) + (size_t)seg.max_ops * sizeof(DevOp) +
@@ -958,6 +1051,7 @@
 			rp.big_slots = big_slots_.p; rp.big_stride = (uint32_t)stride;
 		}
 		if (!wait_for_predecessor(err)) return false;
+		if (!rows_hazard(j, err)) return false;
 		TimedPair *tp = timing_on_ ? new_pair(0) : nullptr;
 		if (tp) (void)hipEventRecord(tp->a, stream_);
 		const void *fn = render_kernel_fn(b.W, b.T, b.V, b.HB);
@@ -967,7 +1061,7 @@
 		HIP_OK(hipLaunchKernel(fn, dim3(j.block_grid), dim3(64 * b.W * b.V), args, b.lds, stream_));
 		HIP_OK(hipGetLastError());
 		if (tp) (void)hipEventRecord(tp->b, stream_);
-		if (debug_) debug_dump("after render", seg, j.block_grid);
+		if (debug_) debug_dump("after render", j);
 		return true;
 	}
 
@@ -975,24 +1069,48 @@
 		const SegmentDesc &seg = j.seg;
 		const uint32_t max_write = j.in.max_write;
 		const Mixer which = plan_mixer(seg, tun_, j.in, pcm_pitch(), j.inmix_live, j.early_mixed_blocks);
-		if (which == MIX_NONE) return true;
-		MixParams mp = mix_params(seg, set_);
+		if (which == MIX_NONE) { report_overlap(j, 0, false); return true; }
+		MixSet &S = sets_[j.set];
+		MixParams mp = mix_params(j);
 		mp.early_blocks = j.early_mixed_blocks;
-		mp.inmix = j.inmix_live ? inmix_ctl_.p : nullptr;
-		mp.tail_ok = j.tail_live ? tail_ok_.p : nullptr;
+		mp.inmix = j.inmix_live ? S.inmix_ctl.p : nullptr;
+		mp.tail_ok = j.tail_live ? S.tail_ok.p : nullptr;
 		TimedPair *tm = timing_on_ ? new_pair(1) : nullptr;
-		if (tm) (void)hipEventRecord(tm->a, stream_);
+		hipStream_t ms = stream_;
+		const uint64_t ticket = j.mode == MIXO_OFF ? 0 : mixo_.next_ticket();
+		if (!ticket) {
+			if (!wait_mixer(mixo_.before_pcm(), "mixer", err)) return false;
+		} else {
+			hipEvent_t fork = mix_fork_[MixOverlapTracker::slot(ticket)];
+			HIP_OK(hipEventRecord(fork, stream_));
+			HIP_OK(hipStreamWaitEvent(mix_stream_, fork, 0));
+			ms = mix_stream_;
+		}
+		if (tm) (void)hipEventRecord(tm->a, ms);
 		switch (which) {
-		case MIX_FEW_F32: hipLaunchKernelGGL(mix_few_kernel_f32, dim3((max_write + 1023) / 1024, seg.n_streams), dim3(256), 0, stream_, mp); break;
-		case MIX_F32: hipLaunchKernelGGL(mix_kernel_f32, dim3((max_write + 255) / 256, seg.n_streams), dim3(256), 0, stream_, mp); break;
-		case MIX_FEW: hipLaunchKernelGGL(mix_few_kernel, dim3((max_write + 1023) / 1024, seg.n_streams), dim3(256), 0, stream_, mp); break;
-		case MIX_64: hipLaunchKernelGGL(mix_kernel64, dim3((max_write + 63) / 64, seg.n_streams), dim3(64), 0, stream_, mp); break;
-		default: hipLaunchKernelGGL(mix_kernel, dim3((max_write + 255) / 256, seg.n_streams), dim3(256), 0, stream_, mp); break;
+		case MIX_FEW_F32: hipLaunchKernelGGL(mix_few_kernel_f32, dim3((max_write + 1023) / 1024, seg.n_streams), dim3(256), 0, ms, mp); break;
+		case MIX_F32: hipLaunchKernelGGL(mix_kernel_f32, dim3((max_write + 255) / 256, seg.n_streams), dim3(256), 0, ms, mp); break;
+		case MIX_FEW: hipLaunchKernelGGL(mix_few_kernel, dim3((max_write + 1023) / 1024, seg.n_streams), dim3(256), 0, ms, mp); break;
+		case MIX_64: hipLaunchKernelGGL(mix_kernel64, dim3((max_write + 63) / 64, seg.n_streams), dim3(64), 0, ms, mp); break;
+		default: hipLaunchKernelGGL(mix_kernel, dim3((max_write + 255) / 256, seg.n_streams), dim3(256), 0, ms, mp); break;
 		}
 		HIP_OK(hipGetLastError());
-		if (tm) (void)hipEventRecord(tm->b, stream_);
+		if (tm) (void)hipEventRecord(tm->b, ms);
+		if (ticket) {
+			HIP_OK(hipEventRecord(mix_done_[MixOverlapTracker::slot(ticket)], mix_stream_));
+			if (mixo_.mixer_launched(j.set, j.block) != ticket) { err = "internal error: the final mixer's ticket changed under its launch"; return false; }
+		}
+		report_overlap(j, ticket, true);
 		if (mp.inmix && inmix_report_) report_inmix(mp, seg.n_voices, max_write);
 		return true;
+	}
+
+	void report_overlap(const Job &j, uint64_t ticket, bool mixer) {
+		if (!overlap_report_) return;
+		fprintf(stderr, "[sau-amd] overlap: mode %s set %u block %u mixer %s ticket %llu waits%s\n",
+				j.mode == MIXO_ALTERNATE ? "alternate" : j.mode == MIXO_SHARED ? "shared" : "off", j.set, j.block,
+				!mixer ? "none" : ticket ? "side" : "main", (unsigned long long)ticket, report_waits_.empty() ? " -" : report_waits_.c_str());
+		report_waits_.clear();
 	}
 
 	void report_inmix(const MixParams &mp, uint32_t n_voices, uint32_t max_write) {
@@ -1000,7 +1118,7 @@
 		uint32_t g[2] = {0, 0};
 		(void)hipStreamSynchronize(stream_);
 		(void)hipMemcpy(h.data(), mp.inmix, INMIX_WORDS * sizeof(uint32_t), hipMemcpyDeviceToHost);
-		(void)hipMemcpy(g, work_count_.p, sizeof g, hipMemcpyDeviceToHost);
+		(void)hipMemcpy(g, mp.guard, sizeof g, hipMemcpyDeviceToHost);
 		const uint32_t nch = h[INMIX_NCH] < INMIX_MAX_CHUNKS ? h[INMIX_NCH] : INMIX_MAX_CHUNKS, tpc = h[INMIX_TPC];
 		uint32_t tiles = 0, whole = 0, all = 0;
 		for (uint32_t k = 0; k < nch; ++k) {
@@ -1017,13 +1135,15 @@
 				n_voices, max_write, nch, h[INMIX_CF], tiles, all, whole, g[0], g[1]);
 	}
 
-	template <typename SetT> MixParams mix_params(const SegmentDesc &seg, const SetT &S) {
+	MixParams mix_params(const Job &j) {
+		const SegmentDesc &seg = j.seg;
+		const MixSet &S = sets_[j.set], &R = sets_[j.block];
 		MixParams mp;
-		mp.streams = S.mstreams.p; mp.vout = S.vout.p; mp.pan = S.pan.p; mp.vinfo = S.vinfo.p;
+		mp.streams = S.mstreams.p; mp.vout = R.vout.p; mp.pan = R.pan.p; mp.vinfo = S.vinfo.p;
 		mp.row_stride = row_stride_; mp.pcm_offset = seg.pcm_offset;
 		mp.stereo = seg.stereo ? 1 : 0;
 		mp.swap_bytes = seg.swap_bytes ? 1 : 0;
-		mp.blk_lo = 0; mp.blk_hi = 0; mp.early_blocks = 0; mp.guard = work_count_.p; mp.inmix = nullptr; mp.tail_ok = nullptr;
+		mp.blk_lo = 0; mp.blk_hi = 0; mp.early_blocks = 0; mp.guard = S.work_count.p; mp.inmix = nullptr; mp.tail_ok = nullptr;
 		return mp;
 	}
 
@@ -1037,6 +1157,7 @@
 	}
 	bool fetch_units(uint32_t stream, int16_t *dst, const size_t n, std::string &err) {
 		use_device();
+		if (!join_mixer("fetch_pcm", err)) return false;
 		const bool pinned = host_blocks_.count(dst) != 0;
 		if (!pinned && !h_pcm_.ensure(n, err)) return false;
 		HIP_OK(hipMemcpyAsync(pinned ? dst : h_pcm_.p, pcm_at(stream), n * sizeof(int16_t),
@@ -1059,6 +1180,7 @@
 	bool fetch_bytes_async(uint32_t stream, void *dst, size_t bytes, int slot, std::string &err) {
 		slot &= 3;
 		use_device();
+		if (!join_mixer("fetch_pcm_async", err)) return false;
 		if (!fetch_ev_[slot]) HIP_OK(hipEventCreateWithFlags(&fetch_ev_[slot], hipEventDisableTiming));
 		hipStream_t cs = stream_;
 		HIP_OK(hipMemcpyAsync(dst, pcm_at(stream), bytes, hipMemcpyDeviceToHost, cs));
@@ -1088,6 +1210,7 @@
 
 	bool begin_metering(std::string &err) override {
 		use_device();
+		if (!join_mixer("begin_metering", err)) return false;
 		if (lev_acc_.p) return true;
 		if (!lev_acc_.ensure(cfg_.n_streams, err)) return false;
 		HIP_OK(hipMemsetAsync(lev_acc_.p, 0, (size_t)cfg_.n_streams * sizeof(LevelsAcc), stream_));
@@ -1109,6 +1232,7 @@
 	}
 	bool measure_streams(const uint32_t *frames, bool stereo, sauengine::SampleFormat format, std::string &err) override {
 		use_device();
+		if (!join_mixer("measure_streams", err)) return false;
 		const bool f32 = format == sauengine::SF_F32;
 		if (!lev_acc_.p) { err = "level metering has not begun"; return false; }
 		if (f32 != pcm_f32_ || !pcm_.p) { err = "no rows of that sample format to measure"; return false; }
@@ -1147,6 +1271,7 @@
 	}
 	bool read_levels(sauengine::Levels *out, bool reset, std::string &err) override {
 		use_device();
+		if (!join_mixer("read_levels", err)) return false;
 		if (!lev_acc_.p) { memset((void *)out, 0, sizeof(sauengine::Levels) * cfg_.n_streams); return true; }
 		if (!read_records(lev_acc_.p, cfg_.n_streams, out, err)) return false;
 		if (reset) HIP_OK(hipMemsetAsync(lev_acc_.p, 0, (size_t)cfg_.n_streams * sizeof(LevelsAcc), stream_));
@@ -1155,6 +1280,7 @@
 	bool measure_rows(const void *rows, size_t pitch, size_t n_rows, sauengine::SampleFormat format, size_t frames, bool stereo,
 			sauengine::Levels *out, std::string &err) override {
 		use_device();
+		if (!join_mixer("measure_rows", err)) return false;
 		const bool f32 = format == sauengine::SF_F32;
 		const size_t ch = stereo ? 2 : 1, size = f32 ? sizeof(float) : sizeof(int16_t);
 		if (!n_rows) return true;
@@ -1186,6 +1312,7 @@
 	bool requantize(uint32_t stream, uint32_t frames, bool stereo, float gain, sauengine::SampleFormat out, bool swap_bytes,
 			std::string &err) override {
 		use_device();
+		if (!join_mixer("requantize", err)) return false;
 		if (!pcm_f32_ || !pcm_.p) { err = "the last run's samples are not float32"; return false; }
 		if (stream >= cfg_.n_streams || frames > row_stride_) { err = "frames beyond the stream's row"; return false; }
 		const bool f32 = out == sauengine::SF_F32;
@@ -1204,6 +1331,7 @@
 	bool fetch_requant_async(void *dst, size_t bytes, int slot, std::string &err) override {
 		slot &= 3;
 		use_device();
+		if (!join_mixer("fetch_requant_async", err)) return false;
 		if (bytes > requant_.bytes) { err = "more bytes than were requantised"; return false; }
 		if (!fetch_ev_[slot]) HIP_OK(hipEventCreateWithFlags(&fetch_ev_[slot], hipEventDisableTiming));
 		HIP_OK(hipMemcpyAsync(dst, requant_.p, bytes, hipMemcpyDeviceToHost, stream_));
@@ -1213,6 +1341,7 @@
 
 	bool begin_decimation(int factor, bool stereo, std::string &err) override {
 		use_device();
+		if (!join_mixer("begin_decimation", err)) return false;
 		const DecimPlan plan = plan_decimate(0, factor, stereo ? 2 : 1, cfg_.n_streams, sizeof(float));
 		if (!plan.ok) { err = "bad argument"; return false; }
 		const size_t hist = (size_t)cfg_.n_streams * plan.hist_floats;
@@ -1232,6 +1361,7 @@
 	bool decimate(const uint32_t *frames_hi, uint32_t buf_len, int factor, bool stereo, sauengine::SampleFormat out_fmt, bool swap_bytes,
 			std::string &err) override {
 		use_device();
+		if (!join_mixer("decimate", err)) return false;
 		if (!decim_hist_.p || factor != decim_factor_ || stereo != decim_stereo_) { err = "decimation has not begun"; return false; }
 		const bool f32 = out_fmt == sauengine::SF_F32;
 		if (f32 && swap_bytes) { err = "float32 samples are not byte-swapped"; return false; }
@@ -1271,6 +1401,7 @@
 	bool fetch_decimated_async(uint32_t stream, void *dst, size_t bytes, int slot, std::string &err) override {
 		slot &= 3;
 		use_device();
+		if (!join_mixer("fetch_decimated_async", err)) return false;
 		if (stream >= cfg_.n_streams || bytes > decim_out_bytes_ || (bytes && !decim_out_.p)) { err = "more bytes than were decimated"; return false; }
 		if (!fetch_ev_[slot]) HIP_OK(hipEventCreateWithFlags(&fetch_ev_[slot], hipEventDisableTiming));
 		if (bytes) {
@@ -1287,9 +1418,10 @@
 		return true;
 	}
 	const float *device_decimated_f32(uint32_t stream) override {
+		join_mixer_quiet("device_decimated");
 		return decim_out_.p && decim_out_f32_ && decim_out_bytes_ && stream < cfg_.n_streams ? (const float *)((const char *)decim_out_.p + decim_out_pitch_ * stream) : nullptr;
 	}
-	size_t device_decimated_pitch() override { return decim_out_.p && decim_out_bytes_ ? decim_out_pitch_ : 0; }
+	size_t device_decimated_pitch() override { join_mixer_quiet("device_decimated"); return decim_out_.p && decim_out_bytes_ ? decim_out_pitch_ : 0; }
 
 	struct LoudSet {
 		DevBuf<LoudState> state;
@@ -1423,11 +1555,13 @@
 	}
 	bool begin_loudness(std::string &err) override {
 		use_device();
+		if (!join_mixer("begin_loudness", err)) return false;
 		if (loud_own_.state.p) return true;
 		return loud_setup(cfg_.srate, err) && loud_make(loud_own_, cfg_.n_streams, err);
 	}
 	bool measure_loudness(const uint32_t *frames, bool stereo, std::string &err) override {
 		use_device();
+		if (!join_mixer("measure_loudness", err)) return false;
 		if (!loud_own_.state.p) { err = "loudness metering has not begun"; return false; }
 		if (!pcm_f32_ || !pcm_.p) { err = "the last run's samples are not float32"; return false; }
 		for (uint32_t s = 0; s < cfg_.n_streams; ++s)
@@ -1437,12 +1571,14 @@
 	}
 	bool read_loudness(sauengine::Loudness *out, bool reset, std::string &err) override {
 		use_device();
+		if (!join_mixer("read_loudness", err)) return false;
 		if (!loud_own_.state.p) { err = "loudness metering has not begun"; return false; }
 		if (!loud_setup(cfg_.srate, err) || !loud_read(loud_own_, out, nullptr, nullptr, err)) return false;
 		return !reset || loud_clear(loud_own_, err);
 	}
 	bool read_loudness_hops(uint32_t stream, double *out, size_t cap, size_t *n_hops, std::string &err) override {
 		use_device();
+		if (!join_mixer("read_loudness_hops", err)) return false;
 		if (!loud_own_.state.p || stream >= cfg_.n_streams) { err = "loudness metering has not begun"; return false; }
 		const uint32_t hop = cfg_.srate / 10;
 		const size_t nh = (size_t)(loud_own_.pos_h[stream] / hop), per = (size_t)loud_own_.rows * 2;
@@ -1456,6 +1592,7 @@
 	bool measure_loudness_rows(const void *rows, size_t pitch, size_t n_rows, size_t frames, bool stereo, uint32_t srate,
 			sauengine::Loudness *out, double *hops_out, size_t hops_cap, std::string &err) override {
 		use_device();
+		if (!join_mixer("measure_loudness_rows", err)) return false;
 		const size_t ch = stereo ? 2 : 1, size = sizeof(float);
 		if (!n_rows) return true;
 		if (!rows || ((uintptr_t)rows & 15u) || (pitch & 15u) || !out) { err = "bad argument: rows and pitch_bytes must be multiples of 16"; return false; }
@@ -1527,6 +1664,7 @@
 	}
 	bool begin_limiting(bool stereo, std::string &err) override {
 		use_device();
+		if (!join_mixer("begin_limiting", err)) return false;
 		const LimitPlan plan = plan_limit(0, cfg_.srate, stereo ? 2 : 1, cfg_.n_streams, sizeof(float));
 		if (!plan.ok) { err = "bad argument"; return false; }
 		const size_t hist = (size_t)cfg_.n_streams * plan.hist_frames * 2;
@@ -1542,6 +1680,7 @@
 	bool limit(const uint32_t *frames, uint32_t buf_len, float pre_gain, float ceiling, bool stereo, sauengine::SampleFormat out_fmt,
 			bool swap_bytes, std::string &err) override {
 		use_device();
+		if (!join_mixer("limit", err)) return false;
 		if (!lim_on_ || stereo != lim_stereo_) { err = "limiting has not begun"; return false; }
 		if (!sauengine::limiter_param_ok(pre_gain) || !sauengine::limiter_param_ok(ceiling)) { err = "bad argument"; return false; }
 		const bool f32 = out_fmt == sauengine::SF_F32;
@@ -1579,6 +1718,7 @@
 	bool fetch_limited_async(uint32_t stream, void *dst, size_t bytes, int slot, std::string &err) override {
 		slot &= 3;
 		use_device();
+		if (!join_mixer("fetch_limited_async", err)) return false;
 		if (stream >= cfg_.n_streams || bytes > lim_out_bytes_ || (bytes && !lim_out_.p)) { err = "more bytes than were limited"; return false; }
 		if (!fetch_ev_[slot]) HIP_OK(hipEventCreateWithFlags(&fetch_ev_[slot], hipEventDisableTiming));
 		if (bytes) {
@@ -1595,11 +1735,13 @@
 		return true;
 	}
 	const float *device_limited_f32(uint32_t stream) override {
+		join_mixer_quiet("device_limited");
 		return lim_out_.p && lim_out_f32_ && lim_out_bytes_ && stream < cfg_.n_streams ? (const float *)((const char *)lim_out_.p + lim_out_pitch_ * stream) : nullptr;
 	}
-	size_t device_limited_pitch() override { return lim_out_.p && lim_out_bytes_ ? lim_out_pitch_ : 0; }
+	size_t device_limited_pitch() override { join_mixer_quiet("device_limited"); return lim_out_.p && lim_out_bytes_ ? lim_out_pitch_ : 0; }
 	bool read_limiter_stats(sauengine::LimiterStats *out, bool reset, std::string &err) override {
 		use_device();
+		if (!join_mixer("read_limiter_stats", err)) return false;
 		if (!lim_stats_.p) { err = "limiting has not begun"; return false; }
 		HIP_OK(hipMemcpyAsync(out, lim_stats_.p, (size_t)cfg_.n_streams * sizeof(LimStats), hipMemcpyDeviceToHost, stream_));
 		HIP_OK(hipStreamSynchronize(stream_));
@@ -1622,6 +1764,7 @@
 	bool limit_rows(const void *rows, size_t pitch, size_t n_rows, size_t frames, bool stereo, uint32_t srate, float pre_gain, float ceiling,
 			void *out_rows, size_t out_pitch, sauengine::LimiterStats *stats_out, std::string &err) override {
 		use_device();
+		if (!join_mixer("limit_rows", err)) return false;
 		const size_t ch = stereo ? 2 : 1, row_bytes = frames * ch * sizeof(float);
 		if (!sauengine::limiter_param_ok(pre_gain) || !sauengine::limiter_param_ok(ceiling) || !srate) { err = "bad argument"; return false; }
 		if (!rows || !out_rows || ((uintptr_t)rows & 15u) || (pitch & 15u) || ((uintptr_t)out_rows & 15u) || (out_pitch & 15u)) {
@@ -1666,7 +1809,7 @@
 			: be_(be), n_(n_rows), ch_(channels), L_(log2n), N_(1u << log2n), bins_((1u << log2n) / 2 + 1), hop_(hop), pos_(n_rows, 0) {}
 		~Spectrum() override {
 			be_->use_device();
-			if (be_->stream_) (void)hipStreamSynchronize(be_->stream_);
+			if (be_->stream_) { be_->join_mixer_quiet("spectrum"); (void)hipStreamSynchronize(be_->stream_); }
 		}
 		size_t n_rows() const override { return n_; }
 		uint32_t channels() const override { return ch_; }
@@ -1684,12 +1827,14 @@
 			return clear(err);
 		}
 		bool clear(std::string &err) {
+			if (!be_->join_mixer("spectrum_clear", err)) return false;
 			HIP_OK(hipMemsetAsync(total_.p, 0, n_ * bins_ * ch_ * sizeof(double), be_->stream_));
 			std::fill(pos_.begin(), pos_.end(), 0);
 			return true;
 		}
 		bool feed_into(const void *rows, size_t pitch, const uint32_t *frames, float *sgram, size_t sgram_segs, std::string &err) {
 			be_->use_device();
+			if (!be_->join_mixer("spectrum_feed", err)) return false;
 			if (!rows || !frames || ((uintptr_t)rows & 15u) || (pitch & 15u)) { err = "bad argument: rows and pitch_bytes must be multiples of 16"; return false; }
 			uint32_t longest = 0;
 			for (size_t r = 0; r < n_; ++r) longest = frames[r] > longest ? frames[r] : longest;
@@ -1736,6 +1881,7 @@
 		}
 		bool read(double *power_out, uint64_t *segments_out, bool reset, std::string &err) override {
 			be_->use_device();
+			if (!be_->join_mixer("spectrum_read", err)) return false;
 			const size_t sums = n_ * bins_ * ch_;
 			std::vector<double> acc(sums);
 			HIP_OK(hipMemcpyAsync(power_out, total_.p, sums * sizeof(double), hipMemcpyDeviceToHost, be_->stream_));
@@ -1761,6 +1907,7 @@
 	};
 	sauengine::SpectrumMeter *create_spectrum(size_t n_rows, uint32_t channels, unsigned log2n, uint32_t hop, std::string &err) override {
 		use_device();
+		if (!join_mixer("create_spectrum", err)) return nullptr;
 		if (!sauengine::spectrum_params_ok((int)channels, log2n, hop) || !n_rows) { err = "bad argument"; return nullptr; }
 		if (n_rows > SPEC_MAX_ROWS) { err = "bad argument: more than 65535 rows"; return nullptr; }
 		Spectrum *m = new Spectrum(this, n_rows, channels, log2n, hop);
@@ -1770,6 +1917,7 @@
 	bool spectrum_rows(const void *rows, size_t pitch, size_t n_rows, size_t frames, uint32_t channels, unsigned log2n, uint32_t hop,
 			double *power_out, uint64_t *segments_out, float *spectrogram_out, size_t spectrogram_cap, std::string &err) override {
 		use_device();
+		if (!join_mixer("spectrum_rows", err)) return false;
 		if (!sauengine::spectrum_params_ok((int)channels, log2n, hop) || !n_rows || !power_out || !segments_out) { err = "bad argument"; return false; }
 		if (!rows || ((uintptr_t)rows & 15u) || (pitch & 15u)) { err = "bad argument: rows and pitch_bytes must be multiples of 16"; return false; }
 		if (n_rows > SPEC_MAX_ROWS || frames > 0xffffffffull) { err = "bad argument: more than 65535 rows, or than 32 bits of frames"; return false; }
@@ -1789,12 +1937,13 @@
 		return true;
 	}
 
-	const int16_t *device_pcm(uint32_t stream) override { return pcm_.p && !pcm_f32_ ? (const int16_t *)pcm_at(stream) : nullptr; }
-	const float *device_pcm_f32(uint32_t stream) override { return pcm_.p && pcm_f32_ ? (const float *)pcm_at(stream) : nullptr; }
-	size_t device_pcm_pitch() override { return pcm_.p ? pcm_pitch() : 0; }
+	const int16_t *device_pcm(uint32_t stream) override { join_mixer_quiet("device_pcm"); return pcm_.p && !pcm_f32_ ? (const int16_t *)pcm_at(stream) : nullptr; }
+	const float *device_pcm_f32(uint32_t stream) override { join_mixer_quiet("device_pcm"); return pcm_.p && pcm_f32_ ? (const float *)pcm_at(stream) : nullptr; }
+	size_t device_pcm_pitch() override { join_mixer_quiet("device_pcm"); return pcm_.p ? pcm_pitch() : 0; }
 
 	bool sync(std::string &err) override {
 		use_device();
+		if (!join_mixer("sync", err)) return false;
 		HIP_OK(hipStreamSynchronize(stream_));
 		arena_used_ = 0;
 		return true;
@@ -1802,6 +1951,7 @@
 	bool save_state(int slot, std::string &err) override {
 		slot &= 3;
 		use_device();
+		if (!join_mixer("save_state", err)) return false;
 		if (!ops_snap_[slot].ensure(ops_.cap, err)) return false;
 		HIP_OK(hipMemcpyAsync(ops_snap_[slot].p, ops_.p, ops_.cap * sizeof(DevOp), hipMemcpyDeviceToDevice, stream_));
 		return true;
@@ -1809,6 +1959,7 @@
 	bool load_state(int slot, std::string &err) override {
 		slot &= 3;
 		use_device();
+		if (!join_mixer("load_state", err)) return false;
 		if (!ops_snap_[slot].p || ops_snap_[slot].cap < ops_.cap) { err = "no operator state was saved under this slot"; return false; }
 		HIP_OK(hipMemcpyAsync(ops_.p, ops_snap_[slot].p, ops_.cap * sizeof(DevOp), hipMemcpyDeviceToDevice, stream_));
 		return true;
@@ -1816,6 +1967,8 @@
 
 	void timing(double *render_ms, double *mix_ms, uint64_t *launches, bool reset) override {
 		if (!timing_on_) { timing_on_ = true; }
+		use_device();
+		join_mixer_quiet("timing");
 		(void)hipStreamSynchronize(stream_);
 		drain_pairs();
 		if (render_ms) *render_ms = acc_ms_[0] + acc_ms_[2];
@@ -1825,13 +1978,14 @@
 	}
 
 	size_t chain_rows_budget() override { return sauengine::chain_rows_budget(free_hint_, chain_rows_failures_); }
-	void *stream_handle() override { return (void *)stream_; }
+	void *stream_handle() override { use_device(); join_mixer_quiet("stream_handle"); return (void *)stream_; }
 	bool order_after(HipBackend *before, std::string &err) override {
 		HipBackendImpl *o = static_cast<HipBackendImpl *>(before);
 		if (o == this) return true;
 		if (o->dev_ != dev_) { err = "sauAmd_Batch_order_after: the two batches are on different devices"; return false; }
 		use_device();
 		if (!after_ev_) HIP_OK(hipEventCreateWithFlags(&after_ev_, hipEventDisableTiming));
+		if (!o->join_mixer("order_after", err)) return false;
 		HIP_OK(hipEventRecord(after_ev_, o->stream_));
 		after_pending_ = true;
 		return true;
@@ -1842,10 +1996,12 @@
 		HIP_OK(hipStreamWaitEvent(stream_, after_ev_, 0));
 		return true;
 	}
-	void set_timing(int level) override { timing_on_ = level > 0; timing_level_ = level; }
+	void set_timing(int level) override { use_device(); join_mixer_quiet("set_timing"); timing_on_ = level > 0; timing_level_ = level; }
 
 	void timing_ex(double *out4, uint64_t *segments, bool reset) override {
 		if (!timing_on_) timing_on_ = true;
+		use_device();
+		join_mixer_quiet("timing");
 		(void)hipStreamSynchronize(stream_);
 		drain_pairs();
 		out4[0] = acc_ms_[2]; out4[1] = acc_ms_[0]; out4[2] = acc_ms_[1]; out4[3] = acc_ms_[3];
@@ -1853,7 +2009,10 @@
 		if (reset) { acc_ms_[0] = acc_ms_[1] = acc_ms_[2] = acc_ms_[3] = 0; acc_launches_ = 0; }
 	}
 
-	void debug_dump(const char *what, const SegmentDesc &seg, uint32_t block_grid) {
+	void debug_dump(const char *what, const Job &j) {
+		const SegmentDesc &seg = j.seg;
+		const uint32_t block_grid = j.block_grid;
+		const MixSet &S = sets_[j.set];
 		(void)hipStreamSynchronize(stream_);
 		uint32_t n = cfg_.op_count < 8 ? cfg_.op_count : 8;
 		std::vector<DevOp> h(n);
@@ -1865,7 +2024,7 @@
 					seg.voices[v].plan_ofs, seg.voices[v].plan_len, seg.voices[v].ops_ofs, seg.voices[v].nops);
 		{
 			uint32_t wc = 0;
-			(void)hipMemcpy(&wc, work_count_.p, 4, hipMemcpyDeviceToHost);
+			(void)hipMemcpy(&wc, S.work_count.p, 4, hipMemcpyDeviceToHost);
 			{
 				std::vector<FastInfo> all(seg.n_voices);
 				(void)hipMemcpy(all.data(), finfo_.p, all.size() * sizeof(FastInfo), hipMemcpyDeviceToHost);
@@ -1882,11 +2041,11 @@
 			std::vector<VoiceOut> vi(seg.n_voices < 4 ? seg.n_voices : 4);
 			std::vector<uint32_t> fd(vi.size());
 			std::vector<FastInfo> fi(vi.size());
-			(void)hipMemcpy(vi.data(), set_.vinfo.p, vi.size() * sizeof(VoiceOut), hipMemcpyDeviceToHost);
+			(void)hipMemcpy(vi.data(), S.vinfo.p, vi.size() * sizeof(VoiceOut), hipMemcpyDeviceToHost);
 			(void)hipMemcpy(fd.data(), fdone_.p, fd.size() * 4, hipMemcpyDeviceToHost);
 			(void)hipMemcpy(fi.data(), finfo_.p, fi.size() * sizeof(FastInfo), hipMemcpyDeviceToHost);
 			float v8[8] = {0};
-			(void)hipMemcpy(v8, set_.vout.p, sizeof v8, hipMemcpyDeviceToHost);
+			(void)hipMemcpy(v8, sets_[j.block].vout.p, sizeof v8, hipMemcpyDeviceToHost);
 			fprintf(stderr, "  work_count %u block_grid %u; row0: %g %g %g %g %g %g\n", wc, block_grid, v8[0], v8[1],
 					v8[2], v8[3], v8[4], v8[5]);
 			for (size_t v = 0; v < vi.size(); ++v)
@@ -1910,7 +2069,7 @@
 	TimedPair *new_pair(int kind) {
 		if (timing_level_ == 1 && kind != 2) return nullptr;
 		if (n_used_ == events_.size()) {
-			if (events_.size() >= 4096) { (void)hipStreamSynchronize(stream_); drain_pairs(); }
+			if (events_.size() >= 4096) { join_mixer_quiet("timing"); (void)hipStreamSynchronize(stream_); drain_pairs(); }
 			else {
 				TimedPair p; p.kind = 0; p.used = false;
 				if (hipEventCreate(&p.a) != hipSuccess || hipEventCreate(&p.b) != hipSuccess) return nullptr;
@@ -1953,11 +2112,21 @@
 		DevBuf<float> vout, pan;
 		DevBuf<VoiceOut> vinfo;
 		DevBuf<MixStream> mstreams;
+		DevBuf<uint32_t> work_count;
+		DevBuf<uint32_t> inmix_ctl;
+		DevBuf<uint32_t> tail_ok;
 		uint32_t vout_rows = 0;
 		std::vector<MixStream> ms_sent;
 		const void *ms_dev = nullptr;
 	};
-	MixSet set_;
+	MixSet sets_[2];
+	MixOverlapTracker mixo_;
+	hipStream_t mix_stream_ = nullptr;
+	bool mix_ready_ = false;
+	hipEvent_t mix_fork_[MIXO_RING] = {}, mix_done_[MIXO_RING] = {};
+	bool second_refused_ = false;
+	bool overlap_report_ = false;
+	std::string report_waits_;
 	DevBuf<int16_t> pcm_;
 	DevBuf<OpUpdate> recs_;
 	const TableSet *tables_ = nullptr;
@@ -1974,7 +2143,7 @@
 	uint64_t acc_launches_ = 0;
 	int timing_level_ = 2;
 	DevBuf<FastInfo> finfo_;
-	DevBuf<uint32_t> fdone_, worklist_, work_count_;
+	DevBuf<uint32_t> fdone_, worklist_;
 	DevBuf<float> big_slots_;
 	DevBuf<unsigned char> fsteps_, flines_, faux_;
 	DevBuf<unsigned long long> scan_;
@@ -1996,8 +2165,6 @@
 	DevBuf<unsigned char> fplines_;
 	hipEvent_t after_ev_ = nullptr;
 	bool after_pending_ = false;
-	DevBuf<uint32_t> inmix_ctl_;
-	DevBuf<uint32_t> tail_ok_;
 	DevBuf<LevelsAcc> lev_acc_, lev_out_;
 	DevBuf<LevelsPart> lev_parts_;
 	DevBuf<uint32_t> lev_frames_;
diff --git a/saugns_amd/csrc/launch_plan.h b/saugns_amd/csrc/launch_plan.h
--- a/saugns_amd/csrc/launch_plan.h
+++ b/saugns_amd/csrc/launch_plan.h
@@ -2,6 +2,7 @@
 #define SAU_LAUNCH_PLAN_H
 
 #include "engine.h"
+#include "mix_overlap.h"
 #include "sau_dev_math.h"
 #include <string.h>
 
@@ -80,6 +81,10 @@
 	bool early_mix = true;
 	bool mix64 = true;
 	bool poison = false;
+	bool mix_overlap = true;
+	bool mix_overlap_shared = false;
+	uint32_t mix_overlap_mb = 4096;
+	bool mix_overlap_fail = false;
 };
 
 inline Tuning tuning_from_env(const char *(*env)(const char *)) {
@@ -145,6 +150,10 @@
 	t.early_mix = off("SAU_AMD_NO_EARLY_MIX");
 	t.mix64 = off("SAU_AMD_NO_MIX64");
 	t.poison = !off("SAU_AMD_POISON");
+	t.mix_overlap = off("SAU_AMD_NO_MIX_OVERLAP");
+	t.mix_overlap_shared = !off("SAU_AMD_MIX_OVERLAP_SHARED");
+	if (const char *mb = env("SAU_AMD_MIX_OVERLAP_MB")) { const long n = atol(mb); t.mix_overlap_mb = n < 0 ? 0u : n > 0x7fffffffl ? 0x7fffffffu : (uint32_t)n; }
+	t.mix_overlap_fail = !off("SAU_AMD_MIX_OVERLAP_FAIL");
 	return t;
 }
 
@@ -535,6 +544,13 @@
 	return MIX_256;
 }
 
+inline MixOverlap plan_mix_overlap(const Tuning &tun, const PlanInputs &in, const FastPlan &fk, size_t rows_bytes, bool second_refused) {
+	if (!tun.mix_overlap || !in.max_write) return MIXO_OFF;
+	if (!fk.use_fast || fk.scan || !fk.queues || !fk.inmix) return MIXO_OFF;
+	if (fk.inner == INNER_NONE || tun.mix_overlap_shared || second_refused || rows_bytes > ((size_t)tun.mix_overlap_mb << 20)) return MIXO_SHARED;
+	return MIXO_ALTERNATE;
+}
+
 constexpr uint32_t LEVELS_THREADS = 256;
 constexpr uint32_t LEVELS_SWEEP_F32 = LEVELS_THREADS * 4, LEVELS_SWEEP_S16 = LEVELS_THREADS * 8;
 constexpr uint32_t LEVELS_WG_SAMPLES = 16384;
diff --git a/saugns_amd/csrc/mix_overlap.h b/saugns_amd/csrc/mix_overlap.h
--- /dev/null
+++ b/saugns_amd/csrc/mix_overlap.h
@@ -0,0 +1,48 @@
+#ifndef SAU_AMD_MIX_OVERLAP_H
+#define SAU_AMD_MIX_OVERLAP_H
+#include <stdint.h>
+
+namespace sauplan {
+
+enum MixOverlap : uint32_t {
+	MIXO_OFF = 0,
+	MIXO_SHARED,
+	MIXO_ALTERNATE
+};
+
+constexpr uint32_t MIXO_RING = 4;
+
+struct MixOverlapTracker {
+	uint64_t next = 0;
+	uint64_t joined = 0;
+	uint64_t set_reader[2] = {0, 0};
+	uint64_t rows_reader[2] = {0, 0};
+	uint64_t segments = 0;
+
+	uint32_t begin_segment() { return (uint32_t)(segments++ & 1u); }
+	static uint32_t block_of(MixOverlap mode, uint32_t set) { return mode == MIXO_ALTERNATE ? (set & 1u) : 0u; }
+
+	uint64_t before_records(uint32_t set) { return need(set_reader[set & 1u]); }
+	uint64_t before_rows(uint32_t block) { return need(rows_reader[block & 1u]); }
+	uint64_t before_pcm() { return need(next); }
+	uint64_t join() { return need(next); }
+	uint64_t next_ticket() const { return next + 1; }
+	uint64_t mixer_launched(uint32_t set, uint32_t block) {
+		++next;
+		set_reader[set & 1u] = next;
+		rows_reader[block & 1u] = next;
+		return next;
+	}
+	bool pending() const { return next > joined; }
+	static uint32_t slot(uint64_t ticket) { return (uint32_t)(ticket % MIXO_RING); }
+
+private:
+	uint64_t need(uint64_t t) {
+		if (t <= joined) return 0;
+		joined = t;
+		return t;
+	}
+};
+
+}
+#endif
```

After: 251.7 million, median of 6. +1.7%, better.
